# hsp-iit/roft

Hardware: AMD Instinct MI355X
Metric: tracker frames/sec per object (640x480) + ADD-S vs CPU ref (higher is better)
Workload: dtype f64; 1 GPU; BASELINE config #4: 640x480, CV_32FC2 flow grid 1, 64 objects in total, 64 per GPU (sharded by object, no data-path collective; result rows all-gathered over RCCL at N > 1), masks+poses at 5 fps with 6-frame delay, flow-aided masks, re-sync and outlier rejection on, frames submitted in batches of at most 8; objects_per_gpu=64, objects_total=64, width=640, height=480, batch_frames=8, ranks=1, backend=nccl

## Files before the change

include/roft_engine.h:

```cpp
#ifndef ROFT_ENGINE_H
#define ROFT_ENGINE_H

#include <stddef.h>
#include <stdint.h>

#ifdef __cplusplus
extern "C" {
#endif

#define ROFT_ABI_VERSION 2

#define ROFT_OK 0
#define ROFT_ERR_INVALID (-1)
#define ROFT_ERR_DEVICE (-2)
#define ROFT_ERR_CAPACITY (-3)
#define ROFT_ERR_STATE (-4)

#define ROFT_FLOW_S16C2 11
#define ROFT_FLOW_F32C2 13

#define ROFT_MEAS_NONE 0
#define ROFT_MEAS_VELOCITY 1
#define ROFT_MEAS_POSE 2
#define ROFT_MEAS_POSE_VELOCITY 3
// ... 53 lines not shown
                            int reweight, double x_out[6], double P_out[36], int* status_out);

int roft_mask_propagate(uint8_t* mask, int W, int H, const roft_flow* flows, int n_flows,
                        int frames_between);

int roft_pose_process_noise(const double psd_lin_acc[3], const double sigma_ang_vel[3], double T,
                            double Q[81]);
int roft_ukf_predict(const double mean[13], const double P[144], const double Q[81], double T,
                     const roft_ut_params* ut, double mean_out[13], double P_out[144]);
int roft_ukf_correct(const double mean[13], const double P[144], int type, const double* meas,
                     const double* Rdiag, const roft_ut_params* ut, double mean_out[13],
                     double P_out[144], int* status_out);

int roft_mesh_classify(const roft_mesh* mesh, uint8_t* flip_out, int* closed_out);
int roft_render_depth(const roft_mesh* mesh, const double x[3], const double q[4],
                      const roft_camera* cam, int divider, float* tile);
int roft_depth_likelihood(const roft_camera* cam, const float* depth, const uint8_t* mask,
                          const float* tile, int divider, double* L_out, long* samples_out);
int roft_outlier_test(const roft_camera* cam, int divider, const float* depth, const uint8_t* mask, const roft_mesh* mesh,
                      const double x[6], const double q[8], int bands, int vertex_cache, int window_pixels, double L_out[2],
                      long samples_out[2], int* selected_out, float* tiles_out);
int roft_outlier_test_split(const roft_camera* cam, int divider, const float* depth, const uint8_t* mask, const roft_mesh* mesh,
                            const double x[6], const double q[8], int bands, int vertex_cache, int window_pixels, int split,
                            double L_out[2], long samples_out[2], int* selected_out, float* tiles_out);
int roft_render_depth_mode(const roft_mesh* mesh, const double x[3], const double q[4], const roft_camera* cam, int divider, int mode,
                           float* tile);
int roft_outlier_test_mode(const roft_camera* cam, int divider, const float* depth, const uint8_t* mask, const roft_mesh* mesh,
                           const double x[6], const double q[8], int bands, int vertex_cache, int window_pixels, int split, int mode,
                           double L_out[2], long samples_out[2], int* selected_out, float* tiles_out);

#define ROFT_POSE_ERROR_ADD  0
#define ROFT_POSE_ERROR_ADDS 1
int roft_pose_errors(int kind, const double* points, int n_points, const double* est, const double* ref, int n_poses,
                     double* out);


typedef struct roft_engine roft_engine;

typedef struct {
    roft_camera cam;
    int flow_type;
    int flow_grid;
    float flow_scale;
    double sample_time;
    roft_ut_params ut;
    double depth_maximum;
    double subsampling_radius;
    int flow_weighting;
    int use_pose, use_pose_resync, use_velocity;
    int outlier_rejection;
    int flow_aided_segmentation;
    int mask_frames_between;
    int pose_frames_between;
    int stamped_masks;
    int max_objects;
    double ukf_cholesky_guard;
    double ukf_cholesky_guard_bilinear;
    int device;
    int max_batch_frames;
    int mask_workgroups_per_object;
    int outlier_bands_per_alternative;
    int render_mode;
} roft_config;

typedef struct {
    double p_mean0[13];
    double p_cov0_diag[12];
    double v_mean0[6];
    double v_cov0_diag[6];
    double p_sigma_ang_vel[3];
    double p_psd_lin_acc[3];
    double v_q_diag[6];
    double p_meas_cov_v[3], p_meas_cov_w[3], p_meas_cov_x[3], p_meas_cov_q[3];
    double v_meas_cov_flow[2];
    roft_mesh mesh;
} roft_object_desc;

#define ROFT_RETAIN_FRAMES 16
typedef struct {
    double dt;
    const float* depth;
    const void* flow;
    const uint8_t* mask;
    int pose_valid;
    double pose_x[3];
    double pose_q[4];
    int mem_kind;
    double stamp;
    double mask_stamp;
} roft_frame_input;

typedef struct {
    double pose[13];
    double twist[6];
    int n_flow_points;
    int outlier_selected;
    double outlier_L[2];
} roft_object_output;

int roft_default_config(roft_config* cfg, int width, int height, int flow_type);
int roft_default_object(roft_object_desc* obj);

int roft_engine_create(const roft_config* cfg, roft_engine** out);
int roft_engine_destroy(roft_engine* e);
int roft_object_add(roft_engine* e, const roft_object_desc* desc, int* obj_id);

#define ROFT_RESTART_KEEP_MESH 1
int roft_objects_restart(roft_engine* e, const int* obj_ids, const roft_object_desc* descs, int n, int flags);
typedef struct { long long calls, objects, meshes_replaced; } roft_engine_restart_stats;
int roft_engine_get_restart_stats(roft_engine* e, roft_engine_restart_stats* out);

int roft_frame_submit(roft_engine* e, const roft_frame_input* inputs, int n_inputs);
int roft_frames_submit(roft_engine* e, const roft_frame_input* inputs, int n_objects, int n_frames);

#define ROFT_LABEL_U8  1
#define ROFT_LABEL_U16 2
typedef struct {
    const void* labels;
    int label_type;
    int label;
} roft_label_mask;
int roft_frames_submit_labels(roft_engine* e, const roft_frame_input* inputs, const roft_label_mask* labels, int n_objects, int n_frames);
int roft_labels_to_masks(const void* labels, int label_type, int W, int H, const int* values, int n, uint8_t* masks_out, int* counts_out);

int roft_step(roft_engine* e);
int roft_engine_retain_frames(const roft_engine* e);
int roft_sync(roft_engine* e);
int roft_get_state(roft_engine* e, int obj_id, double pose13[13], double P12[144], double twist6[6],
                   double Pv[36]);
int roft_get_outputs(roft_engine* e, roft_object_output* outs, int n_outs);
int roft_get_mask(roft_engine* e, int obj_id, uint8_t* mask_out);

int roft_engine_enable_log(roft_engine* e, int n_frames);
int roft_engine_get_log(roft_engine* e, int first_frame, int n_frames, roft_object_output* outs);
int roft_engine_get_log_rows(roft_engine* e, int first_frame, int n_frames, double* rows);
int roft_engine_score_log(roft_engine* e, int kind, int obj_id, int first_frame, int n_frames, const double* points,
                          int n_points, const double* ref, double* out);

typedef struct {
    long long frames;
    long long batches;
    long long launches;
    long long event_ops;
    long long h2d_bytes;
    long long h2d_copies;
} roft_engine_stats;
int roft_engine_get_stats(roft_engine* e, roft_engine_stats* out);

typedef struct {
    int batch;
    int frames;
    int steady, throttled, handoff, early_lanes, outlier_parts_halved;
    int launches, event_ops;
    double t_submit_us;
    double submit_us;
    double wait_us;
    double step_us;
    double t_done_us;
} roft_batch_trace;
int roft_engine_get_batch_trace(roft_engine* e, roft_batch_trace* out, int capacity, int* n_out);

void* roft_engine_stream(roft_engine* e);

int roft_engine_enable_timing(roft_engine* e, int enable);
int roft_engine_get_timing(roft_engine* e, int* n_out, const char*** names_out, const float** ms_out,
                           const int** launches_out);

void* roft_host_alloc(size_t bytes);
void roft_host_free(void* p);
int roft_host_is_pinned(const void* p);

typedef struct {
    int levels;
    int radius;
    int iterations;
    float det_min;
} roft_of_params;

int roft_default_of_params(roft_of_params* p);

int roft_optical_flow(const uint8_t* prev_gray, const uint8_t* cur_gray, int W, int H, const roft_of_params* p,
                      int out_type, void* flow_out);

typedef struct roft_flow_producer roft_flow_producer;
int roft_flow_producer_create(int W, int H, int max_pairs, const roft_of_params* p, int out_type, int device,
                              roft_flow_producer** out);
int roft_flow_producer_destroy(roft_flow_producer* fp);
int roft_flow_producer_run(roft_flow_producer* fp, const uint8_t* const* prev, const uint8_t* const* cur,
                           void* const* out, int n_pairs);
int roft_flow_producer_sync(roft_flow_producer* fp);
void* roft_flow_producer_stream(roft_flow_producer* fp);

#define ROFT_IMAGE_GRAY8 1
#define ROFT_IMAGE_BGR8  2
#define ROFT_IMAGE_RGB8  3
typedef struct {
    const void* image;
    int image_type;
} roft_frame_image;
int roft_engine_enable_flow(roft_engine* e, const roft_of_params* p);
int roft_frames_submit_images(roft_engine* e, const roft_frame_input* inputs, const roft_label_mask* labels,
                              const roft_frame_image* images, int n_objects, int n_frames);
int roft_engine_get_flow(roft_engine* e, int obj_id, void* flow_out);
typedef struct {
    long long images;
    long long image_bytes;
    long long pyramids;
    long long pairs;
} roft_engine_flow_stats;
int roft_engine_get_flow_stats(roft_engine* e, roft_engine_flow_stats* out);
int roft_image_to_gray(const void* image, int image_type, int W, int H, uint8_t* gray_out);

typedef struct {
    float tolerance_abs, tolerance_rel;
} roft_of_consistency;
int roft_default_of_consistency(roft_of_consistency* c);
int roft_optical_flow_checked(const uint8_t* prev_gray, const uint8_t* cur_gray, int W, int H, const roft_of_params* p,
                              const roft_of_consistency* c, float* flow_out);
int roft_flow_producer_set_consistency(roft_flow_producer* fp, const roft_of_consistency* c);
int roft_engine_enable_flow_consistency(roft_engine* e, const roft_of_consistency* c);

#define ROFT_DEPTH_Z16 1
#define ROFT_DEPTH_ALIGN_MAX_SPAN 16
typedef struct {
    int   type;
    float scale;
    int   align;
    roft_camera cam;
    float R[9];
    float t[3];
} roft_depth_source;
int roft_engine_enable_raw_depth(roft_engine* e, const roft_depth_source* src);
int roft_engine_get_depth(roft_engine* e, int obj_id, float* depth_out);
typedef struct {
    long long images;
    long long image_bytes;
    long long products;
} roft_engine_depth_stats;
int roft_engine_get_depth_stats(roft_engine* e, roft_engine_depth_stats* out);
int roft_depth_convert(const uint16_t* raw, int W, int H, float scale, float* out);
int roft_depth_align(const uint16_t* raw, const roft_depth_source* src, const roft_camera* colour, float* out);

typedef struct {
    int32_t frame;
    int32_t n_mask;
    int32_t n_render;
    int32_t n_both;
    int32_t n_depth;
    int32_t n_front;
    int32_t n_behind;
    int32_t reserved;
    double  depth_err;
} roft_quality_record;
typedef struct {
    int   every;
    float depth_tolerance;
} roft_quality_params;
int roft_default_quality_params(roft_quality_params* p);
int roft_engine_enable_quality(roft_engine* e, const roft_quality_params* p);
int roft_engine_get_quality(roft_engine* e, int first_frame, int n_frames, roft_quality_record* out);
int roft_track_quality(const roft_camera* cam, int divider, const float* depth, const uint8_t* mask, const roft_mesh* mesh,
                       const double x[3], const double q[4], float depth_tolerance, double depth_maximum, int window_pixels,
                       roft_quality_record* out);

typedef struct {
    long long silhouettes;
    long long frames;
} roft_engine_pose_mask_stats;
int roft_engine_enable_pose_masks(roft_engine* e, const int* obj_ids, int n_ids);
int roft_engine_get_pose_mask_stats(roft_engine* e, roft_engine_pose_mask_stats* out);
int roft_pose_silhouette(const roft_camera* cam, const roft_mesh* mesh, const double x[3], const double q[4], int bands, int vertex_cache,
                         uint8_t* mask_out, int* count_out);

typedef struct {
    long long resolved;
    long long hidden;
    long long pixels_removed;
} roft_engine_pose_mask_occlusion_stats;
int roft_engine_enable_pose_mask_occlusion(roft_engine* e, const int* obj_ids, const int* scene_ids, int n_ids);
int roft_engine_get_pose_mask_occlusion_stats(roft_engine* e, roft_engine_pose_mask_occlusion_stats* out);
int roft_pose_silhouettes_occluded(const roft_camera* cam, const roft_mesh* meshes, int n, const double* x ,
                                   const double* q , int bands, int vertex_cache,
                                   uint8_t* masks_out , int* counts_out );

typedef struct {
    float front_tolerance;
    float behind_tolerance;
} roft_pose_mask_gate;
int roft_default_pose_mask_gate(roft_pose_mask_gate* g);
int roft_engine_enable_pose_mask_depth_gate(roft_engine* e, const roft_pose_mask_gate* g);
typedef struct {
    long long gated;
    long long emptied;
    long long pixels_front;
    long long pixels_behind;
} roft_engine_pose_mask_gate_stats;
int roft_engine_get_pose_mask_gate_stats(roft_engine* e, roft_engine_pose_mask_gate_stats* out);
int roft_pose_silhouettes_gated(const roft_camera* cam, const roft_mesh* meshes, int n, const double* x ,
                                const double* q , const float* depth , const roft_pose_mask_gate* g,
                                int bands, int vertex_cache, uint8_t* masks_out ,
                                int* counts_out , int* removed_out );

typedef struct {
    float tint[3];
    float opacity;
    float ambient;
} roft_scene_style;

#define ROFT_SCENE_MAX_INSTANCES 256

typedef struct {
    int n_frames;
    int n_instances;
    const int* mesh_index;
    const double* poses;
    const uint8_t* valid;
    const uint8_t* background;
    int background_frames;
    int gray_background;
    const roft_scene_style* styles;
    int window_pixels;
} roft_scene_desc;

typedef struct roft_scene_renderer roft_scene_renderer;
int roft_scene_renderer_create(const roft_camera* cam, const roft_mesh* meshes, int n_meshes, int max_frames_per_call, int device,
                               roft_scene_renderer** out);
int roft_scene_renderer_destroy(roft_scene_renderer* r);
int roft_scene_render(roft_scene_renderer* r, const roft_scene_desc* desc, uint8_t* rgb_out, float* depth_out, int32_t* instance_out,
                      int32_t* triangle_out);
int roft_render_scene(const roft_camera* cam, const roft_mesh* meshes, int n_meshes, const roft_scene_desc* desc, uint8_t* rgb_out,
                      float* depth_out, int32_t* instance_out, int32_t* triangle_out);

int roft_debug_plan(const roft_config* cfg, const int* pose_valid, int n_frames, int* n_steps, int* n_corrections,
                    int* outlier, int* slots);
int roft_debug_restart_check(const roft_config* cfg, int n_objects, const int* has_mesh, const int* enrolled, int enrol_all,
                             const int* obj_ids, const roft_object_desc* descs, int n, int flags);
int roft_debug_probe_streams(roft_engine* e, double out[25]);
int roft_debug_sector_rate(int device, double* sectors_per_second);
int roft_debug_get_residency(roft_engine* e, unsigned long long out[32]);
int roft_debug_outlier_split(int mode);
int roft_debug_pose_errors_kernel_ms(double* ms_out);
int roft_debug_scene_kernel_ms(roft_scene_renderer* r, double ms_out[2]);
int roft_debug_depth_kernel_ms(roft_engine* e, double* ms_out);
int roft_debug_quality_kernel_ms(roft_engine* e, double* ms_out);
int roft_debug_pose_mask_kernel_ms(roft_engine* e, double* ms_out);
int roft_debug_get_dbg(roft_engine* e, int obj_id, long long out[32]);

#ifdef __cplusplus
}
#endif
#endif
```

roft_amd/_lib.py:

```python
import collections
import ctypes as C
import os
import subprocess

_HERE = os.path.dirname(os.path.abspath(__file__))
CSRC = os.path.join(_HERE, "csrc")
SO = os.environ.get("ROFT_LIB_SO") or os.path.join(CSRC, "libroft_hip.so")

OK = 0
ERR_INVALID, ERR_DEVICE, ERR_CAPACITY, ERR_STATE = -1, -2, -3, -4
FLOW_S16C2 = 11
FLOW_F32C2 = 13
MEAS_NONE, MEAS_VELOCITY, MEAS_POSE, MEAS_POSE_VELOCITY = 0, 1, 2, 3
MEM_HOST, MEM_DEVICE = 0, 1
RETAIN_FRAMES = 16
MAX_BATCH_FRAMES = 8
MAX_FLOW_CHASE = 30
RENDER_CONTRACT, RENDER_GL = 0, 1
ABI_VERSION = 2
POSE_ERROR_ADD, POSE_ERROR_ADDS = 0, 1
RESTART_KEEP_MESH = 1
LABEL_U8, LABEL_U16 = 1, 2
IMAGE_GRAY8, IMAGE_BGR8, IMAGE_RGB8 = 1, 2, 3
DEPTH_Z16 = 1
DEPTH_ALIGN_MAX_SPAN = 16
SCENE_MAX_INSTANCES = 256


class RoftError(RuntimeError):
    pass


class Camera(C.Structure):
    _c_name_ = "roft_camera"
    _fields_ = [("width", C.c_int), ("height", C.c_int), ("fx", C.c_double), ("fy", C.c_double),
                ("cx", C.c_double), ("cy", C.c_double)]


class Flow(C.Structure):
    _c_name_ = "roft_flow"
    _fields_ = [("data", C.c_void_p), ("type", C.c_int), ("cols", C.c_int), ("rows", C.c_int),
                ("grid", C.c_int), ("scale", C.c_float), ("valid", C.c_int)]


class UT(C.Structure):
    _c_name_ = "roft_ut_params"
    _fields_ = [("alpha", C.c_double), ("beta", C.c_double), ("kappa", C.c_double)]


class OFParams(C.Structure):
    _c_name_ = "roft_of_params"
    _fields_ = [("levels", C.c_int), ("radius", C.c_int), ("iterations", C.c_int), ("det_min", C.c_float)]


class OFConsistency(C.Structure):
    _c_name_ = "roft_of_consistency"
    _fields_ = [("tolerance_abs", C.c_float), ("tolerance_rel", C.c_float)]


class Mesh(C.Structure):
    _c_name_ = "roft_mesh"
    _fields_ = [("verts", C.c_void_p), ("n_verts", C.c_int), ("tris", C.c_void_p), ("n_tris", C.c_int)]


class Config(C.Structure):
    _c_name_ = "roft_config"
    _fields_ = [("cam", Camera), ("flow_type", C.c_int), ("flow_grid", C.c_int), ("flow_scale", C.c_float),
                ("sample_time", C.c_double), ("ut", UT), ("depth_maximum", C.c_double),
                ("subsampling_radius", C.c_double), ("flow_weighting", C.c_int), ("use_pose", C.c_int),
                ("use_pose_resync", C.c_int), ("use_velocity", C.c_int), ("outlier_rejection", C.c_int),
                ("flow_aided_segmentation", C.c_int), ("mask_frames_between", C.c_int),
                ("pose_frames_between", C.c_int), ("stamped_masks", C.c_int), ("max_objects", C.c_int), ("ukf_cholesky_guard", C.c_double),
                ("ukf_cholesky_guard_bilinear", C.c_double),
                ("device", C.c_int), ("max_batch_frames", C.c_int), ("mask_workgroups_per_object", C.c_int),
                ("outlier_bands_per_alternative", C.c_int), ("render_mode", C.c_int)]


class ObjectDesc(C.Structure):
    _c_name_ = "roft_object_desc"
    _fields_ = [("p_mean0", C.c_double * 13), ("p_cov0_diag", C.c_double * 12), ("v_mean0", C.c_double * 6),
                ("v_cov0_diag", C.c_double * 6), ("p_sigma_ang_vel", C.c_double * 3),
                ("p_psd_lin_acc", C.c_double * 3), ("v_q_diag", C.c_double * 6),
                ("p_meas_cov_v", C.c_double * 3), ("p_meas_cov_w", C.c_double * 3),
                ("p_meas_cov_x", C.c_double * 3), ("p_meas_cov_q", C.c_double * 3),
                ("v_meas_cov_flow", C.c_double * 2), ("mesh", Mesh)]


class FrameInput(C.Structure):
    _c_name_ = "roft_frame_input"
    _fields_ = [("dt", C.c_double), ("depth", C.c_void_p), ("flow", C.c_void_p), ("mask", C.c_void_p),
                ("pose_valid", C.c_int), ("pose_x", C.c_double * 3), ("pose_q", C.c_double * 4),
                ("mem_kind", C.c_int), ("stamp", C.c_double), ("mask_stamp", C.c_double)]


class LabelMask(C.Structure):
    _c_name_ = "roft_label_mask"
    _fields_ = [("labels", C.c_void_p), ("label_type", C.c_int), ("label", C.c_int)]


class FrameImage(C.Structure):
    _c_name_ = "roft_frame_image"
    _fields_ = [("image", C.c_void_p), ("image_type", C.c_int)]


class EngineFlowStats(C.Structure):
    _c_name_ = "roft_engine_flow_stats"
    _fields_ = [("images", C.c_longlong), ("image_bytes", C.c_longlong), ("pyramids", C.c_longlong), ("pairs", C.c_longlong)]


class DepthSource(C.Structure):
    _c_name_ = "roft_depth_source"
    _fields_ = [("type", C.c_int), ("scale", C.c_float), ("align", C.c_int), ("cam", Camera), ("R", C.c_float * 9), ("t", C.c_float * 3)]


class EngineDepthStats(C.Structure):
    _c_name_ = "roft_engine_depth_stats"
    _fields_ = [("images", C.c_longlong), ("image_bytes", C.c_longlong), ("products", C.c_longlong)]


class QualityRecord(C.Structure):
    _c_name_ = "roft_quality_record"
    _fields_ = [("frame", C.c_int32), ("n_mask", C.c_int32), ("n_render", C.c_int32), ("n_both", C.c_int32), ("n_depth", C.c_int32),
                ("n_front", C.c_int32), ("n_behind", C.c_int32), ("reserved", C.c_int32), ("depth_err", C.c_double)]


class QualityParams(C.Structure):
    _c_name_ = "roft_quality_params"
    _fields_ = [("every", C.c_int), ("depth_tolerance", C.c_float)]


class EnginePoseMaskStats(C.Structure):
    _c_name_ = "roft_engine_pose_mask_stats"
    _fields_ = [("silhouettes", C.c_longlong), ("frames", C.c_longlong)]


class EnginePoseMaskOcclusionStats(C.Structure):
    _c_name_ = "roft_engine_pose_mask_occlusion_stats"
    _fields_ = [("resolved", C.c_longlong), ("hidden", C.c_longlong), ("pixels_removed", C.c_longlong)]


class PoseMaskGate(C.Structure):
    _c_name_ = "roft_pose_mask_gate"
    _fields_ = [("front_tolerance", C.c_float), ("behind_tolerance", C.c_float)]


class EnginePoseMaskGateStats(C.Structure):
    _c_name_ = "roft_engine_pose_mask_gate_stats"
    _fields_ = [("gated", C.c_longlong), ("emptied", C.c_longlong), ("pixels_front", C.c_longlong), ("pixels_behind", C.c_longlong)]


class EngineRestartStats(C.Structure):
    _c_name_ = "roft_engine_restart_stats"
    _fields_ = [("calls", C.c_longlong), ("objects", C.c_longlong), ("meshes_replaced", C.c_longlong)]


class EngineStats(C.Structure):
    _c_name_ = "roft_engine_stats"
    _fields_ = [("frames", C.c_longlong), ("batches", C.c_longlong), ("launches", C.c_longlong),
                ("event_ops", C.c_longlong), ("h2d_bytes", C.c_longlong), ("h2d_copies", C.c_longlong)]


class BatchTrace(C.Structure):
    _c_name_ = "roft_batch_trace"
    _fields_ = [("batch", C.c_int), ("frames", C.c_int), ("steady", C.c_int), ("throttled", C.c_int), ("handoff", C.c_int),
                ("early_lanes", C.c_int), ("outlier_parts_halved", C.c_int), ("launches", C.c_int), ("event_ops", C.c_int),
                ("t_submit_us", C.c_double), ("submit_us", C.c_double), ("wait_us", C.c_double), ("step_us", C.c_double),
                ("t_done_us", C.c_double)]


class ObjectOutput(C.Structure):
    _c_name_ = "roft_object_output"
    _fields_ = [("pose", C.c_double * 13), ("twist", C.c_double * 6), ("n_flow_points", C.c_int),
                ("outlier_selected", C.c_int), ("outlier_L", C.c_double * 2)]


class SceneStyle(C.Structure):
    _c_name_ = "roft_scene_style"
    _fields_ = [("tint", C.c_float * 3), ("opacity", C.c_float), ("ambient", C.c_float)]


class SceneDesc(C.Structure):
    _c_name_ = "roft_scene_desc"
    _fields_ = [("n_frames", C.c_int), ("n_instances", C.c_int), ("mesh_index", C.c_void_p), ("poses", C.c_void_p),
                ("valid", C.c_void_p), ("background", C.c_void_p), ("background_frames", C.c_int), ("gray_background", C.c_int),
                ("styles", C.c_void_p), ("window_pixels", C.c_int)]


Fn = collections.namedtuple("Fn", "name restype argtypes optional")
_int, _vp, _ip, _dp = C.c_int, C.c_void_p, C.POINTER(C.c_int), C.POINTER(C.c_double)
_P = C.POINTER
_REQUIRED, _OPTIONAL = False, True
ABI = (
    Fn("roft_last_error_string", C.c_char_p, [], _REQUIRED),
    Fn("roft_device_count", _int, [], _REQUIRED),
    Fn("roft_abi_version", _int, [], _REQUIRED),
    Fn("roft_flow_measurement", _int, [_P(Camera), _vp, _vp, _P(Flow), C.c_double, C.c_float, C.c_double, _int, _vp, _vp, _vp, _ip], _REQUIRED),
    Fn("roft_kf_predict", _int, [_vp] * 5, _REQUIRED),
    Fn("roft_skf_correct", _int, [_vp, _vp, _int, _vp, _vp, _vp, _int, _vp, _vp, _ip], _REQUIRED),
    Fn("roft_skf_correct_points", _int, [_P(Camera), C.c_double, _vp, _vp, _int, _vp, _vp, _vp, _vp, _int, _vp, _vp, _ip], _REQUIRED),
    Fn("roft_mask_propagate", _int, [_vp, _int, _int, _P(Flow), _int, _int], _REQUIRED),
    Fn("roft_pose_process_noise", _int, [_vp, _vp, C.c_double, _vp], _REQUIRED),
    Fn("roft_ukf_predict", _int, [_vp, _vp, _vp, C.c_double, _P(UT), _vp, _vp], _REQUIRED),
    Fn("roft_ukf_correct", _int, [_vp, _vp, _int, _vp, _vp, _P(UT), _vp, _vp, _ip], _REQUIRED),
    Fn("roft_mesh_classify", _int, [_P(Mesh), _vp, _ip], _REQUIRED),
    Fn("roft_render_depth", _int, [_P(Mesh), _vp, _vp, _P(Camera), _int, _vp], _REQUIRED),
    Fn("roft_depth_likelihood", _int, [_P(Camera), _vp, _vp, _vp, _int, _dp, _P(C.c_long)], _REQUIRED),
    Fn("roft_outlier_test", _int, [_P(Camera), _int, _vp, _vp, _P(Mesh), _vp, _vp, _int, _int, _int, _vp, _vp, _ip, _vp], _REQUIRED),
    Fn("roft_outlier_test_split", _int, [_P(Camera), _int, _vp, _vp, _P(Mesh), _vp, _vp, _int, _int, _int, _int, _vp, _vp, _ip, _vp], _REQUIRED),
    Fn("roft_render_depth_mode", _int, [_P(Mesh), _vp, _vp, _P(Camera), _int, _int, _vp], _REQUIRED),
    Fn("roft_outlier_test_mode", _int, [_P(Camera), _int, _vp, _vp, _P(Mesh), _vp, _vp, _int, _int, _int, _int, _int, _vp, _vp, _ip, _vp],
       _REQUIRED),
    Fn("roft_pose_errors", _int, [_int, _vp, _int, _vp, _vp, _int, _vp], _OPTIONAL),
    Fn("roft_default_config", _int, [_P(Config), _int, _int, _int], _REQUIRED),
    Fn("roft_default_object", _int, [_P(ObjectDesc)], _REQUIRED),
    Fn("roft_engine_create", _int, [_P(Config), _P(_vp)], _REQUIRED),
    Fn("roft_engine_destroy", _int, [_vp], _REQUIRED),
    Fn("roft_object_add", _int, [_vp, _P(ObjectDesc), _ip], _REQUIRED),
    Fn("roft_objects_restart", _int, [_vp, _ip, _P(ObjectDesc), _int, _int], _OPTIONAL),
    Fn("roft_engine_get_restart_stats", _int, [_vp, _P(EngineRestartStats)], _OPTIONAL),
    Fn("roft_frame_submit", _int, [_vp, _P(FrameInput), _int], _REQUIRED),
    Fn("roft_frames_submit", _int, [_vp, _P(FrameInput), _int, _int], _REQUIRED),
    Fn("roft_frames_submit_labels", _int, [_vp, _P(FrameInput), _P(LabelMask), _int, _int], _OPTIONAL),
    Fn("roft_labels_to_masks", _int, [_vp, _int, _int, _int, _ip, _int, _vp, _ip], _OPTIONAL),
    Fn("roft_step", _int, [_vp], _REQUIRED),
    Fn("roft_engine_retain_frames", _int, [_vp], _REQUIRED),
    Fn("roft_sync", _int, [_vp], _REQUIRED),
    Fn("roft_get_state", _int, [_vp, _int, _vp, _vp, _vp, _vp], _REQUIRED),
    Fn("roft_get_outputs", _int, [_vp, _P(ObjectOutput), _int], _REQUIRED),
    Fn("roft_get_mask", _int, [_vp, _int, _vp], _REQUIRED),
    Fn("roft_engine_enable_log", _int, [_vp, _int], _REQUIRED),
    Fn("roft_engine_get_log", _int, [_vp, _int, _int, _P(ObjectOutput)], _REQUIRED),
    Fn("roft_engine_get_log_rows", _int, [_vp, _int, _int, _vp], _REQUIRED),
    Fn("roft_engine_score_log", _int, [_vp, _int, _int, _int, _int, _vp, _int, _vp, _vp], _OPTIONAL),
    Fn("roft_engine_get_stats", _int, [_vp, _P(EngineStats)], _REQUIRED),
    Fn("roft_engine_get_batch_trace", _int, [_vp, _P(BatchTrace), _int, _ip], _REQUIRED),
    Fn("roft_engine_stream", _vp, [_vp], _REQUIRED),
    Fn("roft_engine_enable_timing", _int, [_vp, _int], _REQUIRED),
    Fn("roft_engine_get_timing", _int, [_vp, _ip, _P(_P(C.c_char_p)), _P(_P(C.c_float)), _P(_ip)], _REQUIRED),
    Fn("roft_host_alloc", _vp, [C.c_size_t], _REQUIRED),
    Fn("roft_host_free", None, [_vp], _REQUIRED),
    Fn("roft_host_is_pinned", _int, [_vp], _REQUIRED),
    Fn("roft_default_of_params", _int, [_P(OFParams)], _REQUIRED),
    Fn("roft_optical_flow", _int, [_vp, _vp, _int, _int, _P(OFParams), _int, _vp], _REQUIRED),
    Fn("roft_flow_producer_create", _int, [_int, _int, _int, _P(OFParams), _int, _int, _P(_vp)], _REQUIRED),
    Fn("roft_flow_producer_destroy", _int, [_vp], _REQUIRED),
    Fn("roft_flow_producer_run", _int, [_vp, _P(_vp), _P(_vp), _P(_vp), _int], _REQUIRED),
    Fn("roft_flow_producer_sync", _int, [_vp], _REQUIRED),
    Fn("roft_flow_producer_stream", _vp, [_vp], _REQUIRED),
    Fn("roft_engine_enable_flow", _int, [_vp, _P(OFParams)], _OPTIONAL),
    Fn("roft_frames_submit_images", _int, [_vp, _P(FrameInput), _P(LabelMask), _P(FrameImage), _int, _int], _OPTIONAL),
    Fn("roft_engine_get_flow", _int, [_vp, _int, _vp], _OPTIONAL),
    Fn("roft_engine_get_flow_stats", _int, [_vp, _P(EngineFlowStats)], _OPTIONAL),
    Fn("roft_image_to_gray", _int, [_vp, _int, _int, _int, _vp], _OPTIONAL),
    Fn("roft_default_of_consistency", _int, [_P(OFConsistency)], _OPTIONAL),
    Fn("roft_optical_flow_checked", _int, [_vp, _vp, _int, _int, _P(OFParams), _P(OFConsistency), _vp], _OPTIONAL),
    Fn("roft_flow_producer_set_consistency", _int, [_vp, _P(OFConsistency)], _OPTIONAL),
    Fn("roft_engine_enable_flow_consistency", _int, [_vp, _P(OFConsistency)], _OPTIONAL),
    Fn("roft_engine_enable_raw_depth", _int, [_vp, _P(DepthSource)], _OPTIONAL),
    Fn("roft_engine_get_depth", _int, [_vp, _int, _vp], _OPTIONAL),
    Fn("roft_engine_get_depth_stats", _int, [_vp, _P(EngineDepthStats)], _OPTIONAL),
    Fn("roft_depth_convert", _int, [_vp, _int, _int, C.c_float, _vp], _OPTIONAL),
    Fn("roft_depth_align", _int, [_vp, _P(DepthSource), _P(Camera), _vp], _OPTIONAL),
    Fn("roft_default_quality_params", _int, [_P(QualityParams)], _OPTIONAL),
    Fn("roft_engine_enable_quality", _int, [_vp, _P(QualityParams)], _OPTIONAL),
    Fn("roft_engine_get_quality", _int, [_vp, _int, _int, _vp], _OPTIONAL),
    Fn("roft_track_quality", _int, [_P(Camera), _int, _vp, _vp, _P(Mesh), _vp, _vp, C.c_float, C.c_double, _int, _P(QualityRecord)], _OPTIONAL),
    Fn("roft_engine_enable_pose_masks", _int, [_vp, _ip, _int], _OPTIONAL),
    Fn("roft_engine_get_pose_mask_stats", _int, [_vp, _P(EnginePoseMaskStats)], _OPTIONAL),
    Fn("roft_pose_silhouette", _int, [_P(Camera), _P(Mesh), _vp, _vp, _int, _int, _vp, _ip], _OPTIONAL),
    Fn("roft_engine_enable_pose_mask_occlusion", _int, [_vp, _ip, _ip, _int], _OPTIONAL),
    Fn("roft_engine_get_pose_mask_occlusion_stats", _int, [_vp, _P(EnginePoseMaskOcclusionStats)], _OPTIONAL),
    Fn("roft_pose_silhouettes_occluded", _int, [_P(Camera), _P(Mesh), _int, _vp, _vp, _int, _int, _vp, _ip], _OPTIONAL),
    Fn("roft_default_pose_mask_gate", _int, [_P(PoseMaskGate)], _OPTIONAL),
    Fn("roft_engine_enable_pose_mask_depth_gate", _int, [_vp, _P(PoseMaskGate)], _OPTIONAL),
    Fn("roft_engine_get_pose_mask_gate_stats", _int, [_vp, _P(EnginePoseMaskGateStats)], _OPTIONAL),
    Fn("roft_pose_silhouettes_gated", _int, [_P(Camera), _P(Mesh), _int, _vp, _vp, _vp, _P(PoseMaskGate), _int, _int, _vp, _ip, _ip], _OPTIONAL),
    Fn("roft_scene_renderer_create", _int, [_P(Camera), _P(Mesh), _int, _int, _int, _P(_vp)], _OPTIONAL),
    Fn("roft_scene_renderer_destroy", _int, [_vp], _OPTIONAL),
    Fn("roft_scene_render", _int, [_vp, _P(SceneDesc), _vp, _vp, _vp, _vp], _OPTIONAL),
    Fn("roft_render_scene", _int, [_P(Camera), _P(Mesh), _int, _P(SceneDesc), _vp, _vp, _vp, _vp], _OPTIONAL),
    Fn("roft_debug_plan", _int, [_P(Config), _vp, _int, _vp, _vp, _vp, _vp], _OPTIONAL),
    Fn("roft_debug_restart_check", _int, [_P(Config), _int, _ip, _ip, _int, _ip, _P(ObjectDesc), _int, _int], _OPTIONAL),
    Fn("roft_debug_probe_streams", _int, [_vp, _dp], _OPTIONAL),
    Fn("roft_debug_sector_rate", _int, [_int, _dp], _OPTIONAL),
    Fn("roft_debug_get_residency", _int, [_vp, _P(C.c_ulonglong)], _OPTIONAL),
    Fn("roft_debug_outlier_split", _int, [_int], _OPTIONAL),
    Fn("roft_debug_pose_errors_kernel_ms", _int, [_dp], _OPTIONAL),
    Fn("roft_debug_scene_kernel_ms", _int, [_vp, _dp], _OPTIONAL),
    Fn("roft_debug_depth_kernel_ms", _int, [_vp, _dp], _OPTIONAL),
    Fn("roft_debug_quality_kernel_ms", _int, [_vp, _dp], _OPTIONAL),
    Fn("roft_debug_pose_mask_kernel_ms", _int, [_vp, _dp], _OPTIONAL),
    Fn("roft_debug_get_dbg", _int, [_vp, _int, _P(C.c_longlong)], _OPTIONAL),
)
ABI_SYMBOLS = [f.name for f in ABI]
NEWER_SYMBOLS = tuple(f.name for f in ABI if f.optional and not f.name.startswith("roft_debug_"))


def build(force=False):
    srcs = [os.path.join(CSRC, f) for f in os.listdir(CSRC) if f.endswith((".hip", ".h"))]
    srcs.append(os.path.join(_HERE, "..", "include", "roft_engine.h"))
    stale = (not os.path.exists(SO)) or any(os.path.getmtime(s) > os.path.getmtime(SO) for s in srcs)
    if force or stale:
        jobs = str(min(8, os.cpu_count() or 1))
        r = subprocess.run(["make", "-C", CSRC, "-j", jobs, "libroft_hip.so"], capture_output=True, text=True)
        if r.returncode != 0:
            raise RoftError("building libroft_hip.so failed:\n" + r.stdout[-4000:] + r.stderr[-4000:])
    return SO


_lib = None


def lib():
    global _lib
    if _lib is not None:
        return _lib
    if not os.path.exists(SO):
        build()
    L = C.CDLL(SO)
    version = L.roft_abi_version() if hasattr(L, "roft_abi_version") else None
    if version != ABI_VERSION:
        raise RoftError("%s has ABI version %s, this binding mirrors version %d: rebuild the library" % (SO, version, ABI_VERSION))
    for f in ABI:
        if f.optional and not hasattr(L, f.name):
            continue
        fn = getattr(L, f.name)
        fn.restype, fn.argtypes = f.restype, f.argtypes
    _lib = L
    return L


def check(rc):
    if rc != OK:
        raise RoftError("libroft_hip error %d: %s" % (rc, lib().roft_last_error_string().decode()))


def require_device():
    if lib().roft_device_count() <= 0:
        raise RoftError("no HIP device visible: roft_amd has no CPU fallback")
```

roft_amd/csrc/batch_plan.h:

```cpp
#pragma once

#include <cstdlib>

namespace roft {
namespace host {

constexpr int kPlanLanes = 2;

struct SchedKnobs {
    int handoff_mode = 1;
    int prep_mode = 1;
    int part_mode = 1;
    int feat_mask_mode = 1;
    int lanes_wait_skf = 1;
    int early_lanes = 1;
    int ctrl_ingest = 1;
    int gather_copy = 1;
    int outlier_steady_div = 2;
    bool host_prof = false;
    bool host_prof_per_batch = false;
    bool one_stream = false;
};

inline SchedKnobs knobs_from_env()
{
    SchedKnobs k;
    auto num = [](const char* name, int& v) { const char* s = getenv(name); if (s) v = atoi(s); return s != nullptr; };
    num("ROFT_HANDOFF", k.handoff_mode);
    num("ROFT_PREP_AHEAD", k.prep_mode);
    num("ROFT_MASK_PART_GATE", k.part_mode);
    num("ROFT_FEAT_ON_MASK", k.feat_mask_mode);
    if (!num("ROFT_LANES_WAIT_SKF", k.lanes_wait_skf) && getenv("ROCPROF_COUNTER_COLLECTION")) k.handoff_mode = 0;
    num("ROFT_EARLY_LANES", k.early_lanes);
    num("ROFT_CTRL_INGEST", k.ctrl_ingest);
    num("ROFT_GATHER_COPY", k.gather_copy);
    num("ROFT_OUTLIER_STEADY_DIV", k.outlier_steady_div);
    const char* hp = getenv("ROFT_HOST_PROF");
    k.host_prof = hp && hp[0] == '1';
    k.host_prof_per_batch = k.host_prof && hp[1] == '+';
    const char* one = getenv("ROFT_ONE_STREAM");
    k.one_stream = one && one[0] == '1';
    return k;
}

struct SubmitFacts {
    int T = 1;
    bool had_uploads = false;
    bool produced_flows = false;
    unsigned plain_mask_frames = 0;
    int label_sets = 0;
    int pose_masks = 0;
    int pose_resolve = 0;
    bool any_feat = false, any_feat_now = false;
    bool feat_dep_in_batch = false;
    int n_segments[kPlanLanes] = {1, 1};
    bool lin_any[kPlanLanes] = {false, false};
    int lane_objs[kPlanLanes] = {0, 0}, lane_old_first[kPlanLanes] = {0, 0};
    int relabel_wait[kPlanLanes] = {-1, -1};
};

struct PlanInputs : SubmitFacts {
    SchedKnobs knobs;
    bool multi = true;
    bool timing = false;
    int timing_level = 2;
    bool wait_value_ok = true;
    bool have_skf_started = true;
    int n_obj = 0, cus = 256;
    int batch_counter = 0, idle_mark = 0, lead = 6, completed_batches = 0;
    int outlier_bands_per_alternative = 0;
    bool conflict_free = false;
    bool up_stream_distinct = true;
    bool feat_used_two_back = false;
    bool vel_used_prev = false;
    bool done_used_relabel[kPlanLanes] = {false, false};
    int quality_frames = 0;
};

enum class Signal {
    none,
    stop,
    record,
};
enum class FeatRun { none, mask_stream, behind_skf };
enum class VelWait { none, ev_ctrl, ev_part, ev_mask };
enum class Release {
    none,
    ev_vel,
    ev_skf,
    gate,
    ctrl_only,
};

struct LanePlan {
    bool early = false;
    bool wait_relabel = false;
    Release release = Release::none;
    bool wait_feat = false;
    bool wait_prev_vel = false;
    bool gate_second = false;
    Signal ev_done = Signal::none;
};

struct BatchPlan {
    bool steady = false, handoff = false;
    bool early_lanes = false;
    bool prep = false;
    bool prep_waits_mask = false, prep_waits_feat = false;
    bool wait_up = false;
    bool try_fused = false;
    bool label_ingest = false;
    bool pose_silhouettes = false;
    bool pose_resolve = false;
    Signal ev_ctrl = Signal::none, ev_prep = Signal::none;
    bool part_gate = false;
    Signal ev_mask = Signal::none;
    FeatRun feat = FeatRun::none;
    Signal ev_feat = Signal::none;
    VelWait vel_waits = VelWait::none;
    bool feat_waits_mask = false;
    Signal ev_skf = Signal::none, ev_vel = Signal::none;
    LanePlan lane[kPlanLanes];
    int outlier_div = 1;
    bool quality = false;
    bool quality_waits_mask = false;
    bool quality_waits_lane = false;
    Signal ev_quality = Signal::none;
};

template <class AloneFn>
BatchPlan plan_batch(const PlanInputs& in, AloneFn&& alone)
{
    const SchedKnobs& k = in.knobs;
    BatchPlan p;
    const bool multi = in.multi;
    const bool batch = multi && in.T > 1;
    const bool full = in.timing && in.timing_level > 1;
    auto ends = [full](bool signalled) { return !signalled ? Signal::none : full ? Signal::record : Signal::stop; };
    auto by_mode = [](int mode, bool by_index, bool by_count) { return mode == 2 || (mode == 3 && by_index) || (mode == 1 && by_index && by_count); };
    const bool cus_to_spare = 8 * in.n_obj <= in.cus;
    const bool own_sets = in.feat_dep_in_batch || in.any_feat_now;

    p.steady = in.batch_counter - in.idle_mark >= in.lead;

    p.handoff = batch && k.handoff_mode > 0 && in.wait_value_ok && !(k.handoff_mode == 1 && p.steady && !cus_to_spare) && !own_sets &&
                in.have_skf_started;
    const bool early_ok = p.handoff && !p.steady && k.early_lanes != 0 && in.conflict_free && alone();
    p.early_lanes = early_ok && cus_to_spare;
    bool any_early = false;
    for (int l = 0; l < kPlanLanes; ++l) {
        p.lane[l].early = p.early_lanes || (early_ok && in.n_segments[l] > 1 && in.lane_old_first[l] > 0 &&
                                            8 * (in.lane_objs[l] - in.lane_old_first[l]) <= in.cus && 2 * in.lane_objs[l] <= in.cus);
        any_early = any_early || p.lane[l].early;
    }

    p.prep = batch && in.up_stream_distinct && by_mode(k.prep_mode, p.steady, !cus_to_spare);
    p.prep_waits_mask = p.prep && in.batch_counter >= 2;
    p.prep_waits_feat = p.prep_waits_mask && in.feat_used_two_back;
    p.wait_up = multi && (in.had_uploads || in.produced_flows) && !p.prep;
    p.try_fused = k.ctrl_ingest != 0 && !p.prep && in.plain_mask_frames != 0 && !in.timing;
    p.ev_ctrl = (multi && (in.T == 1 || any_early)) ? Signal::stop : Signal::none;
    p.label_ingest = in.label_sets > 0;
    p.pose_silhouettes = in.pose_masks > 0;
    p.pose_resolve = p.pose_silhouettes && in.pose_resolve > 0;
    p.ev_prep = !p.prep ? Signal::none
                : (full || (in.plain_mask_frames == 0 && !p.label_ingest && !p.pose_silhouettes)) ? Signal::record : Signal::stop;

    p.part_gate = batch && by_mode(k.part_mode, !p.steady, cus_to_spare);
    p.ev_mask = ends(multi);

    const bool feat_behind_skf = batch && !(k.feat_mask_mode == 2 || (k.feat_mask_mode == 1 && 16 * in.n_obj <= in.cus));
    p.feat = !in.any_feat ? FeatRun::none : feat_behind_skf ? FeatRun::behind_skf : FeatRun::mask_stream;
    p.ev_feat = ends(multi && p.feat == FeatRun::mask_stream);

    p.vel_waits = !multi ? VelWait::none : in.T == 1 ? VelWait::ev_ctrl : p.part_gate ? VelWait::ev_part : VelWait::ev_mask;
    p.feat_waits_mask = p.feat == FeatRun::behind_skf && p.part_gate;
    const bool lanes_wait_skf = p.feat == FeatRun::behind_skf && k.lanes_wait_skf != 0 && !own_sets;
    p.ev_skf = ends(lanes_wait_skf);
    p.ev_vel = ends(multi);

    const bool lanes_wait_feat = p.ev_feat != Signal::none && (in.T > 1 || in.any_feat_now);
    for (int l = 0; l < kPlanLanes; ++l) {
        LanePlan& lp = p.lane[l];
        const int wb = in.relabel_wait[l];
        lp.wait_relabel = multi && wb >= in.completed_batches && wb < in.batch_counter && in.done_used_relabel[l];
        if (!in.lin_any[l]) continue;
        lp.ev_done = ends(true);
        if (!multi) continue;
        const bool tests = in.n_segments[l] > 1;
        if (lp.early) {
            lp.release = Release::ctrl_only;
            lp.wait_prev_vel = tests && in.batch_counter - 1 >= in.completed_batches && in.batch_counter >= 1 && in.vel_used_prev;
            lp.gate_second = !p.early_lanes;
        } else if (p.handoff) {
            lp.release = Release::gate;
        } else {
            lp.release = lanes_wait_skf ? Release::ev_skf : Release::ev_vel;
            lp.wait_feat = lanes_wait_feat && tests;
        }
    }

    p.quality = in.quality_frames > 0;
    p.quality_waits_mask = p.quality && multi;
    p.quality_waits_lane = p.quality && multi && in.lin_any[0];
    p.ev_quality = ends(p.quality);

    p.outlier_div = (in.outlier_bands_per_alternative == 0 && p.steady && k.outlier_steady_div > 1) ? k.outlier_steady_div : 1;
    return p;
}

enum class PrepLaunch { none, mask_ingest, label_ingest, pose_silhouettes, pose_resolve };
inline PrepLaunch prep_last_launch(const BatchPlan& p, unsigned plain_mask_frames)
{
    return p.pose_resolve ? PrepLaunch::pose_resolve
           : p.pose_silhouettes ? PrepLaunch::pose_silhouettes
           : p.label_ingest ? PrepLaunch::label_ingest
           : plain_mask_frames ? PrepLaunch::mask_ingest : PrepLaunch::none;
}
inline int pose_silhouette_launches(const BatchPlan& p) { return p.pose_resolve ? 2 : p.pose_silhouettes ? 1 : 0; }

}
}
```

roft_amd/csrc/engine_debug.hip:

```cpp
#include "engine_internal.h"


extern "C" int roft_debug_get_dbg(roft_engine* e, int id, long long out[32])
{
    if (!e || id < 0 || id >= (int)e->objs.size()) return ROFT_ERR_INVALID;
    if (roft_sync(e) != ROFT_OK) return ROFT_ERR_DEVICE;
    ObjState* st = new ObjState();
    hipError_t err = hipMemcpy(st, e->arr.state.p + id, sizeof(ObjState), hipMemcpyDeviceToHost);
    if (err == hipSuccess) std::memcpy(out, st->dbg, sizeof(long long) * 32);
    delete st;
    if (err == hipSuccess) err = hipMemset(reinterpret_cast<char*>(e->arr.state.p + id) + offsetof(ObjState, dbg), 0, sizeof(long long) * 32);
    return err == hipSuccess ? ROFT_OK : ROFT_ERR_DEVICE;
}

extern "C" int roft_debug_outlier_split(int mode)
{
    roft::set_outlier_split(mode);
    return ROFT_OK;
}

extern "C" int roft_debug_get_residency(roft_engine* e, unsigned long long out[32])
{
    if (!e || !out) return ROFT_ERR_INVALID;
    if (roft_sync(e) != ROFT_OK) return ROFT_ERR_DEVICE;
    if (hipMemcpy(out, e->arr.residency.p, sizeof(unsigned long long) * 32, hipMemcpyDeviceToHost) != hipSuccess) return ROFT_ERR_DEVICE;
    return hipMemset(e->arr.residency.p, 0, sizeof(unsigned long long) * 32) == hipSuccess ? ROFT_OK : ROFT_ERR_DEVICE;
}

extern "C" int roft_debug_sector_rate(int device, double* sectors_per_second)
{
    if (!sectors_per_second) return fail(ROFT_ERR_INVALID, "null output");
    HIP_TRY(hipSetDevice(device));
    const size_t bytes = (size_t)2 << 30;
    unsigned* buf = nullptr;
    unsigned* sink = nullptr;
    HIP_TRY(hipMalloc(reinterpret_cast<void**>(&buf), bytes));
    const int grid = 2048;
    hipError_t err = hipMalloc(reinterpret_cast<void**>(&sink), (size_t)grid * 1024 * sizeof(unsigned));
    hipEvent_t e0 = nullptr, e1 = nullptr;
    if (err == hipSuccess) err = hipMemset(buf, 0, bytes);
    if (err == hipSuccess) err = hipEventCreate(&e0);
    if (err == hipSuccess) err = hipEventCreate(&e1);
    float best_ms = 0.f;
    for (int rep = 0; rep < 5 && err == hipSuccess; ++rep) {
        (void)hipEventRecord(e0, nullptr);
        hipLaunchKernelGGL(probe_sectors_kernel, dim3(grid), dim3(1024), 0, nullptr, buf, (unsigned)(bytes / 64 - 1), 0x9e3779b9u * (unsigned)(rep + 1), sink);
        (void)hipEventRecord(e1, nullptr);
        err = hipEventSynchronize(e1);
        float ms = 0.f;
        if (err == hipSuccess) err = hipEventElapsedTime(&ms, e0, e1);
        if (rep > 0 && (best_ms == 0.f || ms < best_ms)) best_ms = ms;
    }
    if (e0) (void)hipEventDestroy(e0);
    if (e1) (void)hipEventDestroy(e1);
    (void)hipFree(sink);
    (void)hipFree(buf);
    if (err != hipSuccess || !(best_ms > 0.f)) return fail(ROFT_ERR_DEVICE, std::string("sector-rate probe: ") + hipGetErrorString(err));
    *sectors_per_second = (double)grid * 1024.0 * 8.0 / ((double)best_ms * 1e-3);
    return ROFT_OK;
}

extern "C" int roft_debug_probe_streams(roft_engine* e, double out[25])
{
    if (!e || !out) return ROFT_ERR_INVALID;
    if (roft_sync(e) != ROFT_OK) return ROFT_ERR_DEVICE;
    hipStream_t st[5] = {e->pose_stream[0], e->pose_stream[1], e->vel_stream, e->stream, e->up_stream};
    (void)set_max_dynamic_lds(reinterpret_cast<const void*>(probe_blocker_kernel), 150 * 1024);
    DevBuf<int> flag;
    if (flag.ensure(1) != hipSuccess) return ROFT_ERR_DEVICE;
    const int cus = device_cu_count();
    for (int a = 0; a < 5; ++a)
        for (int b = 0; b < 5; ++b) {
            out[a * 5 + b] = 0.0;
            if (a == b || st[a] == st[b]) continue;
            double best = 1e30;
            for (int rep = 0; rep < 3; ++rep) {
                (void)hipDeviceSynchronize();
                const double t0 = host_now_us();
                hipLaunchKernelGGL(probe_blocker_kernel, dim3(3 * cus), dim3(64), 150 * 1024, st[a], 10000ll);
                hipLaunchKernelGGL(probe_tiny_kernel, dim3(1), dim3(64), 0, st[b], flag.p);
                (void)hipStreamSynchronize(st[b]);
                best = std::min(best, host_now_us() - t0);
            }
            out[a * 5 + b] = best;
        }
    (void)hipDeviceSynchronize();
    return hipGetLastError() == hipSuccess ? ROFT_OK : ROFT_ERR_DEVICE;
}

extern "C" int roft_debug_plan(const roft_config* cfg, const int* pose_valid, int n_frames, int* n_steps, int* n_corrections,
                               int* outlier, int* slots )
{
    if (!cfg || !pose_valid || n_frames < 0) return ROFT_ERR_INVALID;
    Sched o;
    roft_frame_input in{};
    for (int k = 0; k < n_frames; ++k) {
        FrameCtrl c;
        clear_ctrl(c);
        in.pose_valid = pose_valid[k];
        if (!build_pose_program(*cfg, o, in, c)) return ROFT_ERR_CAPACITY;
        o.frame_idx++;
        o.track_frames++;
        if (n_steps) n_steps[k] = c.n_steps;
        int nc = 0;
        for (int s = 0; s < c.n_steps; ++s) {
            nc += c.steps[s].n_corr;
            if (slots) slots[k * kMaxSteps + s] = c.steps[s].twist_slot;
        }
        if (slots) for (int s = c.n_steps; s < kMaxSteps; ++s) slots[k * kMaxSteps + s] = -1;
        if (n_corrections) n_corrections[k] = nc;
        if (outlier) outlier[k] = c.outlier_step;
    }
    return ROFT_OK;
}
```

roft_amd/csrc/engine_internal.h:

```cpp
#pragma once

#include <hip/hip_runtime.h>

#include <algorithm>
#include <cfloat>
#include <chrono>
#include <cmath>
#include <cstdio>
#include <cstdlib>
#include <cstring>
#include <map>
#include <mutex>
#include <string>
#include <vector>

#include "roft_device.h"
#include "mesh_class.h"
#include "mesh_clusters.h"
#include "scene.h"
#include "batch_plan.h"
#include "pose_mask_gate.h"
#include "opticalflow.h"
#include "depth.h"
#include "quality.h"
// ... 11 lines not shown
    do {                                                                                                   \
        hipError_t _e = (expr);                                                                            \
        if (_e != hipSuccess)                                                                              \
            return fail(ROFT_ERR_DEVICE, std::string(#expr) + ": " + hipGetErrorString(_e));               \
    } while (0)
#define TRY(call) do { if (int _rc = (call)) return _rc; } while (0)

template <class T>
struct DevBuf {
    T* p = nullptr;
    size_t n = 0;
    DevBuf() = default;
    DevBuf(DevBuf&& o) noexcept { swap(o); }
    DevBuf& operator=(DevBuf&& o) noexcept { swap(o); return *this; }
    void swap(DevBuf& o) { std::swap(p, o.p); std::swap(n, o.n); }
    ~DevBuf() { release(); }
    void release()
    {
        if (p) (void)hipFree(p);
        p = nullptr;
        n = 0;
    }
    hipError_t ensure(size_t count, bool zero = false)
    {
        if (count <= n && p) return hipSuccess;
        release();
        hipError_t e = hipMalloc(reinterpret_cast<void**>(&p), std::max<size_t>(count, 1) * sizeof(T));
        if (e != hipSuccess) { p = nullptr; return e; }
        n = count;
        if (zero) e = hipMemset(p, 0, std::max<size_t>(count, 1) * sizeof(T));
        return e;
    }
};

inline int check_mesh(const roft_mesh& m, const std::string& what, bool may_be_absent, int tri_index_bits = 0)
{
    if (!has_mesh(m)) return may_be_absent ? ROFT_OK : fail(ROFT_ERR_INVALID, what + ": no vertices or no triangles");
    if (tri_index_bits > 0 && m.n_tris >= (1 << tri_index_bits))
        return fail(ROFT_ERR_INVALID, what + ": 2^" + std::to_string(tri_index_bits) + " triangles or more (a triangle's index is kept in that many bits)");
    const MeshFault f = check_mesh_arrays(m.verts, m.n_verts, m.tris, m.n_tris);
    if (f.kind == MeshFault::kNullArray) return fail(ROFT_ERR_INVALID, what + ": null vertex or triangle array");
    if (f.kind == MeshFault::kBadIndex)
        return fail(ROFT_ERR_INVALID, what + ": triangle " + std::to_string(f.triangle) + " refers to vertex " + std::to_string(f.vertex) + " of " +
                                          std::to_string(m.n_verts));
    return ROFT_OK;
}

struct DeviceMesh {
    DevBuf<float> verts;
    DevBuf<int32_t> tris;
    DevBuf<uint8_t> flip;
    DevBuf<uint32_t> cl_headers, cl_words;
    DevBuf<float> cl_slots, box_corners;
    int n_verts = 0, n_tris = 0, n_clusters = 0;
    bool closed = false;

    int upload(const roft_mesh& m, MeshLayout layout, hipStream_t s)
    {
        const bool clusters = layout == MeshLayout::kWalkClusters;
        n_verts = n_tris = n_clusters = 0;
        closed = false;
        if (!has_mesh(m)) return ROFT_OK;
        PreparedMesh pm;
        prepare_mesh(m.verts, m.n_verts, m.tris, m.n_tris, layout, pm);
        HIP_TRY(verts.ensure((size_t)3 * m.n_verts));
        HIP_TRY(tris.ensure((size_t)3 * m.n_tris));
        HIP_TRY(hipMemcpyAsync(verts.p, m.verts, sizeof(float) * 3 * m.n_verts, hipMemcpyHostToDevice, s));
        HIP_TRY(hipMemcpyAsync(tris.p, pm.tris(m.tris), sizeof(int32_t) * 3 * m.n_tris, hipMemcpyHostToDevice, s));
        if (pm.closed) {
            HIP_TRY(flip.ensure((size_t)m.n_tris));
            HIP_TRY(hipMemcpyAsync(flip.p, pm.flip.data(), (size_t)m.n_tris, hipMemcpyHostToDevice, s));
        }
        MeshClusters mc;
        if (clusters) {
            build_clusters(m.verts, m.n_verts, pm.tris(m.tris), m.n_tris, pm.closed ? pm.flip.data() : nullptr,
                           pm.bucket.empty() ? nullptr : pm.bucket.data(), mc);
            HIP_TRY(cl_headers.ensure(mc.headers.size()));
            HIP_TRY(cl_slots.ensure(mc.slots.size()));
            HIP_TRY(cl_words.ensure(mc.words.size()));
            HIP_TRY(box_corners.ensure(24));
            HIP_TRY(hipMemcpyAsync(cl_headers.p, mc.headers.data(), sizeof(uint32_t) * mc.headers.size(), hipMemcpyHostToDevice, s));
            HIP_TRY(hipMemcpyAsync(cl_slots.p, mc.slots.data(), sizeof(float) * mc.slots.size(), hipMemcpyHostToDevice, s));
            HIP_TRY(hipMemcpyAsync(cl_words.p, mc.words.data(), sizeof(uint32_t) * mc.words.size(), hipMemcpyHostToDevice, s));
            HIP_TRY(hipMemcpyAsync(box_corners.p, &mc.box[0][0], sizeof(float) * 24, hipMemcpyHostToDevice, s));
        }
        HIP_TRY(hipStreamSynchronize(s));
        n_verts = m.n_verts;
        n_tris = m.n_tris;
        n_clusters = mc.n_clusters;
        closed = pm.closed;
        return ROFT_OK;
    }

    SceneMesh scene_mesh() const
    {
        const bool has = has_mesh(*this);
        return SceneMesh{has ? verts.p : nullptr, has ? tris.p : nullptr, closed ? flip.p : nullptr, n_verts, n_tris};
    }
    void describe(ObjParams& p) const
    {
        const SceneMesh m = scene_mesh();
        p.verts = m.verts; p.tris = m.tris; p.tri_flip = m.flip;
        p.n_verts = m.n_verts; p.n_tris = m.n_tris;
        const bool cl = has_mesh(*this) && n_clusters > 0;
        p.cl_headers = cl ? cl_headers.p : nullptr; p.cl_slots = cl ? cl_slots.p : nullptr; p.cl_words = cl ? cl_words.p : nullptr;
        p.box_corners = cl ? box_corners.p : nullptr; p.n_clusters = cl ? n_clusters : 0;
    }
};

inline size_t flow_bytes(const DevFlowFmt& f)
{
    return (size_t)f.cols * f.rows * 2 * (f.type == ROFT_FLOW_S16C2 ? sizeof(int16_t) : sizeof(float));
}

inline DevCamera make_cam(const roft_camera& c)
{
    DevCamera d;
    d.W = c.width;
    d.H = c.height;
    d.wpr = c.width / 32;
    d.divider = (c.width == 640) ? 2 : 4;
    d.fx = c.fx; d.fy = c.fy; d.cx = c.cx; d.cy = c.cy;
    return d;
}

inline int check_geometry(int W, int H)
{
    if (W <= 0 || H <= 0 || (W % 32) != 0 || (((size_t)W * H) % 64) != 0)
        return fail(ROFT_ERR_INVALID, "image width must be a multiple of 32 and width*height a multiple of 64");
    if ((size_t)W * H >= (1u << 24))
        return fail(ROFT_ERR_INVALID, "width*height must be < 2^24 (float-accumulated sampling index, hpp:237)");
    return ROFT_OK;
}

struct Arrays {
    EngineArrays a{};
    DevBuf<ObjParams> params;
    DevBuf<ObjState> state;
    DevBuf<FrameCtrl> ctrl;
    DevBuf<uint32_t> planes;
    DevBuf<int32_t> map;
    DevBuf<FlowRec> cand, recs;
    DevBuf<double> norms;
    DevBuf<int> npts;
    DevBuf<MaskRec> mrec;
    DevBuf<unsigned> mask_general;
    DevBuf<uint32_t> feat_pix;
    DevBuf<float> feat_depth;
    DevBuf<uint32_t> zbuf;
    DevBuf<uint32_t> zmerge;
    DevBuf<int> zcount;
    int ensure_zmerge(int n, size_t tpix)
    {
        const size_t slabs = std::max<size_t>((size_t)n, std::min<size_t>((size_t)n * kMaxOutlierParts, (size_t)std::max(device_cu_count() / 2, 1)));
        const size_t need = (size_t)kNumLin * slabs * 2 * tpix;
        if (need > zmerge.n || !zmerge.p || tpix != a.zmerge_stride || slabs != a.zmerge_slabs) {
            HIP_TRY(zmerge.ensure(need));
            a.zmerge_stride = tpix;
            a.zmerge_slabs = slabs;
        }
        HIP_TRY(zcount.ensure((size_t)kNumLin * n * 2 * kMaxOutlierParts, true));
        a.zmerge = zmerge.p;
        a.zcount = zcount.p;
        return ROFT_OK;
    }
    DevBuf<roft_object_output> log;
    DevBuf<unsigned long long> skf_started, residency;

    int alloc(int n_obj, int T, const DevCamera& cam, const DevFlowFmt& ffmt, int radius)
    {
        a.n_obj = n_obj;
        a.T = 1;
        a.cam = cam;
        a.ffmt = ffmt;
        a.plane_words = (size_t)cam.wpr * cam.H;
        const size_t npix = (size_t)cam.W * cam.H;
        a.cand_cap = ((int)((npix + radius - 1) / std::max(radius, 1)) + 9) & ~1;
        a.feat_cap = (int)(npix / 2 + 8);
        a.tile_w = cam.W / cam.divider;
        a.tile_h = cam.H / cam.divider;
        HIP_TRY(params.ensure(n_obj, true));
        HIP_TRY(state.ensure(n_obj, true));
        HIP_TRY(ctrl.ensure((size_t)n_obj * T, true));
        HIP_TRY(planes.ensure((size_t)n_obj * kPlaneSlotsTotal * 2 * a.plane_words, true));
        HIP_TRY(mrec.ensure((size_t)2 * n_obj * (kMaxBatch + 1), true));
        HIP_TRY(mask_general.ensure(n_obj, true));
        HIP_TRY(map.ensure((size_t)n_obj * npix, true));
        HIP_TRY(cand.ensure((size_t)n_obj * T * a.cand_cap));
        HIP_TRY(recs.ensure((size_t)n_obj * T * a.cand_cap));
        HIP_TRY(npts.ensure((size_t)n_obj * T, true));
        HIP_TRY(norms.ensure((size_t)n_obj * 3 * a.cand_cap));
        HIP_TRY(feat_pix.ensure((size_t)n_obj * kFeatRing * a.feat_cap));
        HIP_TRY(feat_depth.ensure((size_t)n_obj * kFeatRing * a.feat_cap));
        HIP_TRY(zbuf.ensure((size_t)2 * a.tile_w * a.tile_h));
        if (int rc = ensure_zmerge(n_obj, (size_t)a.tile_w * a.tile_h)) return rc;
        a.params = params.p; a.state = state.p; a.ctrl = ctrl.p; a.planes = planes.p; a.map = map.p;
        a.cand = cand.p; a.recs = recs.p; a.norms = norms.p; a.npts = npts.p; a.mrec = mrec.p;
        a.mask_general = mask_general.p;
        a.mrec_carry = mrec.p; a.slot_new = kSlotNew; a.slot_prev0 = -1; a.feat_pix = feat_pix.p; a.feat_depth = feat_depth.p;
        a.zbuf = zbuf.p;
        a.out_log = nullptr;
        a.log_cap = 0;
        a.max_tris = 0;
        a.max_verts = 0;
        a.meshes_without_clusters = 0;
        a.ukf_chol_guard = 0.0;
        a.ukf_chol_guard_bil = 0.0;
        a.mask_wgs = 0;
        a.outlier_parts = 0;
        a.dev_error = nullptr;
        a.k1_span = nullptr;
        HIP_TRY(skf_started.ensure(1, true));
        HIP_TRY(residency.ensure(32, true));
        a.residency = residency.p;
        a.skf_started = nullptr;
        a.handoff = 0;
        return ROFT_OK;
    }
};

struct PoseErrorScratch {
    DevBuf<double> pts, est, ref, cloud, partial, out;
    hipEvent_t ev0 = nullptr, ev1 = nullptr;
    bool timed = false;
    ~PoseErrorScratch()
    {
        if (ev0) (void)hipEventDestroy(ev0);
        if (ev1) (void)hipEventDestroy(ev1);
    }
};
int pose_errors_run(PoseErrorScratch& sc, int kind, const double* d_pts, int P, const double* est_host, PoseView est_dev,
                    const double* ref_host, int n, double* out_host, hipStream_t s);

inline void init_state(ObjState& st)
{
    std::memset(&st, 0, sizeof(st));
    for (PoseLane& pl : st.lane) { pl.pending_frame = -1; pl.outlier_selected = -1; }
    st.n_flow_points = -1;
}

inline void clear_ctrl(FrameCtrl& c)
{
    std::memset(&c, 0, sizeof(c));
    c.outlier_step = -1;
    c.feat_write = c.feat_read = -1;
}



struct FlowEntry {
    const void* ptr;
    int frame;
    int owned;
    const float* depth_before;
};

struct Sched {
    int frame_idx = 0;
    int track_frames = 0;
    bool seg_available = false;
    bool of_first_frame = true;
    bool flow_first_frame = true;
    bool features_initialized = false;
    int feat_slot = 0;
    int feat_next = 0;
    int feat_use[kFeatRing];
    int feat_batch[kFeatRing];
    int n_hist = 0;
    FlowEntry hist[kMaxFlowHist];
    int n_stamps = 0;
    double stamps[30];
    int n_vel = 0;
    int vel_buf[kTwistRing];
    int last_meas_slot = 0;
    int cur_slot = 0;
    int own[kNumLin] = {0, 1};
    int last_touch[kNumLin] = {-1, -1};
    int flows_since_mask = 0;
    int flows_buffered = 0;
    const float* depth_prev = nullptr;
    int pyr_prev = -1;
    const void* flow_made = nullptr;
    Sched() { for (int i = 0; i < kFeatRing; ++i) feat_use[i] = feat_batch[i] = -1; }
};

struct OwnedFlow {
    DevBuf<unsigned char> buf;
    DevBuf<float> depth;
    int last_ref_frame = -1;
};

struct HostObject {
    Sched s;
    int stepped_slot = 0, stepped_lane = 0;
    const void* stepped_flow = nullptr;
    const float* stepped_depth = nullptr;
    std::vector<OwnedFlow*> owned;
    DeviceMesh mesh;
    bool pose_masks = false;
    int pose_scene = -1, pose_zscene = -1;
    double pose0[7] = {0, 0, 0, 1, 0, 0, 0};
    roft_object_output last_out{};
    bool last_out_valid = false;
    ~HostObject() { for (auto* o : owned) delete o; }
};

struct FlowImageJob { const void* dev; int type; };
// ... 248 lines not shown
```

roft_amd/csrc/engine_step.hip:

```cpp
#include "engine_internal.h"

__global__ void ctrl_upload_kernel(const uint4* __restrict__ src, EngineArrays a, size_t n16, int reset)
{
    uint4* dst = reinterpret_cast<uint4*>(a.ctrl);
    const size_t i0 = (size_t)blockIdx.x * blockDim.x + threadIdx.x, stride = (size_t)gridDim.x * blockDim.x;
    for (size_t i = i0; i < n16; i += stride) dst[i] = src[i];
    if (reset)
        for (size_t i = i0; i < (size_t)a.T * a.n_obj; i += stride) roft::mask_reset_tables(a, i);
}


static hipEvent_t push_mark(roft_engine* e, const char* name, int which)
{
    const size_t idx = e->tmark.size();
    while (e->tev.size() <= idx) {
        hipEvent_t ev;
        (void)hipEventCreate(&ev);
        e->tev.push_back(ev);
    }
    int id = -1;
    if (name) {
        for (size_t i = 0; i < e->tnames_s.size(); ++i)
            if (e->tnames_s[i] == name) id = (int)i;
        if (id < 0) { e->tnames_s.push_back(name); id = (int)e->tnames_s.size() - 1; }
// ... 15 lines not shown
    if (!e->timing) return;
    *start = push_mark(e, nullptr, which);
    *stop = push_mark(e, name, which);
}

#define CHECK_LAUNCH(what)                                                                              \
    do {                                                                                                \
        hipError_t _e = hipGetLastError();                                                              \
        if (_e != hipSuccess) return fail(ROFT_ERR_DEVICE, std::string(what) + ": " + hipGetErrorString(_e)); \
    } while (0)

struct Enqueue {
    roft_engine* e;
    const BatchPlan& p;
    BatchSlot& cur;
    EngineArrays a;
    long long& launches;
    long long& evops;
    int wait(hipStream_t s, hipEvent_t ev)
    {
        HIP_TRY(hipStreamWaitEvent(s, ev, 0));
        ++evops;
        return ROFT_OK;
    }
    int wait_gate(hipStream_t s)
    {
        HIP_TRY(hipStreamWaitValue64(s, e->arr.skf_started.p, e->skf_total, hipStreamWaitValueGte, ~0ull));
        ++evops;
        return ROFT_OK;
    }
    static hipEvent_t stop(Signal how, hipEvent_t ev) { return how == Signal::stop ? ev : nullptr; }
    int signalled(Signal how, hipEvent_t ev, hipStream_t s)
    {
        if (how != Signal::record) return ROFT_OK;
        HIP_TRY(hipEventRecord(ev, s));
        ++evops;
        return ROFT_OK;
    }
};

static int enqueue_preparation(Enqueue& q)
{
    roft_engine* e = q.e;
    const PendingBatch& pb = e->pending;
    const BatchPlan& p = q.p;
    const EngineArrays& a = q.a;
    hipStream_t s = e->stream, sp = p.prep ? e->up_stream : s;
    if (p.wait_up) TRY(q.wait(s, q.cur.ev_up));
    if (p.prep_waits_mask) {
        BatchSlot& two_back = e->slot_of(e->batch_counter - 2);
        TRY(q.wait(sp, two_back.ev_mask));
        if (p.prep_waits_feat) TRY(q.wait(sp, two_back.ev_feat));
    }
    tmark(e, nullptr, p.prep ? 4 : 0);
    static_assert(sizeof(FrameCtrl) % 16 == 0, "FrameCtrl is copied in 16-byte units");
    const size_t n16 = (sizeof(FrameCtrl) * (size_t)a.n_obj * a.T + (p.label_ingest ? pb.label_table_bytes : 0)) / 16;
    const hipEvent_t ctrl_stop = Enqueue::stop(p.ev_ctrl, q.cur.ev_ctrl);
    const PrepLaunch last_launch = prep_last_launch(p, pb.facts.plain_mask_frames);
    auto label_ingest = [&]() -> int {
        LabelIngestArgs la;
        la.sets = reinterpret_cast<const LabelSet*>(a.ctrl + (size_t)a.n_obj * a.T);
        la.members = reinterpret_cast<const LabelMember*>(la.sets + pb.label_sets.size());
        la.planes = a.planes;
        la.plane_words = a.plane_words;
        la.obj_stride = (size_t)kPlaneSlotsTotal * 2 * a.plane_words;
        la.slot0 = a.slot_new;
        la.mrec = a.mrec;
        la.n_obj = a.n_obj;
        la.n_grp = a.cam.W * a.cam.H / 64;
        launch_label_ingest(la, (int)pb.label_sets.size(), sp, last_launch == PrepLaunch::label_ingest ? Enqueue::stop(p.ev_prep, q.cur.ev_prep) : nullptr);
        ++q.launches;
        CHECK_LAUNCH("label image ingest");
        return ROFT_OK;
    };
    auto pose_silhouettes = [&]() -> int {
        EnginePoseMasks& pm = e->pose_masks;
        SilhouetteArgs sa{};
        sa.ctrl = a.ctrl;
        sa.params = a.params;
        sa.planes = a.planes;
        sa.plane_words = a.plane_words;
        sa.obj_stride = (size_t)kPlaneSlotsTotal * 2 * a.plane_words;
        sa.slot0 = a.slot_new;
        sa.mrec = a.mrec;
        sa.n_obj = a.n_obj;
        sa.W = a.cam.W; sa.H = a.cam.H; sa.wpr = a.cam.wpr;
        sa.fx = (float)a.cam.fx; sa.fy = (float)a.cam.fy; sa.cx = (float)a.cam.cx; sa.cy = (float)a.cam.cy;
        int n_frames = 0;
        for (int t = 0; t < a.T && t < 8; ++t)
            if (pb.pose_mask_frames & (1u << t)) sa.frames_packed |= (unsigned)t << (4 * n_frames++);
        if (p.pose_resolve) {
            const int par = e->batch_counter & 1;
            sa.n_zscenes = pm.n_zscenes;
            sa.zbuf = pm.zbuf.p + (size_t)par * kMaxBatch * pm.n_zscenes * a.cam.W * a.cam.H;
            sa.zpairs = pm.zpairs.p + (size_t)par * kMaxBatch * e->cfg.max_objects;
            sa.zstats = pm.zstats.p;
        }
        if (pm.gate) {
            sa.gate = 1;
            sa.gate_tf = pm.gate_prm.front_tolerance;
            sa.gate_tb = pm.gate_prm.behind_tolerance;
            sa.gstats = pm.gstats.p;
            sa.zpairs = pm.zpairs.p + (size_t)(e->batch_counter & 1) * kMaxBatch * e->cfg.max_objects;
        }
        const int slot = e->batch_counter % roft_engine::kBatchRing;
        const hipEvent_t plan_stop = Enqueue::stop(p.ev_prep, q.cur.ev_prep);
        if (!p.prep) tmark(e, nullptr, 0);
        const int launched = launch_pose_silhouette(sa, n_frames, a.max_verts, 0, 1, sp, pm.ev_start[slot], plan_stop ? plan_stop : pm.ev_stop[slot]);
        if (launched != pose_silhouette_launches(p))
            return fail(ROFT_ERR_INVALID, "pose masks: the image does not fit the kernel's bit window");
        pm.last_slot = slot;
        pm.last_timed = plan_stop == nullptr;
        q.launches += launched;
        CHECK_LAUNCH(p.pose_resolve ? "pose silhouettes: clear, draw and resolve" : "pose silhouettes");
        if (!p.prep) tmark(e, "pose_silhouettes", 0);
        return ROFT_OK;
    };
    if (p.try_fused && launch_ctrl_ingest(q.cur.stage, a, n16, pb.facts.plain_mask_frames, sp, ctrl_stop)) {
        ++q.launches;
        CHECK_LAUNCH("FrameCtrl upload + mask ingest");
        if (p.label_ingest) TRY(label_ingest());
        return p.pose_silhouettes ? pose_silhouettes() : ROFT_OK;
    }
    hipExtLaunchKernelGGL(ctrl_upload_kernel, dim3((unsigned)std::min<size_t>((n16 + 255) / 256, 64)), dim3(256), 0, sp, nullptr, ctrl_stop, 0,
                          reinterpret_cast<const uint4*>(q.cur.stage), a, n16, 1);
    ++q.launches;
    CHECK_LAUNCH("FrameCtrl upload");
    int last = -1;
    for (int t = 0; t < a.T; ++t)
        if (pb.facts.plain_mask_frames & (1u << t)) last = t;
    for (int t = 0; t <= last; ++t)
        if (pb.facts.plain_mask_frames & (1u << t)) {
            launch_mask_ingest(a, t, sp, (t == last && last_launch == PrepLaunch::mask_ingest) ? Enqueue::stop(p.ev_prep, q.cur.ev_prep) : nullptr);
            ++q.launches;
        }
    CHECK_LAUNCH("mask ingest");
    if (p.label_ingest) TRY(label_ingest());
    if (p.pose_silhouettes) TRY(pose_silhouettes());
    if (p.prep) {
        TRY(q.signalled(p.ev_prep, q.cur.ev_prep, sp));
        tmark(e, "mask_prepare", 4);
        TRY(q.wait(s, q.cur.ev_prep));
    }
    return ROFT_OK;
}

static int enqueue_mask_frames(Enqueue& q)
{
    roft_engine* e = q.e;
    const BatchPlan& p = q.p;
    hipStream_t s = e->stream;
    tmark(e, nullptr, 0);
    q.launches += launch_mask_chain(q.a, e->cfg.mask_frames_between, e->cfg.flow_aided_segmentation, e->pending.new_mask_frames, s,
                                    Enqueue::stop(p.ev_mask, q.cur.ev_mask), p.part_gate ? q.cur.ev_part : nullptr);
    CHECK_LAUNCH("mask chain");
    tmark(e, "mask_chain", 0);
    TRY(q.signalled(p.ev_mask, q.cur.ev_mask, s));
    q.cur.feat_used = p.ev_feat != Signal::none;
    if (p.feat == FeatRun::mask_stream) {
        launch_features(q.a, s, Enqueue::stop(p.ev_feat, q.cur.ev_feat), e->pending.feat_frames);
        ++q.launches;
        CHECK_LAUNCH("features");
        tmark(e, "features", 0);
        TRY(q.signalled(p.ev_feat, q.cur.ev_feat, s));
    }
    return ROFT_OK;
}

static int enqueue_velocity(Enqueue& q)
{
    roft_engine* e = q.e;
    const BatchPlan& p = q.p;
    const EngineArrays& a = q.a;
    hipStream_t sv = e->vel_stream;
    if (p.vel_waits != VelWait::none)
        TRY(q.wait(sv, p.vel_waits == VelWait::ev_ctrl ? q.cur.ev_ctrl : p.vel_waits == VelWait::ev_part ? q.cur.ev_part : q.cur.ev_mask));
    {
        hipEvent_t k1_start = nullptr, k1_stop = nullptr;
        tmark_kernel(e, "flow_measure", 2, &k1_start, &k1_stop);
        EngineArrays ak = a;
        if (e->timing && (int)e->span_wgs.size() < roft_engine::kSpanLaunches && e->k1_span.p) {
            ak.k1_span = e->k1_span.p + (size_t)2 * kMaxBatch * e->cfg.max_objects * e->span_wgs.size();
            e->span_wgs.push_back(a.T * a.n_obj);
        }
        launch_flow_measure(ak, e->cfg.depth_maximum, (int)(size_t)e->cfg.subsampling_radius, sv, k1_start, k1_stop);
        ++q.launches;
        CHECK_LAUNCH("flow measurement");
    }
    const bool feat_behind = p.feat == FeatRun::behind_skf;
    const Signal skf_how = feat_behind ? p.ev_skf : p.ev_vel;
    const hipEvent_t skf_ev = feat_behind ? q.cur.ev_skf : q.cur.ev_vel;
    q.cur.vel_used = p.ev_vel != Signal::none;
    launch_skf_chain(a, e->cfg.flow_weighting, sv, Enqueue::stop(skf_how, skf_ev));
    ++q.launches;
    if (hipError_t le = hipGetLastError()) {
        e->knobs.handoff_mode = 0;
        return fail(ROFT_ERR_DEVICE, std::string("velocity filter chain: ") + hipGetErrorString(le));
    }
    e->skf_total += (unsigned long long)a.n_obj;
    tmark(e, "skf_chain", 2);
    TRY(q.signalled(skf_how, skf_ev, sv));
    if (feat_behind) {
        if (p.feat_waits_mask) TRY(q.wait(sv, q.cur.ev_mask));
        launch_features(a, sv, Enqueue::stop(p.ev_vel, q.cur.ev_vel), e->pending.feat_frames);
        ++q.launches;
        CHECK_LAUNCH("features");
        tmark(e, "features", 2);
        TRY(q.signalled(p.ev_vel, q.cur.ev_vel, sv));
    }
    return ROFT_OK;
}

static int enqueue_lane(Enqueue& q, int lin)
{
    roft_engine* e = q.e;
    const LanePlan& lp = q.p.lane[lin];
    hipStream_t sp = e->pose_stream[lin];
    q.cur.done_used[lin] = lp.ev_done != Signal::none;
    const SubmitFacts& facts = e->pending.facts;
    if (lp.wait_relabel) TRY(q.wait(sp, e->slot_of(facts.relabel_wait[lin]).ev_done[1 - lin]));
    if (!facts.lin_any[lin]) return ROFT_OK;
    const int which = lin == 0 ? 1 : 3;
    switch (lp.release) {
    case Release::none: break;
    case Release::ctrl_only: TRY(q.wait(sp, q.cur.ev_ctrl)); break;
    case Release::gate: TRY(q.wait_gate(sp)); break;
    case Release::ev_skf: TRY(q.wait(sp, q.cur.ev_skf)); break;
    case Release::ev_vel: TRY(q.wait(sp, q.cur.ev_vel)); break;
    }
    if (lp.wait_feat) TRY(q.wait(sp, q.cur.ev_feat));
    tmark(e, nullptr, which);
    OutlierLaunchOpts oo;
    oo.render_mode = e->cfg.render_mode;
    if (q.p.outlier_div > 1) oo.parts = -q.p.outlier_div;
    const int n_seg = facts.n_segments[lin];
    for (int seg = 0; seg < n_seg; ++seg) {
        const bool last = seg == n_seg - 1;
        if (seg == 1 && lp.gate_second) TRY(q.wait_gate(sp));
        launch_ukf_chain(q.a, e->cfg.ut, seg == 0, lin, sp, last ? Enqueue::stop(lp.ev_done, q.cur.ev_done[lin]) : nullptr);
        ++q.launches;
        CHECK_LAUNCH("pose chain segment");
        tmark(e, "ukf_chain", which);
        if (last) break;
        if (seg == 0 && lp.wait_prev_vel) TRY(q.wait(sp, e->slot_of(e->batch_counter - 1).ev_vel));
        TRY(launch_outlier(q.a, lin, sp, nullptr, &oo));
        ++q.launches;
        CHECK_LAUNCH("outlier rejection");
        tmark(e, "outlier_render_likelihood", which);
    }
    return q.signalled(lp.ev_done, q.cur.ev_done[lin], sp);
}

static int enqueue_quality(Enqueue& q)
{
    roft_engine* e = q.e;
    const BatchPlan& p = q.p;
    q.cur.quality_used = p.ev_quality != Signal::none;
    if (!p.quality) return ROFT_OK;
    const int slot = e->batch_counter % roft_engine::kBatchRing;
    hipStream_t sp = e->pose_stream[kNumLin - 1];
    if (p.quality_waits_mask) TRY(q.wait(sp, q.cur.ev_mask));
    if (p.quality_waits_lane) TRY(q.wait(sp, q.cur.ev_done[0]));
    int n_frames = 0;
    const unsigned packed = quality_frames_of_batch(e, &n_frames);
    EngineQuality& eq = e->quality;
    launch_quality(q.a, eq.ring.p, eq.cap, packed, n_frames, eq.prm.depth_tolerance, e->cfg.depth_maximum, 0, sp, eq.ev_start[slot],
                   Enqueue::stop(p.ev_quality, eq.ev_done[slot]));
    ++q.launches;
    CHECK_LAUNCH("track quality");
    tmark(e, "track_quality", 3);
    eq.last_slot = slot;
    return q.signalled(p.ev_quality, eq.ev_done[slot], sp);
}

static PlanInputs plan_inputs(roft_engine* e)
{
    PlanInputs in;
    static_cast<SubmitFacts&>(in) = e->pending.facts;
    in.knobs = e->knobs;
    in.multi = e->multi();
    in.timing = e->timing;
    in.timing_level = e->timing_level;
    in.wait_value_ok = e->wait_value_ok;
    in.have_skf_started = e->arr.skf_started.p != nullptr;
    in.n_obj = e->arr.a.n_obj;
    in.cus = device_cu_count();
    in.batch_counter = e->batch_counter; in.idle_mark = e->idle_mark; in.lead = e->lead; in.completed_batches = e->completed_batches;
    in.outlier_bands_per_alternative = e->cfg.outlier_bands_per_alternative;
    in.conflict_free = e->streams && e->streams->conflicts == 0;
    in.up_stream_distinct = e->up_stream != e->stream;
    if (e->quality.enabled) (void)quality_frames_of_batch(e, &in.quality_frames);
    in.feat_used_two_back = e->batch_counter >= 2 && e->slot_of(e->batch_counter - 2).feat_used;
    in.vel_used_prev = e->batch_counter >= 1 && e->slot_of(e->batch_counter - 1).vel_used;
    for (int l = 0; l < kNumLin; ++l) in.done_used_relabel[l] = in.relabel_wait[l] >= 0 && e->slot_of(in.relabel_wait[l]).done_used[1 - l];
    return in;
}

int step_batch(roft_engine* e)
{
    const PendingBatch& pb = e->pending;
    const int T = pb.facts.T;
    double hp_t = e->knobs.host_prof ? host_now_us() : 0.0;
    (void)hipGetLastError();
    const BatchPlan p = plan_batch(plan_inputs(e), [e] { return e->alone_on_device = alone_on_device(e->streams); });
    BatchSlot& cur = e->slot_of(e->batch_counter);
    Enqueue q{e, p, cur, e->arr.a, e->stats.launches, e->stats.event_ops};
    EngineArrays& a = q.a;
    a.T = T;
    a.ctrl = cur.dctrl.p;
    {
        const size_t table = (size_t)(kMaxBatch + 1) * a.n_obj;
        const int par = e->batch_counter & 1;
        MaskRec* base = e->arr.mrec.p;
        a.mrec = base + par * table;
        a.mrec_carry = e->prev_T > 0 ? base + (1 - par) * table + (size_t)e->prev_T * a.n_obj : a.mrec;
        a.slot_new = kSlotNew + par * kMaxBatch;
        a.slot_prev0 = (e->frame_counter + kPlaneSlots - 1) % kPlaneSlots;
    }
    a.handoff = p.handoff ? 1 : 0;
    a.skf_started = e->arr.skf_started.p;
    const long long launches0 = e->stats.launches, evops0 = e->stats.event_ops;

    TRY(enqueue_preparation(q));
    HP_MARK(e, 3, hp_t);
    TRY(enqueue_mask_frames(q));
    HP_MARK(e, 4, hp_t);
    TRY(enqueue_velocity(q));
    HP_MARK(e, 5, hp_t);
    for (int lin = 0; lin < kNumLin; ++lin) TRY(enqueue_lane(q, lin));
    TRY(enqueue_quality(q));
    HP_MARK(e, 6, hp_t);
    if (e->knobs.host_prof) {
        e->hp_batches++;
        if (e->knobs.host_prof_per_batch)
            std::fprintf(stderr, "[roft host batch %d T=%d] ctrl %.1f mask %.1f vel %.1f lanes %.1f us (cumulative)\n", e->batch_counter, T,
                         e->hp_acc[3], e->hp_acc[4], e->hp_acc[5], e->hp_acc[6]);
    }
    {
        roft_batch_trace& tr = e->trace[e->batch_counter % roft_engine::kTraceRing];
        tr = roft_batch_trace{};
        tr.batch = e->batch_counter;
        tr.frames = T;
        tr.steady = p.steady; tr.throttled = pb.throttled; tr.handoff = p.handoff;
        tr.early_lanes = (p.early_lanes ? 4 : 0) | (p.lane[0].early ? 1 : 0) | (p.lane[1].early ? 2 : 0);
        tr.outlier_parts_halved = p.outlier_div > 1 ? 1 : 0;
        tr.launches = (int)(e->stats.launches - launches0);
        tr.event_ops = (int)(e->stats.event_ops - evops0);
        tr.t_submit_us = pb.submit_t0; tr.submit_us = pb.submit_us; tr.wait_us = pb.wait_us;
    }
    HIP_TRY(hipGetLastError());
    return ROFT_OK;
}

int roft_step(roft_engine* e)
{
    if (!e) return fail(ROFT_ERR_INVALID, "null engine");
    if (!e->submitted) return fail(ROFT_ERR_STATE, "roft_frame_submit must precede roft_step");
    HIP_TRY(hipSetDevice(e->cfg.device));
    const double t_step0 = host_now_us();
    const int rc = step_batch(e);
    if (rc != ROFT_OK && e->arr.mask_general.p) {
        (void)hipMemsetAsync(e->arr.mask_general.p, 0, sizeof(unsigned) * (size_t)std::max(e->arr.a.n_obj, 1), e->stream);
        if (e->arr.mrec.p) {
            EngineArrays a2 = e->arr.a;
            a2.T = kMaxBatch;
            for (int par = 0; par < 2; ++par) {
                a2.mrec = e->arr.mrec.p + (size_t)par * (kMaxBatch + 1) * a2.n_obj;
                launch_mask_reset(a2, e->stream);
            }
        }
        (void)hipGetLastError();
    }
    {
        roft_batch_trace& tr = e->trace[e->batch_counter % roft_engine::kTraceRing];
        if (tr.batch == e->batch_counter) tr.step_us = host_now_us() - t_step0;
    }
    for (HostObject* ho : e->objs) { ho->stepped_slot = ho->s.cur_slot; ho->stepped_lane = ho->s.own[ho->s.cur_slot]; ho->stepped_flow = ho->s.flow_made; ho->stepped_depth = ho->s.depth_prev; ho->last_out_valid = false; }
    const int T = e->pending.facts.T;
    e->frame_counter += T;
    e->prev_T = T;
    e->slot_of(e->batch_counter).end_frame = e->frame_counter;
    e->batch_counter++;
    e->stats.frames += T;
    e->stats.batches++;
    e->submitted = false;
    return rc;
}

int roft_sync(roft_engine* e)
{
    if (!e) return fail(ROFT_ERR_INVALID, "null engine");
    HIP_TRY(hipSetDevice(e->cfg.device));
    const int first_open = e->completed_batches, n_open = e->batch_counter - e->completed_batches;
    if (e->multi() && n_open > 1)
        for (int b = first_open; b < e->batch_counter; ++b)
            if (int rc = wait_batch(e, b)) return rc;
    HIP_TRY(hipStreamSynchronize(e->stream));
    if (e->multi()) {
        HIP_TRY(hipStreamSynchronize(e->vel_stream));
        for (int l = 0; l < kNumLin; ++l) HIP_TRY(hipStreamSynchronize(e->pose_stream[l]));
        HIP_TRY(hipStreamSynchronize(e->up_stream));
    }
    for (int b = std::max(first_open, e->batch_counter - roft_engine::kTraceRing); b < e->batch_counter; ++b) {
        roft_batch_trace& tr = e->trace[b % roft_engine::kTraceRing];
        if (tr.batch == b && tr.t_done_us == 0.0) tr.t_done_us = host_now_us();
    }
    e->completed_batches = e->batch_counter;
    e->completed_frames = e->frame_counter;
    e->idle_mark = e->batch_counter;
    return check_dev_error(e);
}
```

roft_amd/csrc/k_mask.hip:

```cpp
#include <algorithm>
#include <initializer_list>

#include "roft_device.h"

namespace roft {

__device__ __forceinline__ void bytes_to_bits(uint32_t w, int shift, unsigned long long& nz, unsigned long long& ob)
{
#pragma unroll
    for (int k = 0; k < 4; ++k) {
        const uint32_t v = (w >> (8 * k)) & 0xFFu;
        nz |= (unsigned long long)(v != 0u) << (shift + k);
        ob |= (unsigned long long)(v > 1u) << (shift + k);
    }
}

__device__ __forceinline__ void ingest_group(const uint4* src, int g, uint2* nz, uint2* ob, int& count, int& ones)
{
    unsigned long long bnz = 0, bob = 0;
    uint4 v[4];
#pragma unroll
    for (int q = 0; q < 4; ++q) v[q] = src[(size_t)g * 4 + q];
#pragma unroll
    for (int q = 0; q < 4; ++q) {
        bytes_to_bits(v[q].x, 16 * q, bnz, bob);
        bytes_to_bits(v[q].y, 16 * q + 4, bnz, bob);
        bytes_to_bits(v[q].z, 16 * q + 8, bnz, bob);
        bytes_to_bits(v[q].w, 16 * q + 12, bnz, bob);
    }
    nz[g] = make_uint2((uint32_t)bnz, (uint32_t)(bnz >> 32));
    ob[g] = make_uint2((uint32_t)bob, (uint32_t)(bob >> 32));
    count += __popcll(bnz);
    ones += __popcll(bnz & ~bob);
}

__device__ __forceinline__ void ingest_delivered(const EngineArrays& a, const FrameCtrl& c, int t, int obj, int chunk)
{
    const int n_grp = (a.cam.W * a.cam.H) >> 6;
    const int g = chunk * blockDim.x + threadIdx.x;
    int count = 0, ones = 0;
    if (g < n_grp)
        ingest_group(reinterpret_cast<const uint4*>(c.new_mask), g,
                     reinterpret_cast<uint2*>(a.planes + plane_offset(a, obj, a.slot_new + t, 0)),
                     reinterpret_cast<uint2*>(a.planes + plane_offset(a, obj, a.slot_new + t, 1)), count, ones);
    for (int off = 32; off > 0; off >>= 1) { count += __shfl_xor(count, off, 64); ones += __shfl_xor(ones, off, 64); }
    if ((threadIdx.x & 63) == 0 && count) {
        MaskRec& r = a.mrec[(size_t)(t + 1) * a.n_obj + obj];
        atomicAdd(&r.new_count, count);
        if (ones) atomicAdd(&r.new_ones, ones);
    }
}

__global__ __launch_bounds__(256) void mask_ingest_kernel(EngineArrays a, int t)
{
    ROFT_RESIDENT(a, RK_MASK_INGEST);
    const int obj = blockIdx.y;
    const FrameCtrl& c = frame_ctrl(a, t, obj);
    if (!c.has_new_mask || c.label_type) return;
    ingest_delivered(a, c, t, obj, blockIdx.x);
}

__global__ __launch_bounds__(256) void ctrl_ingest_kernel(const uint4* __restrict__ src, EngineArrays a, size_t n16, int copy_blocks,
                                                          int chunks, unsigned frames_packed)
{
    if ((int)blockIdx.x < copy_blocks) {
        uint4* dst = reinterpret_cast<uint4*>(a.ctrl);
        const size_t stride = (size_t)copy_blocks * blockDim.x;
        for (size_t i = (size_t)blockIdx.x * blockDim.x + threadIdx.x; i < n16; i += stride) dst[i] = src[i];
        return;
    }
    ROFT_RESIDENT(a, RK_MASK_INGEST);
    const int w = (int)blockIdx.x - copy_blocks;
    const int chunk = w % chunks, rest = w / chunks, obj = rest % a.n_obj, fi = rest / a.n_obj;
    const int t = (int)((frames_packed >> (4 * fi)) & 15u);
    const FrameCtrl& c = reinterpret_cast<const FrameCtrl*>(src)[(size_t)t * a.n_obj + obj];
    if (!c.has_new_mask || c.label_type) return;
    ingest_delivered(a, c, t, obj, chunk);
}

bool launch_ctrl_ingest(const void* staging, const EngineArrays& a, size_t n16, unsigned new_mask_frames, hipStream_t s, hipEvent_t stop)
{
    unsigned packed = 0;
    int n_frames = 0;
    for (int t = 0; t < a.T && t < 16; ++t)
        if (new_mask_frames & (1u << t)) {
            if (n_frames >= 8) return false;
            packed |= (unsigned)t << (4 * n_frames++);
        }
    const int n_grp = a.cam.W * a.cam.H / 64, chunks = (n_grp + 255) / 256;
    const int copy_blocks = (int)std::min<size_t>((n16 + 255) / 256, 64);
    const unsigned grid = (unsigned)copy_blocks + (unsigned)n_frames * (unsigned)a.n_obj * (unsigned)chunks;
    hipExtLaunchKernelGGL(ctrl_ingest_kernel, dim3(grid), dim3(256), 0, s, nullptr, stop, 0, reinterpret_cast<const uint4*>(staging), a, n16,
                          copy_blocks, chunks, packed);
    return true;
}

void launch_mask_ingest(const EngineArrays& a, int t, hipStream_t s, hipEvent_t stop)
{
    const int n_grp = a.cam.W * a.cam.H / 64;
    hipExtLaunchKernelGGL(mask_ingest_kernel, dim3((n_grp + 255) / 256, a.n_obj), dim3(256), 0, s, nullptr, stop, 0, a, t);
}

__device__ __forceinline__ uint32_t eq_bits_u8(uint32_t w, uint32_t rep)
{
    const uint32_t x = w ^ rep;
    const uint32_t z = ~(((x & 0x7F7F7F7Fu) + 0x7F7F7F7Fu) | x | 0x7F7F7F7Fu);
    return ((z >> 7) * 0x01020408u) >> 24;
}
__device__ __forceinline__ uint32_t eq_bits_u16(uint32_t w, uint32_t rep)
{
    const uint32_t x = w ^ rep;
    const uint32_t z = ~(((x & 0x7FFF7FFFu) + 0x7FFF7FFFu) | x | 0x7FFF7FFFu);
    return ((z >> 15) | (z >> 30)) & 3u;
}

template <int NQ>
__device__ __forceinline__ void label_ingest_group(const LabelIngestArgs& la, const LabelSet& set, LabelMember* s_mem, int g)
{
    const bool in = g < la.n_grp;
    uint4 v[NQ];
#pragma unroll
    for (int q = 0; q < NQ; ++q) v[q] = in ? reinterpret_cast<const uint4*>(set.img)[(size_t)g * NQ + q] : make_uint4(0u, 0u, 0u, 0u);
    const size_t slot_off = (size_t)(la.slot0 + set.t) * 2 * la.plane_words;
    for (int m0 = 0; m0 < set.n; m0 += 256) {
        __syncthreads();
        if (m0 + (int)threadIdx.x < set.n) s_mem[threadIdx.x] = la.members[set.first + m0 + threadIdx.x];
        __syncthreads();
        const int n_here = min(256, set.n - m0);
        for (int m = 0; m < n_here; ++m) {
            const LabelMember mem = s_mem[m];
            if ((unsigned)mem.obj >= (unsigned)la.n_obj) continue;
            unsigned long long bits = 0ull;
            if (NQ == 4) {
                const uint32_t rep = (uint32_t)mem.label * 0x01010101u;
#pragma unroll
                for (int q = 0; q < 4; ++q) {
                    const uint32_t b = eq_bits_u8(v[q].x, rep) | (eq_bits_u8(v[q].y, rep) << 4) | (eq_bits_u8(v[q].z, rep) << 8) |
                                       (eq_bits_u8(v[q].w, rep) << 12);
                    bits |= (unsigned long long)b << (16 * q);
                }
            } else {
                const uint32_t rep = (uint32_t)mem.label * 0x00010001u;
#pragma unroll
                for (int q = 0; q < 8; ++q) {
                    const uint32_t b = eq_bits_u16(v[q].x, rep) | (eq_bits_u16(v[q].y, rep) << 2) | (eq_bits_u16(v[q].z, rep) << 4) |
                                       (eq_bits_u16(v[q].w, rep) << 6);
                    bits |= (unsigned long long)b << (8 * q);
                }
            }
            if (in) {
                uint32_t* base = la.planes + (size_t)mem.obj * la.obj_stride + slot_off;
                const uint2 w = make_uint2((uint32_t)bits, (uint32_t)(bits >> 32));
                reinterpret_cast<uint2*>(base)[g] = w;
// ... 176 lines not shown
            float t_x[NCH], t_y[NCH];
            int src[NCH];
#pragma unroll
            for (int u = 0; u < NCH; ++u) {
                t_x[u] = nan;
                t_y[u] = 0.0f;
                src[u] = 0;
                if (pending) {
                    const int it = __builtin_ctzll(pending);
                    pending &= pending - 1;
                    const uint32_t yx = (uint32_t)__builtin_amdgcn_readlane((int)my_yx, it);
                    unsigned long long bits = ((unsigned long long)(uint32_t)__builtin_amdgcn_readlane((int)mine.y, it) << 32) |
                                              (uint32_t)__builtin_amdgcn_readlane((int)mine.x, it);
                    if (clear00 && yx == 0u) bits &= ~1ull;
                    const int y0 = (int)(yx >> 16), x0 = (int)(yx & 0xFFFFu);
                    int px, py;
                    group_pixel(W, yx, lane, px, py);
                    src[u] = y0 * W + x0 + lane;
                    t_x[u] = ((bits >> lane) & 1ull) ? (float)px : nan;
                    t_y[u] = (float)py;
                }
            }
            for (int j = n_flows - 1; j >= 0; --j) {
                const ROFT_GLOBAL unsigned char* fl = uniform_global(flows[j]);
                uint2 raw[NCH];
#pragma unroll
                for (int u = 0; u < NCH; ++u) {
                    const int ix = trunc_clamped(t_x[u]), iy = trunc_clamped(t_y[u]);
                    const bool in = (unsigned)ix < (unsigned)W && (unsigned)iy < (unsigned)H;
                    t_x[u] = in ? t_x[u] : nan;
                    int fr, fc;
                    if (MODE == 2) { fr = iy; fc = ix; }
                    else if (MODE == 1) { fr = trunc_clamped(t_y[u] * g.inv_grid); fc = trunc_clamped(t_x[u] * g.inv_grid); }
                    else { fr = trunc_clamped(t_y[u] / g.grid_f); fc = trunc_clamped(t_x[u] / g.grid_f); }
                    raw[u] = flow_load<FT>(fl + (in ? (uint32_t)(fr * g.cols + fc) * kFlowElem<FT> : 0u));
                }
#pragma unroll
                for (int u = 0; u < NCH; ++u) {
                    float dx, dy;
                    flow_value<FT>(raw[u], dx, dy);
                    scale_flow<MODE>(g, dx, dy);
                    t_x[u] += dx;
                    t_y[u] += dy;
                }
            }
#pragma unroll
            for (int u = 0; u < NCH; ++u) {
                const int ix = trunc_clamped(t_x[u]), iy = trunc_clamped(t_y[u]);
                if ((unsigned)ix < (unsigned)W && (unsigned)iy < (unsigned)H) hit(iy * W + ix, ix, iy, src[u]);
            }
        }
    }
}

constexpr int kSingleWalks = 12;
template <int FT, int MODE, int NW>
__device__ __forceinline__ void walk_single(const ChaseGeo g, const uint32_t* list_, const uint2* words_, int n_list, bool clear00,
                                            const void* flow, const OrTarget tgt)
{
    constexpr int NCH = kSingleWalks;
    const ROFT_LDS uint32_t* const list = uniform_lds(list_);
    const ROFT_LDS uint32_t* const words = uniform_lds(words_);
    const int W = g.W, H = g.H;
    const int lane = threadIdx.x & 63, wave = threadIdx.x >> 6;
    const ROFT_GLOBAL unsigned char* fl = uniform_global(flow);
    for (int e0 = wave; e0 < n_list; e0 += NCH * NW) {
        uint2 raw[NCH];
#pragma unroll
        for (int u = 0; u < NCH; ++u) {
            const int e = e0 + u * NW;
            raw[u] = make_uint2(0u, 0u);
            if (e < n_list) {
                const uint32_t yx = (uint32_t)__builtin_amdgcn_readfirstlane((int)list[e]);
                int px, py, fr, fc;
                group_pixel(W, yx, lane, px, py);
                if (MODE == 2) { fr = py; fc = px; }
                else { fr = trunc_clamped((float)py * g.inv_grid); fc = trunc_clamped((float)px * g.inv_grid); }
                raw[u] = flow_load<FT>(fl + (uint32_t)(fr * g.cols + fc) * kFlowElem<FT>);
            }
        }
#pragma unroll
        for (int u = 0; u < NCH; ++u) {
            const int e = e0 + u * NW;
            if (e < n_list) {
                const uint32_t yx = (uint32_t)__builtin_amdgcn_readfirstlane((int)list[e]);
                unsigned long long bits = ((unsigned long long)(uint32_t)__builtin_amdgcn_readfirstlane((int)words[2 * e + 1]) << 32) |
                                          (uint32_t)__builtin_amdgcn_readfirstlane((int)words[2 * e]);
                if (clear00 && yx == 0u) bits &= ~1ull;
                int px, py;
                group_pixel(W, yx, lane, px, py);
                float dx, dy;
                flow_value<FT>(raw[u], dx, dy);
                scale_flow<MODE>(g, dx, dy);
                const float t_x = (float)px + dx, t_y = (float)py + dy;
                const int ix = trunc_clamped(t_x), iy = trunc_clamped(t_y);
                if (((bits >> lane) & 1ull) && (unsigned)ix < (unsigned)W && (unsigned)iy < (unsigned)H) tgt.hit(iy * W + ix);
            }
        }
    }
}

template <int FT, int MODE, int NW>
__device__ __forceinline__ void walk_single_aligned(const ChaseGeo g, const uint32_t* list_, const uint2* words_, int n_list, bool clear00,
                                                    const void* flow, const OrTarget tgt)
{
    static_assert(MODE == 1 || MODE == 2, "power-of-two grid and scale");
    constexpr int NCH = kSingleWalks;
    const ROFT_LDS uint32_t* const list = uniform_lds(list_);
    const ROFT_LDS uint32_t* const words = uniform_lds(words_);
    const int W = g.W, H = g.H;
    const int lane = threadIdx.x & 63, wave = __builtin_amdgcn_readfirstlane((int)(threadIdx.x >> 6));
    constexpr uint32_t elem = kFlowElem<FT>;
    const int sh = (MODE == 2) ? 0 : __builtin_ctz((unsigned)g.grid);
    const ROFT_GLOBAL unsigned char* const fl = uniform_global(flow);
    const uint32_t lane_off = (uint32_t)(lane >> sh) * elem;
    const uint32_t m_lo = lane < 32 ? 1u << lane : 0u, m_hi = lane < 32 ? 0u : 1u << (lane - 32);
    const float lane_f = (float)lane;
    const int my_e = wave + lane * NW;
    uint32_t my_yx = 0u, my_lo = 0u, my_hi = 0u;
    if (my_e < n_list) { my_yx = list[my_e]; my_lo = words[2 * my_e]; my_hi = words[2 * my_e + 1]; }
    const int n_mine = n_list > wave ? min(64, (n_list - wave + NW - 1) / NW) : 0;
    for (int u0 = 0; u0 < n_mine; u0 += NCH) {
        uint2 raw[NCH];
#pragma unroll
        for (int u = 0; u < NCH; ++u) {
            raw[u] = make_uint2(0u, 0u);
            if (u0 + u < n_mine) {
                const uint32_t yx = (uint32_t)__builtin_amdgcn_readlane((int)my_yx, u0 + u);
                const uint32_t y0 = yx >> 16, x0 = yx & 0xFFFFu;
                const uint32_t off = ((y0 >> sh) * (uint32_t)g.cols + (x0 >> sh)) * elem;
                raw[u] = flow_load<FT>(fl + off + lane_off);
            }
        }
#pragma unroll
        for (int u = 0; u < NCH; ++u) {
            if (u0 + u < n_mine) {
                const uint32_t yx = (uint32_t)__builtin_amdgcn_readlane((int)my_yx, u0 + u);
                uint32_t lo = (uint32_t)__builtin_amdgcn_readlane((int)my_lo, u0 + u);
                const uint32_t hi = (uint32_t)__builtin_amdgcn_readlane((int)my_hi, u0 + u);
                if (clear00 && yx == 0u) lo &= ~1u;
                const float x0f = (float)(int)(yx & 0xFFFFu), y0f = (float)(int)(yx >> 16);
                float dx, dy;
                flow_value<FT>(raw[u], dx, dy);
                scale_flow<MODE>(g, dx, dy);
                const float t_x = (x0f + lane_f) + dx, t_y = y0f + dy;
                const int ix = trunc_clamped(t_x), iy = trunc_clamped(t_y);
                if ((((lo & m_lo) | (hi & m_hi)) != 0u) && (unsigned)ix < (unsigned)W && (unsigned)iy < (unsigned)H) tgt.hit(iy * W + ix);
            }
        }
    }
}

constexpr int kBinaryWalks = 8;
template <int FT, int NW>
__device__ __forceinline__ void propagate_binary(ChaseGeo g, const uint2* plane2, const uint32_t* list, int n_list, int n_flows,
                                                 bool clear00, const void* const* flows, const OrTarget tgt, const uint2* words)
{
    if (n_flows == 1 && words && g.mode != 0) {
        if ((g.W & 63) == 0 && n_list <= 64 * NW) {
            if (g.mode == 2) walk_single_aligned<FT, 2, NW>(g, list, words, n_list, clear00, flows[0], tgt);
            else walk_single_aligned<FT, 1, NW>(g, list, words, n_list, clear00, flows[0], tgt);
        } else if (g.mode == 2) walk_single<FT, 2, NW>(g, list, words, n_list, clear00, flows[0], tgt);
        else walk_single<FT, 1, NW>(g, list, words, n_list, clear00, flows[0], tgt);
        return;
    }
    auto hit = [tgt](int tp, int, int, int) { tgt.hit(tp); };
    if (g.mode == 2) chase_groups<FT, kBinaryWalks, 2, NW>(g, plane2, list, n_list, n_flows, clear00, flows, hit, words);
    else if (g.mode == 1) chase_groups<FT, kBinaryWalks, 1, NW>(g, plane2, list, n_list, n_flows, clear00, flows, hit, words);
    else chase_groups<FT, 4, 0, NW>(g, plane2, list, n_list, n_flows, clear00, flows, hit, words);
}

template <int FT, int NW>
__device__ __noinline__ void propagate_general(ChaseGeo g, const uint2* plane2, const uint32_t* list, int n_list, int n_flows,
                                               bool clear00, const void* const* flows, int32_t* map, int* s_bbox)
{
    int bx0 = INT32_MAX, by0 = INT32_MAX, bx1 = -1, by1 = -1;
    auto hit = [map, &bx0, &by0, &bx1, &by1](int tp, int ix, int iy, int p) {
        atomicMax(&map[tp], p);
        bx0 = min(bx0, ix); bx1 = max(bx1, ix);
        by0 = min(by0, iy); by1 = max(by1, iy);
    };
    if (g.mode == 2) chase_groups<FT, 4, 2, NW>(g, plane2, list, n_list, n_flows, clear00, flows, hit);
    else if (g.mode == 1) chase_groups<FT, 4, 1, NW>(g, plane2, list, n_list, n_flows, clear00, flows, hit);
    else chase_groups<FT, 4, 0, NW>(g, plane2, list, n_list, n_flows, clear00, flows, hit);
    for (int off = 32; off > 0; off >>= 1) {
        bx0 = min(bx0, __shfl_xor(bx0, off, 64)); by0 = min(by0, __shfl_xor(by0, off, 64));
        bx1 = max(bx1, __shfl_xor(bx1, off, 64)); by1 = max(by1, __shfl_xor(by1, off, 64));
    }
    if ((threadIdx.x & 63) == 0 && bx1 >= 0) {
        atomicMin(&s_bbox[0], bx0); atomicMin(&s_bbox[1], by0);
        atomicMax(&s_bbox[2], bx1); atomicMax(&s_bbox[3], by1);
    }
}

__device__ __forceinline__ void plane_copy(uint32_t* d, const uint32_t* s, size_t n_words)
{
    if (((n_words & 3) | ((reinterpret_cast<uintptr_t>(d) | reinterpret_cast<uintptr_t>(s)) & 15)) == 0)
        for (size_t i = threadIdx.x; i < n_words / 4; i += blockDim.x) reinterpret_cast<uint4*>(d)[i] = reinterpret_cast<const uint4*>(s)[i];
    else
        for (size_t i = threadIdx.x; i < n_words / 2; i += blockDim.x) reinterpret_cast<uint2*>(d)[i] = reinterpret_cast<const uint2*>(s)[i];
}

__device__ __forceinline__ void plane_fill(uint32_t* d, uint32_t v, size_t n_words)
{
    if (((n_words & 3) | (reinterpret_cast<uintptr_t>(d) & 15)) == 0)
        for (size_t i = threadIdx.x; i < n_words / 4; i += blockDim.x) reinterpret_cast<uint4*>(d)[i] = make_uint4(v, v, v, v);
    else
        for (size_t i = threadIdx.x; i < n_words / 2; i += blockDim.x) reinterpret_cast<uint2*>(d)[i] = make_uint2(v, v);
}

__device__ __forceinline__ MaskRec decide_frame(const MaskRec& prev, const MaskRec& cur, int new_slot, const FrameCtrl& c,
                                                int frames_between, int flow_aided)
{
    MaskRec r = cur;
    const int new_count = c.has_new_mask ? r.new_count : 0;
    const int new_binary = r.new_ones == 0;
    if (flow_aided) {
        r.mode = decide_mode(c, new_slot, prev.fbuf_n, new_count, frames_between, r.src_slot, r.n_flows);
        r.fbuf_n = next_fbuf(c, prev.fbuf_n, new_count, r.mode, frames_between);
    } else {
        r.mode = 0;
        r.src_slot = c.has_new_mask ? new_slot : c.slot_prev;
        r.n_flows = 0;
        r.fbuf_n = 0;
    }
    r.src_binary = (r.src_slot >= kSlotNew) ? new_binary : prev.binary;
    r.binary = r.src_binary;
    return r;
}

#ifdef ROFT_MASK_PROFILE
#define MTICK(i) do { __syncthreads(); if (threadIdx.x == 0) atomicMax((unsigned long long*)&a.state[blockIdx.y].dbg[(i)], (unsigned long long)wall_clock64()); } while (0)
#else
#define MTICK(i) do {} while (0)
#endif

template <int FT, int THREADS>
__global__ __launch_bounds__(THREADS) __attribute__((amdgpu_waves_per_eu(4, 8)))
void mask_frame_kernel(EngineArrays a, int t, int frames_between, int flow_aided, int grp_per_wg, int margin, int win_cap)
{
#ifdef ROFT_MASK_PROFILE
    if (threadIdx.x == 0) atomicMax((unsigned long long*)&a.state[blockIdx.y].dbg[8], (unsigned long long)((1ll << 62) - wall_clock64()));
#endif
    ROFT_RESIDENT(a, THREADS == kFreshThreads ? RK_MASK_FRESH_EMPTY : RK_MASK_FRAME_EMPTY);
    extern __shared__ __attribute__((aligned(16))) unsigned char smem[];
    __shared__ MaskShared S;
    __shared__ FrameCtrl s_c;
    __shared__ MaskRec s_rec[2];
    static_assert(sizeof(MaskRec) == 32, "two 16-byte loads per record");
    uint32_t* s_win = reinterpret_cast<uint32_t*>(smem);
    uint32_t* s_list = s_win + win_cap;
    uint2* s_words = reinterpret_cast<uint2*>(s_list + THREADS);
    const int obj = blockIdx.y, q = blockIdx.x;
    const int W = a.cam.W, H = a.cam.H, wpr = a.cam.wpr, n_grp = (W * H) >> 6;
    const int tid = threadIdx.x;
    const int g0 = q * grp_per_wg, g1 = min(n_grp, g0 + grp_per_wg);
    const int r_lo = max(0, (g0 * 64) / W - margin), r_hi = min(H - 1, (g1 * 64 - 1) / W + margin);
    const int win_off = r_lo * wpr, win_words = min(win_cap, (r_hi - r_lo + 1) * wpr);
    stage_ctrl(&s_c, frame_ctrl(a, t, obj));
    if (tid >= THREADS / 2 && tid < THREADS / 2 + 4) {
        const int k = tid - THREADS / 2;
        const MaskRec* prev = (t == 0) ? a.mrec_carry + obj : a.mrec + (size_t)t * a.n_obj + obj;
        reinterpret_cast<uint4*>(s_rec)[k] = (k >= 2) ? reinterpret_cast<const uint4*>(a.mrec + (size_t)(t + 1) * a.n_obj + obj)[k & 1]
                                                      : reinterpret_cast<const uint4*>(prev)[k & 1];
    }
    const int guess_prev = a.slot_prev0 >= 0 ? (a.slot_prev0 + t) % kPlaneSlots : -1, guess_new = a.slot_new + t;
    const ROFT_GLOBAL unsigned long long* pl_prev = guess_prev >= 0 ? (const ROFT_GLOBAL unsigned long long*)(a.planes + plane_offset(a, obj, guess_prev, 1)) : nullptr;
    const ROFT_GLOBAL unsigned long long* pl_new = (const ROFT_GLOBAL unsigned long long*)(a.planes + plane_offset(a, obj, guess_new, 1));
    unsigned long long w_prev = 0ull, w_new = 0ull;
    if (g0 + tid < g1) {
        if (pl_prev) w_prev = pl_prev[g0 + tid];
        w_new = pl_new[g0 + tid];
    }
    if (tid == THREADS * 3 / 4) { S.w00[0] = pl_prev ? pl_prev[0] : 0ull; S.w00[1] = pl_new[0]; }
    for (int i = tid; i < win_words; i += THREADS) s_win[i] = 0u;
    if (tid == 0) S.n_list = 0;
    __syncthreads();
    MTICK(4);
    const FrameCtrl& c = s_c;
    const MaskRec r = decide_frame(s_rec[0], s_rec[1], a.slot_new + t, c, frames_between, flow_aided);
    if (q == 0 && tid == 0) a.mrec[(size_t)(t + 1) * a.n_obj + obj] = r;
    if (tid < kMaxFlowHist) S.flows[tid] = (tid < r.n_flows) ? c.flow[tid] : nullptr;
    MTICK(0);
    const size_t sh0 = (size_t)2 * g0, sh_n = (size_t)2 * (g1 - g0);
    plane_fill(a.planes + plane_offset(a, obj, (c.slot_cur + 1) % kPlaneSlots, 1) + sh0, 0u, sh_n);
    MTICK(5);
    const uint32_t* src = a.planes + plane_offset(a, obj, r.src_slot, 1);
    uint32_t* dst = a.planes + plane_offset(a, obj, c.slot_cur, 1);
    if (!r.src_binary) {
        if (q == 0 && tid == 0) atomicOr(&a.mask_general[obj], 1u << t);
        return;
    }
    if (r.mode == 0) {
        plane_copy(dst + sh0, src + sh0, sh_n);
        return;
    }
    const bool from_guess = r.src_slot == guess_prev || r.src_slot == guess_new;
    const unsigned long long w00 = from_guess ? S.w00[r.src_slot == guess_new ? 1 : 0] : *reinterpret_cast<const unsigned long long*>(src);
    if (r.mode == 2 && (w00 & 1ull)) {
        plane_fill(dst + sh0, ~0u, sh_n);
        return;
    }
    MTICK(6);
    const ChaseGeo geo = make_chase_geo(a.cam, a.ffmt);
    OrTarget tgt;
    tgt.win = uniform_lds(s_win);
    tgt.off = win_off;
    tgt.words = win_words;
    tgt.dst = dst;
    const uint2* plane2 = reinterpret_cast<const uint2*>(src);
    for (int c0 = g0; c0 < g1; c0 += THREADS) {
        const int g = c0 + tid;
        unsigned long long ww = 0ull;
        if (g < g1) {
            if (c0 == g0 && from_guess) ww = (r.src_slot == guess_new) ? w_new : w_prev;
            else ww = *reinterpret_cast<const unsigned long long*>(plane2 + g);
        }
        if (c0 > g0) {
            __syncthreads();
            if (tid == 0) S.n_list = 0;
            __syncthreads();
        }
        MTICK(7);
        const ListSlot slot = list_reserve(S.n_list, ww != 0ull);
        if (ww != 0ull) {
            const int e = slot.entry();
            s_list[e] = group_entry(g, W);
            s_words[e] = make_uint2((uint32_t)ww, (uint32_t)(ww >> 32));
        }
        __syncthreads();
        MTICK(1);
        if (S.n_list > 0) ROFT_RESIDENT_AS(a, THREADS == kFreshThreads ? RK_MASK_FRESH : RK_MASK_FRAME);
        propagate_binary<FT, THREADS / 64>(geo, plane2, s_list, S.n_list, r.n_flows, r.mode == 1, S.flows, tgt, s_words);
    }
    __syncthreads();
    MTICK(2);
    for (int i = tid; i < win_words; i += THREADS) {
        const uint32_t v = s_win[i];
        if (v) atomicOr(&dst[win_off + i], v);
    }
    MTICK(3);
}

constexpr int kMaskThreads = 256;
constexpr int kMaskWaves = kMaskThreads / 64;
constexpr int kGeneralList = 16384;
template <int FT>
__global__ __launch_bounds__(kMaskThreads) void mask_general_kernel(EngineArrays a, int final_launch)
{
    extern __shared__ __attribute__((aligned(16))) unsigned char smem[];
    __shared__ MaskShared S;
    uint32_t* s_list = reinterpret_cast<uint32_t*>(smem);
    const int obj = blockIdx.x;
    const int W = a.cam.W, H = a.cam.H, npix = W * H, n_grp = npix >> 6;
    const int tid = threadIdx.x, lane = tid & 63;
    ROFT_RESIDENT(a, RK_MASK_GENERAL);
    if (final_launch && tid < a.T) {
        MaskRec& r0 = a.mrec[(size_t)(tid + 1) * a.n_obj + obj];
        r0.new_count = 0;
        r0.new_ones = 0;
    }
    const unsigned todo = a.mask_general[obj];
    if (!todo) return;
    __syncthreads();
    if (tid == 0) a.mask_general[obj] = 0u;
    for (int t = 0; t < a.T; ++t) {
        if (!((todo >> t) & 1u)) continue;
        const MaskRec r = a.mrec[(size_t)(t + 1) * a.n_obj + obj];
        const FrameCtrl& c = frame_ctrl(a, t, obj);
        const uint32_t* snz = a.planes + plane_offset(a, obj, r.src_slot, 0);
        const uint32_t* sob = a.planes + plane_offset(a, obj, r.src_slot, 1);
        uint32_t* dnz = a.planes + plane_offset(a, obj, c.slot_cur, 0);
        uint32_t* dob = a.planes + plane_offset(a, obj, c.slot_cur, 1);
        if (r.mode == 0) {
            plane_copy(dnz, snz, a.plane_words);
            plane_copy(dob, sob, a.plane_words);
        } else {
            const bool bg_nz = (r.mode == 2) && (snz[0] & 1u), bg_ob = (r.mode == 2) && (sob[0] & 1u);
            if (tid < kMaxFlowHist) S.flows[tid] = (tid < r.n_flows) ? c.flow[tid] : nullptr;
            if (tid == 0) { S.n_list = 0; S.bbox[0] = INT32_MAX; S.bbox[1] = INT32_MAX; S.bbox[2] = -1; S.bbox[3] = -1; }
            __syncthreads();
            const uint2* plane2 = reinterpret_cast<const uint2*>(snz);
            int32_t* map = a.map + (size_t)obj * npix;
            for (int c0 = 0; c0 < n_grp; c0 += kGeneralList) {
                const int c1 = min(n_grp, c0 + kGeneralList);
                for (int g0 = c0; g0 < c1; g0 += kMaskThreads) {
                    const int g = g0 + tid;
                    bool ne = false;
                    if (g < c1) { const uint2 w = plane2[g]; ne = (w.x | w.y) != 0u; }
                    const ListSlot slot = list_reserve(S.n_list, ne);
                    if (ne) { const uint32_t yx = group_entry(g, W); s_list[slot.entry()] = yx; }
                }
                __syncthreads();
                propagate_general<FT, kMaskWaves>(make_chase_geo(a.cam, a.ffmt), plane2, s_list, S.n_list, r.n_flows, r.mode == 1, S.flows, map, S.bbox);
                __syncthreads();
                if (tid == 0) S.n_list = 0;
                __syncthreads();
            }
            const int bx0 = S.bbox[0], by0 = S.bbox[1], bx1 = S.bbox[2], by1 = S.bbox[3];
            const int wave = tid >> 6;
            for (int g = wave; g < n_grp; g += kMaskWaves) {
                const int p = g * 64 + lane;
                const int y = p / W, x = p - y * W;
                bool nzb = bg_nz, obb = bg_ob;
                if (y >= by0 && y <= by1 && x >= bx0 && x <= bx1) {
                    const int m = atomicExch(&map[p], 0);
                    if (m != 0) {
                        nzb = (snz[m >> 5] >> (m & 31)) & 1u;
                        obb = (sob[m >> 5] >> (m & 31)) & 1u;
                    }
                }
                const unsigned long long b1 = __ballot(nzb), b2 = __ballot(obb);
                if (lane == 0) {
                    reinterpret_cast<uint2*>(dnz)[g] = make_uint2((uint32_t)b1, (uint32_t)(b1 >> 32));
                    reinterpret_cast<uint2*>(dob)[g] = make_uint2((uint32_t)b2, (uint32_t)(b2 >> 32));
                }
            }
        }
        __syncthreads();
    }
}

int launch_mask_chain(const EngineArrays& a, int frames_between, int flow_aided, unsigned new_mask_frames, hipStream_t s, hipEvent_t stop,
                      hipEvent_t stop_early)
{
    const int n_grp = a.cam.W * a.cam.H / 64;
    constexpr int kBandRows = 20, kBandRowsFresh = 6;
    auto per_for = [&](bool fresh) {
        if (a.mask_wgs > 0) return (n_grp + a.mask_wgs - 1) / a.mask_wgs;
        const int per = std::max(1, (fresh ? kBandRowsFresh : kBandRows) * a.cam.W / 64);
        return std::min(per, n_grp);
    };
    const size_t lds_cap = 160 * 1024 - 4096;
    auto frame_kernel = [](bool s16, int threads) {
        if (threads == kFrameThreads) return s16 ? mask_frame_kernel<ROFT_FLOW_S16C2, kFrameThreads> : mask_frame_kernel<ROFT_FLOW_F32C2, kFrameThreads>;
        return s16 ? mask_frame_kernel<ROFT_FLOW_S16C2, kFreshThreads> : mask_frame_kernel<ROFT_FLOW_F32C2, kFreshThreads>;
    };
    auto general_kernel = [](bool s16) { return s16 ? mask_general_kernel<ROFT_FLOW_S16C2> : mask_general_kernel<ROFT_FLOW_F32C2>; };
    for (int threads : {kFrameThreads, kFreshThreads})
        for (bool f16 : {true, false}) (void)set_max_dynamic_lds(reinterpret_cast<const void*>(frame_kernel(f16, threads)), (int)lds_cap);
    int launches = 0;
    const bool s16 = a.ffmt.type == ROFT_FLOW_S16C2;
    auto launch_general = [&](hipEvent_t ev, int final_launch) {
        const size_t lds_gen = ((size_t)std::min(n_grp, kGeneralList) * 4 + 15) & ~(size_t)15;
        for (bool f16 : {true, false}) (void)set_max_dynamic_lds(reinterpret_cast<const void*>(general_kernel(f16)), kGeneralList * 4 + 16);
        hipExtLaunchKernelGGL(general_kernel(s16), dim3(a.n_obj), dim3(kMaskThreads), (uint32_t)lds_gen, s, nullptr, ev, 0, a, final_launch);
    };
    for (int t = 0; t < a.T; ++t) {
        const bool fresh = (new_mask_frames >> t) & 1u;
        const int per = per_for(fresh);
        constexpr int kMargin = 16, kMarginFresh = 48;
        const int margin = fresh ? kMarginFresh : kMargin;
        const int threads = fresh ? kFreshThreads : kFrameThreads;
        const size_t fixed = (size_t)threads * 12;
        size_t win_cap = ((size_t)std::min(a.cam.H, (per * 64 + a.cam.W - 1) / a.cam.W + 1 + 2 * margin) * a.cam.wpr + 1) & ~(size_t)1;
        win_cap = std::min(win_cap, ((lds_cap - fixed) / 4) & ~(size_t)1);
        const size_t lds = win_cap * 4 + fixed;
        const dim3 grid((n_grp + per - 1) / per, a.n_obj);
        hipLaunchKernelGGL(frame_kernel(s16, threads), grid, dim3(threads), (uint32_t)lds, s, a, t, frames_between, flow_aided, per, margin, (int)win_cap);
        ++launches;
        if (stop_early && t == a.T - 2) { launch_general(stop_early, 0); ++launches; }
    }
    launch_general(stop, 1);
    return launches + 1;
}

__global__ __launch_bounds__(256) void plane_to_mask_kernel(const uint32_t* nz, const uint32_t* ob, int npix,
                                                            uint8_t* mask)
{
    const int p = blockIdx.x * blockDim.x + threadIdx.x;
    if (p >= npix) return;
    const bool o = (ob[p >> 5] >> (p & 31)) & 1u;
    const bool n = nz ? ((nz[p >> 5] >> (p & 31)) & 1u) : false;
    mask[p] = o ? 255 : (n ? 1 : 0);
}

void launch_planes_to_mask(const uint32_t* nz, const uint32_t* ob, int npix, uint8_t* mask, hipStream_t s)
{
    hipLaunchKernelGGL(plane_to_mask_kernel, dim3((npix + 255) / 256), dim3(256), 0, s, nz, ob, npix, mask);
}

}
```

roft_amd/csrc/k_render.hip:

```cpp
#include <algorithm>
#include <atomic>
#include <string>

#include "mesh_clusters.h"
#include "plane_rank.h"
#include "raster.h"

namespace roft {

namespace host { int fail(int code, const std::string& msg); }

constexpr int kFeatThreads = 1024;

#ifdef ROFT_FEAT_PROFILE
#define FTICK(i) do { __syncthreads(); if (threadIdx.x == 0) { long long _t = wall_clock64(); a.state[obj].dbg[i] = _t - f_t0; f_t0 = _t; } } while (0)
#else
#define FTICK(i) do {} while (0)
#endif

template <bool LDS>
__global__ __launch_bounds__(kFeatThreads) void features_kernel(EngineArrays a, unsigned frames_packed)
{
    ROFT_RESIDENT(a, RK_FEATURES);
    extern __shared__ __attribute__((aligned(16))) unsigned char smem[];
    __shared__ int s_wave[16];
    __shared__ int s_chunk[kFeatThreads];
    const int obj = blockIdx.x;
    const FrameCtrl& c = frame_ctrl(a, (int)((frames_packed >> (4 * blockIdx.y)) & 15u), obj);
#ifdef ROFT_FEAT_PROFILE
    long long f_t0 = wall_clock64();
#endif
    int feat_write = c.feat_write, slot_cur = c.slot_cur;
    const float* depth = c.depth_cur;
    asm volatile("" : "+v"(feat_write), "+v"(slot_cur), "+v"(depth));
    if (feat_write < 0) return;
    const int W = a.cam.W, wpr = a.cam.wpr;
    const uint32_t* gplane = a.planes + plane_offset(a, obj, slot_cur, 1);
    uint32_t* s_stage = reinterpret_cast<uint32_t*>(smem);
    if (LDS) {
        const size_t n4 = a.plane_words / 4;
        for (size_t i = threadIdx.x; i < n4; i += blockDim.x)
            reinterpret_cast<uint4*>(s_stage)[i] = reinterpret_cast<const uint4*>(gplane)[i];
        for (size_t i = n4 * 4 + threadIdx.x; i < a.plane_words; i += blockDim.x) s_stage[i] = gplane[i];
        __syncthreads();
    }
    const uint32_t* s_plane = LDS ? s_stage : gplane;
    FTICK(0);
    uint32_t* fpix = a.feat_pix + ((size_t)obj * kFeatRing + feat_write) * a.feat_cap;
    float* fdep = a.feat_depth + ((size_t)obj * kFeatRing + feat_write) * a.feat_cap;
    const int n_words = (int)a.plane_words;
    const int per = (n_words + blockDim.x - 1) / blockDim.x;
    const int w0 = min(n_words, (int)threadIdx.x * per), w1 = min(n_words, w0 + per);
    int cnt = 0;
    for (int w = w0; w < w1; ++w) cnt += __popc(s_plane[w]);
    int total;
    s_chunk[threadIdx.x] = block_exclusive_scan(cnt, s_wave, &total);
    __syncthreads();
    FTICK(1);
    for (int w = threadIdx.x; w < n_words; w += blockDim.x) {
        uint32_t bits = s_plane[w];
        if (!bits) continue;
        const int chunk = w / per;
        int r0 = s_chunk[chunk];
        for (int v = chunk * per; v < w; ++v) r0 += __popc(s_plane[v]);
        if (r0 & 1) bits &= bits - 1;
        int slot = (r0 + 1) >> 1;
        const int row = w / wpr;
        const uint32_t pix0 = ((uint32_t)row << 16) | (uint32_t)((w - row * wpr) * 32);
        while (bits) {
            if (slot < a.feat_cap) fpix[slot] = pix0 + (uint32_t)__builtin_ctz(bits);
            ++slot;
            bits &= bits - 1;
            bits &= bits - 1;
        }
    }
    __syncthreads();
    FTICK(2);
    constexpr int kBatch = 16;
    const int n = min((total + 1) / 2, a.feat_cap);
    for (int sb = threadIdx.x; sb < n; sb += kBatch * blockDim.x) {
        uint32_t px[kBatch];
        float d[kBatch];
#pragma unroll
        for (int u = 0; u < kBatch; ++u) {
            const int sl = sb + u * (int)blockDim.x;
            px[u] = (sl < n) ? fpix[sl] : 0u;
        }
#pragma unroll
        for (int u = 0; u < kBatch; ++u) d[u] = depth[(size_t)(px[u] >> 16) * W + (px[u] & 0xFFFFu)];
#pragma unroll
        for (int u = 0; u < kBatch; ++u) {
            const int sl = sb + u * (int)blockDim.x;
            if (sl < n) fdep[sl] = d[u];
        }
    }
    FTICK(3);
    if (threadIdx.x == 0) a.state[obj].n_feat[feat_write] = n;
}

void launch_features(const EngineArrays& a, hipStream_t s, hipEvent_t stop, unsigned feat_frames)
{
    unsigned packed = 0;
    int n_frames = 0;
    for (int t = 0; t < a.T && t < 8; ++t)
        if (feat_frames == 0 || (feat_frames & (1u << t))) packed |= (unsigned)t << (4 * n_frames++);
    if (n_frames == 0) n_frames = 1;
    const size_t lds = (a.plane_words * 4 + 15) & ~(size_t)15;
    const size_t lds_cap = 160 * 1024 - 256 - kFeatThreads * sizeof(int) - 128;
    if (lds <= lds_cap) {
        (void)set_max_dynamic_lds(reinterpret_cast<const void*>(features_kernel<true>), (int)lds_cap);
        hipExtLaunchKernelGGL(features_kernel<true>, dim3(a.n_obj, n_frames), dim3(kFeatThreads), (uint32_t)lds, s, nullptr, stop, 0, a, packed);
    } else {
        hipExtLaunchKernelGGL(features_kernel<false>, dim3(a.n_obj, n_frames), dim3(kFeatThreads), 0, s, nullptr, stop, 0, a, packed);
    }
}


constexpr float kGlNear = 0.001f, kGlFar = 1000.0f;
constexpr uint32_t kGlDepthClear = 0xFFFFFFu;
constexpr uint64_t kGlKeyClear = ((uint64_t)kGlDepthClear << 32) | 0xFFFFFFFFu;

__device__ __forceinline__ void project_vertex_gl(const float* v, const RenderPose& P, float fx, float fy, float cx,
                                                  float cy, float& sx, float& sy, float& z)
{
    const float X = ((P.R[0] * v[0] + P.R[1] * v[1]) + P.R[2] * v[2]) + P.t[0];
    const float Y = ((P.R[3] * v[0] + P.R[4] * v[1]) + P.R[5] * v[2]) + P.t[1];
    z = ((P.R[6] * v[0] + P.R[7] * v[1]) + P.R[8] * v[2]) + P.t[2];
    if (z > 0.001f) {
        sx = (fx * X) / z + cx;
        sy = (fy * Y) / z + cy;
    } else {
        sx = sy = 0.0f;
    }
}

__device__ __forceinline__ float gl_vertex_window_z(float Z)
{
    const float gl_a = (kGlFar + kGlNear) / (kGlFar - kGlNear), gl_b = (2.0f * (kGlFar * kGlNear)) / (kGlFar - kGlNear);
    const float z_ndc = (gl_a * Z - gl_b) / Z;
    return 0.5f * z_ndc + 0.5f;
}

__device__ __forceinline__ float gl_pixel_window_z(float x0, float y0, float x1, float y1, float x2, float y2, float zw0, float zw1,
                                                   float zw2, float px, float py)
{
    const double dw0 = ((double)x2 - x1) * ((double)py - y1) - ((double)y2 - y1) * ((double)px - x1);
    const double dw1 = ((double)x0 - x2) * ((double)py - y2) - ((double)y0 - y2) * ((double)px - x2);
    const double dw2 = ((double)x1 - x0) * ((double)py - y0) - ((double)y1 - y0) * ((double)px - x0);
    return (float)((dw0 * zw0 + dw1 * zw1 + dw2 * zw2) / (dw0 + dw1 + dw2));
}

__device__ __forceinline__ float gl_linear_depth(float z_w)
{
    const float zn = z_w * 2.0f - 1.0f;
    return (2.0f * kGlNear * kGlFar) / (kGlFar + kGlNear - zn * (kGlFar - kGlNear));
}

template <class Store>
__device__ __forceinline__ void raster_projected_gl(float x0, float y0, float z0, float x1, float y1, float z1, float x2, float y2,
                                                    float z2, int w, int h, int j_lo, int j_hi, Store store)
{
    if (!(z0 > 0.001f && z1 > 0.001f && z2 > 0.001f)) return;
    const float area = (x1 - x0) * (y2 - y0) - (x2 - x0) * (y1 - y0);
    if (area == 0.0f || !(area == area)) return;
    const float minx = fminf(x0, fminf(x1, x2)), maxx = fmaxf(x0, fmaxf(x1, x2));
    const float miny = fminf(y0, fminf(y1, y2)), maxy = fmaxf(y0, fmaxf(y1, y2));
    float fi0 = ceilf(minx - 0.5f), fi1 = floorf(maxx - 0.5f);
    float fj0 = ceilf(miny - 0.5f), fj1 = floorf(maxy - 0.5f);
    if (fi0 < 0.0f) fi0 = 0.0f;
    if (fj0 < 0.0f) fj0 = 0.0f;
    if (fi1 > (float)(w - 1)) fi1 = (float)(w - 1);
    if (fj1 > (float)(h - 1)) fj1 = (float)(h - 1);
    if (!(fi0 <= fi1) || !(fj0 <= fj1)) return;
    const int ia = (int)fi0, ib = (int)fi1, ja = max((int)fj0, j_lo), jb = min((int)fj1, j_hi);
    if (jb < ja) return;
    const float sgn = (area > 0.0f) ? 1.0f : -1.0f;
    const float ea0 = -sgn * (y2 - y1), ea1 = -sgn * (y0 - y2), ea2 = -sgn * (y1 - y0);
    const float eb0 = sgn * (x2 - x1), eb1 = sgn * (x0 - x2), eb2 = sgn * (x1 - x0);
    const bool own0 = (ea0 > 0.0f) || (ea0 == 0.0f && eb0 > 0.0f);
    const bool own1 = (ea1 > 0.0f) || (ea1 == 0.0f && eb1 > 0.0f);
    const bool own2 = (ea2 > 0.0f) || (ea2 == 0.0f && eb2 > 0.0f);
    const float zw0 = gl_vertex_window_z(z0), zw1 = gl_vertex_window_z(z1), zw2 = gl_vertex_window_z(z2);
    for (int j = ja; j <= jb; ++j) {
        const float py = (float)j + 0.5f;
        for (int i = ia; i <= ib; ++i) {
            const float px = (float)i + 0.5f;
            const float w0 = (x2 - x1) * (py - y1) - (y2 - y1) * (px - x1);
            const float w1 = (x0 - x2) * (py - y2) - (y0 - y2) * (px - x2);
            const float w2 = (x1 - x0) * (py - y0) - (y1 - y0) * (px - x0);
            const bool inside = (area > 0.0f) ? (w0 >= 0.0f && w1 >= 0.0f && w2 >= 0.0f)
                                              : (w0 <= 0.0f && w1 <= 0.0f && w2 <= 0.0f);
            if (!inside) continue;
            if ((w0 == 0.0f && !own0) || (w1 == 0.0f && !own1) || (w2 == 0.0f && !own2)) continue;
            const float z_w = gl_pixel_window_z(x0, y0, x1, y1, x2, y2, zw0, zw1, zw2, px, py);
            if (!(z_w >= 0.0f && z_w <= 1.0f)) continue;
            const uint32_t qz = (uint32_t)floor((double)z_w * 16777215.0 + 0.5);
            if (qz >= kGlDepthClear) continue;
            store(i, j, qz);
        }
    }
}

constexpr int kOutlierThreads = 1024;

__global__ __launch_bounds__(kOutlierThreads) void outlier_kernel(EngineArrays a, int lin)
{
    __shared__ double s_err[2][kOutlierThreads / 64];
    __shared__ double s_cnt[2][kOutlierThreads / 64];
    __shared__ int s_sel;
    const int obj = blockIdx.x;
    ObjState& st = a.state[obj];
    PoseLane& pl = st.lane[lin];
    if (pl.pending_frame < 0) return;
    const FrameCtrl& c = frame_ctrl(a, pl.pending_frame, obj);
    const int d = a.cam.divider, tw = a.tile_w;
    const int fslot = (c.feat_read >= 0) ? c.feat_read : 0;
    const uint32_t* fpix = a.feat_pix + ((size_t)obj * kFeatRing + fslot) * a.feat_cap;
    const float* fdep = a.feat_depth + ((size_t)obj * kFeatRing + fslot) * a.feat_cap;
    const uint32_t* z0 = a.zbuf + (((size_t)lin * a.n_obj + obj) * 2) * a.tile_w * a.tile_h;
    const uint32_t* z1 = z0 + (size_t)a.tile_w * a.tile_h;
    double err[2] = {0.0, 0.0}, cnt[2] = {0.0, 0.0};
    const int n = st.n_feat[fslot];
    constexpr int kBatch = 16;
    for (int i0 = threadIdx.x; i0 < n; i0 += kBatch * blockDim.x) {
        float dep[kBatch];
        uint32_t pix[kBatch];
#pragma unroll
        for (int k = 0; k < kBatch; ++k) {
            const int i = i0 + k * blockDim.x;
            dep[k] = (i < n) ? fdep[i] : 0.0f;
            pix[k] = (i < n) ? fpix[i] : 0u;
        }
        uint32_t b0[kBatch], b1[kBatch];
#pragma unroll
        for (int k = 0; k < kBatch; ++k) {
            const int v = (int)(pix[k] >> 16), u = (int)(pix[k] & 0xFFFFu);
            const size_t ti = (size_t)(v / d) * tw + (u / d);
            b0[k] = z0[ti];
            b1[k] = z1[ti];
        }
#pragma unroll
        for (int k = 0; k < kBatch; ++k) {
            if (!((dep[k] > 0) && ((double)dep[k] < 2.0))) continue;
            if (b0[k] != kDepthEmpty) { err[0] += (double)fabsf(dep[k] - __uint_as_float(b0[k])); cnt[0] += 1.0; }
            if (b1[k] != kDepthEmpty) { err[1] += (double)fabsf(dep[k] - __uint_as_float(b1[k])); cnt[1] += 1.0; }
        }
    }
    for (int k = 0; k < 2; ++k) {
        double e = err[k], n2 = cnt[k];
        for (int off = 32; off > 0; off >>= 1) { e += __shfl_down(e, off, 64); n2 += __shfl_down(n2, off, 64); }
        if ((threadIdx.x & 63) == 0) { s_err[k][threadIdx.x >> 6] = e; s_cnt[k][threadIdx.x >> 6] = n2; }
    }
    __syncthreads();
    if (threadIdx.x == 0) {
        double L[2];
        for (int k = 0; k < 2; ++k) {
            double e = 0.0, n2 = 0.0;
            for (int w = 0; w < kOutlierThreads / 64; ++w) { e += s_err[k][w]; n2 += s_cnt[k][w]; }
            L[k] = (n2 == 0.0) ? 1.7976931348623157e308 : (e / n2) / 1.0;
        }
        const int sel = (L[0] > 2.0 * L[1]) ? 1 : 0;
        pl.outlier_selected = sel;
        pl.outlier_L[0] = L[0];
        pl.outlier_L[1] = L[1];
        for (int k = 0; k < 2; ++k) {
            double n2 = 0.0;
            for (int w = 0; w < kOutlierThreads / 64; ++w) n2 += s_cnt[k][w];
            pl.outlier_cnt[k] = n2;
        }
        s_sel = sel;
    }
    __syncthreads();
    const PoseBelief& src = st.belief[b_alt(lin, s_sel ? 1 : 0)];
    PoseBelief& dst = st.belief[c.cur_slot];
    for (int i = threadIdx.x; i < 144; i += blockDim.x) dst.cov[i] = src.cov[i];
    if (threadIdx.x < 13) dst.mean[threadIdx.x] = src.mean[threadIdx.x];
    if (roft_object_output* row = log_row(a, c, obj)) {
        if (threadIdx.x < 13) row->pose[threadIdx.x] = src.mean[threadIdx.x];
        if (threadIdx.x == 0) {
            row->outlier_selected = s_sel;
            row->outlier_L[0] = pl.outlier_L[0];
            row->outlier_L[1] = pl.outlier_L[1];
        }
    }
}

constexpr int kFusedThreads = 1024;
#ifdef ROFT_FUSED_PROFILE
#define UTICK(i) do { __syncthreads(); if (threadIdx.x == 0 && bx < 4) { long long _t = wall_clock64(); st.dbg[bx * 8 + (i)] += _t - u_t0; u_t0 = _t; } } while (0)
#else
#define UTICK(i) do {} while (0)
#endif

template <bool GL>
__global__ __launch_bounds__(kFusedThreads) void outlier_fused_kernel(EngineArrays a, int lin, int vcache_cap, int win_cap, int parts,
                                                                     int split_tris, float* tile_dump)
{
    ROFT_RESIDENT(a, RK_OUTLIER);
    extern __shared__ __attribute__((aligned(16))) unsigned char smem[];
    __shared__ long long s_hi[kFusedThreads / 64], s_lo[kFusedThreads / 64];
    __shared__ int s_cnt[kFusedThreads / 64];
    __shared__ int s_box[4];
    __shared__ int s_behind;
    __shared__ int s_last;
    __shared__ int s_settled;
    const int per = 2 * parts, lin_id = (int)blockIdx.x;
    const int obj = (lin_id / (8 * per)) * 8 + (lin_id & 7), bx = (lin_id >> 3) % per;
    if (obj >= a.n_obj) return;
    const int alt = bx / parts, part = bx % parts, tid = threadIdx.x;
    ObjState& st = a.state[obj];
    PoseLane& pl = st.lane[lin];
    if (pl.pending_frame < 0) return;
    const FrameCtrl& c = frame_ctrl(a, pl.pending_frame, obj);
    const ObjParams& prm = a.params[obj];
    const PoseBelief& bl = st.belief[b_alt(lin, alt)];
    const RenderPose P = make_pose(bl.mean + 6, bl.mean + 9);
    const int d = a.cam.divider, tw = a.tile_w, th = a.tile_h;
    const float fx = (float)(a.cam.fx / d), fy = (float)(a.cam.fy / d), cx = (float)(a.cam.cx / d), cy = (float)(a.cam.cy / d);
    const int nv = prm.n_verts, nt = prm.n_tris;
    const bool cached = GL && nv <= vcache_cap;
    float* s_v = reinterpret_cast<float*>(smem);
    uint32_t* s_z = reinterpret_cast<uint32_t*>(smem + (GL ? vertex_cache_bytes(vcache_cap) : 0));
    uint64_t* s_k = reinterpret_cast<uint64_t*>(s_z);
    if (tid < 4) s_box[tid] = (tid < 2) ? INT32_MAX : -1;
    if (tid == 0) s_behind = 0;
#ifdef ROFT_FUSED_PROFILE
    long long u_t0 = wall_clock64();
    if (tid < 8 && bx < 4) st.dbg[bx * 8 + tid] = 0;
#endif
    __syncthreads();
    auto project = [&](const float* v, float& sx, float& sy, float& z) {
        if constexpr (GL) project_vertex_gl(v, P, fx, fy, cx, cy, sx, sy, z);
        else project_vertex(v, P, fx, fy, cx, cy, sx, sy, z);
    };
    if constexpr (GL) {
        project_mesh<kFusedThreads, 4>(prm.verts, nv, cached, s_v, tw, th, s_box, &s_behind, project);
        __syncthreads();
    } else {
        if (tid < 64 && prm.n_clusters > 0) {
            const int k = tid & 7;
            const float vc[3] = {prm.box_corners[3 * k], prm.box_corners[3 * k + 1], prm.box_corners[3 * k + 2]};
            int box[4];
            const bool settled = corner_box_settles(vc, P, fx, fy, cx, cy, tw, th, box);
            if (tid == 0) {
                s_settled = settled ? 1 : 0;
                if (settled) { s_box[0] = box[0]; s_box[1] = box[1]; s_box[2] = box[2]; s_box[3] = box[3]; }
            }
        } else if (tid == 0) {
            s_settled = 1;
        }
        __syncthreads();
        if (!s_settled) {
            project_mesh<kFusedThreads, 4>(prm.verts, nv, false, s_v, tw, th, s_box, &s_behind, project);
            __syncthreads();
        }
    }
    UTICK(0);
    const int i0 = min(s_box[0], tw - 1), i1 = s_box[2];
    int j0 = min(s_box[1], th - 1), j1 = s_box[3];
    int R = parts;
    if (!GL && split_tris && parts > 1 && i1 >= i0 && j1 >= j0 && i0 >= 0 && j0 >= 0) {
        const long long w_all = i1 - i0 + 1, rows_all = j1 - j0 + 1;
        for (R = 1; R < parts; ++R)
            if (parts % R == 0 && ((rows_all + R - 1) / R) * w_all <= (long long)win_cap) break;
    }
    const int G = parts / R, band = part / G, grp = part % G;
    const bool split = G > 1;
    if (j1 >= j0 && R > 1) {
        const int rows_all = j1 - j0 + 1, b0 = j0 + (int)((long long)rows_all * band / R), b1 = j0 + (int)((long long)rows_all * (band + 1) / R) - 1;
        j0 = b0;
        j1 = b1;
    }
    const int win_w = i1 - i0 + 1;
    const int fslot = (c.feat_read >= 0) ? c.feat_read : 0;
    const uint32_t* fpix = a.feat_pix + ((size_t)obj * kFeatRing + fslot) * a.feat_cap;
    const float* fdep = a.feat_depth + ((size_t)obj * kFeatRing + fslot) * a.feat_cap;
    const int n = st.n_feat[fslot];
    LikelihoodSum err;
    int cnt = 0;
    auto gl_resolve = [&](uint64_t key, int i, int j) -> float {
        const int32_t* tri = prm.tris + (size_t)3 * (uint32_t)key;
        const int v0 = tri[0], v1 = tri[1], v2 = tri[2];
        float x0, y0, z0, x1, y1, z1, x2, y2, z2;
        fetch_triangle(s_v, cached, prm.verts, v0, v1, v2, project, x0, y0, z0, x1, y1, z1, x2, y2, z2);
        return gl_linear_depth(gl_pixel_window_z(x0, y0, x1, y1, x2, y2, gl_vertex_window_z(z0), gl_vertex_window_z(z1),
                                                 gl_vertex_window_z(z2), (float)i + 0.5f, (float)j + 0.5f));
    };
    if (win_w > 0 && j1 >= j0 && i0 >= 0 && j0 >= 0) {
        const int rows = max(1, win_cap / win_w);
        for (int js = j0; js <= j1; js += rows) {
            const int je = min(j1, js + rows - 1), npx = win_w * (je - js + 1);
            if constexpr (GL) {
                for (int i = tid; i < npx; i += kFusedThreads) s_k[i] = kGlKeyClear;
            } else {
                for (int i = tid; i < npx; i += kFusedThreads) s_z[i] = kDepthEmpty;
            }
            __syncthreads();
            UTICK(1);
            ROFT_LDS uint32_t* const zw = pin_lds(s_z);
            auto store = [zw, i0, js, win_w](int i, int j, float z) {
                (void)__hip_atomic_fetch_min(zw + ((j - js) * win_w + (i - i0)), __float_as_uint(z), __ATOMIC_RELAXED, __HIP_MEMORY_SCOPE_WORKGROUP);
            };
            ROFT_LDS uint64_t* const zk = (ROFT_LDS uint64_t*)zw;
            auto store_key = [zk, i0, js, win_w](int i, int j, uint64_t key) {
                (void)__hip_atomic_fetch_min(zk + ((j - js) * win_w + (i - i0)), key, __ATOMIC_RELAXED, __HIP_MEMORY_SCOPE_WORKGROUP);
            };
            if constexpr (GL) {
                constexpr int kTB = 8;
                for (int tb = tid; tb < nt; tb += kTB * kFusedThreads) {
                    int idx[kTB][3];
#pragma unroll
                    for (int k = 0; k < kTB; ++k) {
                        const int32_t* tri = prm.tris + (size_t)3 * min(tb + k * kFusedThreads, nt - 1);
                        idx[k][0] = tri[0]; idx[k][1] = tri[1]; idx[k][2] = tri[2];
                    }
#pragma unroll
                    for (int k = 0; k < kTB; ++k) {
                        if (tb + k * kFusedThreads >= nt) break;
                        float x0, y0, z0, x1, y1, z1, x2, y2, z2;
                        fetch_triangle(s_v, cached, prm.verts, idx[k][0], idx[k][1], idx[k][2], project, x0, y0, z0, x1, y1, z1, x2, y2, z2);
                        const uint64_t t = (uint32_t)(tb + k * kFusedThreads);
                        raster_projected_gl(x0, y0, z0, x1, y1, z1, x2, y2, z2, tw, th, js, je,
                                            [&](int i, int j, uint32_t qz) { store_key(i, j, ((uint64_t)qz << 32) | t); });
                    }
                }
            } else {
                const bool rule_on = cull_table(prm.tri_flip, s_behind) != nullptr;
                const bool cones = rule_on && fx > 0.0f && fy > 0.0f && pose_is_rotation(P.R);
                const float f_lo = fminf(fx, fy), f_hi = fmaxf(fx, fy), c_abs = fabsf(cx) + fabsf(cy);
                const int lane = tid & 63, wave = __builtin_amdgcn_readfirstlane(tid >> 6);
                const int nc = prm.n_clusters, n_waves = kFusedThreads / 64;
                auto cluster_of = [=](int i) { return (i * n_waves + wave) * G + grp; };
                auto fetch = [&](int c, float (&v)[3], uint32_t& w) {
                    const float* sl = prm.cl_slots + (size_t)c * 3 * kClusterSize + lane;
                    v[0] = sl[0]; v[1] = sl[kClusterSize]; v[2] = sl[2 * kClusterSize];
                    w = prm.cl_words[(size_t)c * kClusterSize + lane];
                };
                for (int base = 0; cluster_of(base) < nc; base += 64) {
                    const int mine = cluster_of(base + lane);
                    bool live = mine < nc;
                    if (live && cones) {
                        const uint4* hp = reinterpret_cast<const uint4*>(prm.cl_headers + (size_t)mine * kClusterWords);
                        const uint4 h0 = hp[0], h1 = hp[1], h2 = hp[2], h3 = hp[3];
                        static_assert(kCwCone == 2 && kCwAxis == 4 && kCwCos == 7 && kCwSin == 8 && kCwCenter == 9 && kCwRadius == 12 &&
                                      kCwAreaMin == 13 && kCwEdgeMax == 14, "the header words as they are unpacked here");
                        if (h0.z && cluster_faces_away(__uint_as_float(h1.x), __uint_as_float(h1.y), __uint_as_float(h1.z), __uint_as_float(h1.w),
                                                       __uint_as_float(h2.x), __uint_as_float(h2.y), __uint_as_float(h2.z), __uint_as_float(h2.w),
                                                       __uint_as_float(h3.x), __uint_as_float(h3.y), __uint_as_float(h3.z), P.R, P.t, f_lo, f_hi, c_abs))
                            live = false;
                    }
                    unsigned long long todo = __ballot(live);
                    if (!todo) continue;
                    float v[3];
                    uint32_t w;
                    fetch(cluster_of(base + (int)__builtin_ctzll(todo)), v, w);
                    while (todo) {
                        todo &= todo - 1;
                        float v_n[3] = {v[0], v[1], v[2]};
                        uint32_t w_n = w;
                        if (todo) fetch(cluster_of(base + (int)__builtin_ctzll(todo)), v_n, w_n);
                        float sx, sy, z;
                        project_vertex(v, P, fx, fy, cx, cy, sx, sy, z);
                        const int a0 = (int)(w & 63u), a1 = (int)((w >> 6) & 63u), a2 = (int)((w >> 12) & 63u);
                        const float x0 = __shfl(sx, a0, 64), y0 = __shfl(sy, a0, 64), z0 = __shfl(z, a0, 64);
                        const float x1 = __shfl(sx, a1, 64), y1 = __shfl(sy, a1, 64), z1 = __shfl(z, a1, 64);
                        const float x2 = __shfl(sx, a2, 64), y2 = __shfl(sy, a2, 64), z2 = __shfl(z, a2, 64);
                        raster_projected(x0, y0, z0, x1, y1, z1, x2, y2, z2, tw, th, js, je, rule_on ? 1 + (int)((w >> 18) & 1u) : 0, store);
                        v[0] = v_n[0]; v[1] = v_n[1]; v[2] = v_n[2];
                        w = w_n;
                    }
                }
            }
            __syncthreads();
            UTICK(2);
            if constexpr (!GL) if (split) {
                const size_t slab0 = (((size_t)lin * a.zmerge_slabs + (size_t)obj * parts + (size_t)band * G) * 2 + alt) * a.zmerge_stride;
                uint32_t* mine = a.zmerge + slab0 + (size_t)grp * 2 * a.zmerge_stride;
                int* arrivals = a.zcount + (((size_t)lin * a.n_obj + obj) * 2 + alt) * kMaxOutlierParts + band;
                for (int i = tid; i < npx; i += kFusedThreads)
                    __hip_atomic_store(&mine[i], s_z[i], __ATOMIC_RELAXED, __HIP_MEMORY_SCOPE_AGENT);
                __atomic_signal_fence(__ATOMIC_SEQ_CST);
                __builtin_amdgcn_s_waitcnt(0);
                __atomic_signal_fence(__ATOMIC_SEQ_CST);
                __syncthreads();
                if (tid == 0) {
                    const int before = __hip_atomic_fetch_add(arrivals, 1, __ATOMIC_RELAXED, __HIP_MEMORY_SCOPE_AGENT);
                    s_last = (before == G - 1) ? 1 : 0;
                    if (before == G - 1) __hip_atomic_store(arrivals, 0, __ATOMIC_RELAXED, __HIP_MEMORY_SCOPE_AGENT);
                }
                __syncthreads();
                if (!s_last) return;
                static_assert(kMaxOutlierParts <= 8, "eight slabs per pixel");
                const uint32_t* others = a.zmerge + slab0;
                const size_t slab_step = 2 * a.zmerge_stride;
                const uint32_t* op[7];
                {
                    int k = 0;
#pragma unroll
                    for (int p = 0; p < 8; ++p)
                        if (p < G && p != grp && k < 7) op[k++] = others + (size_t)p * slab_step;
                    for (; k < 7; ++k) op[k] = others;
                }
                for (int i = tid; i < npx; i += kFusedThreads) {
                    uint32_t m = s_z[i];
                    uint32_t v0, v1, v2, v3, v4, v5, v6;
                    switch (G - 1) {
                    case 1:
                        asm volatile("global_load_dword %0, %1, off sc1\n\ts_waitcnt vmcnt(0)" : "=&v"(v0) : "v"(op[0] + i) : "memory");
                        m = min(m, v0);
                        break;
                    case 2:
                        asm volatile("global_load_dword %0, %2, off sc1\n\tglobal_load_dword %1, %3, off sc1\n\ts_waitcnt vmcnt(0)"
                                     : "=&v"(v0), "=&v"(v1) : "v"(op[0] + i), "v"(op[1] + i) : "memory");
                        m = min(m, min(v0, v1));
                        break;
                    case 3:
                        asm volatile("global_load_dword %0, %3, off sc1\n\tglobal_load_dword %1, %4, off sc1\n\tglobal_load_dword %2, %5, off sc1\n\t"
                                     "s_waitcnt vmcnt(0)"
                                     : "=&v"(v0), "=&v"(v1), "=&v"(v2) : "v"(op[0] + i), "v"(op[1] + i), "v"(op[2] + i) : "memory");
                        m = min(min(m, v0), min(v1, v2));
                        break;
                    case 4:
                        asm volatile("global_load_dword %0, %4, off sc1\n\tglobal_load_dword %1, %5, off sc1\n\tglobal_load_dword %2, %6, off sc1\n\t"
                                     "global_load_dword %3, %7, off sc1\n\ts_waitcnt vmcnt(0)"
                                     : "=&v"(v0), "=&v"(v1), "=&v"(v2), "=&v"(v3) : "v"(op[0] + i), "v"(op[1] + i), "v"(op[2] + i), "v"(op[3] + i) : "memory");
                        m = min(m, min(min(v0, v1), min(v2, v3)));
                        break;
                    default:
                        asm volatile("global_load_dword %0, %7, off sc1\n\tglobal_load_dword %1, %8, off sc1\n\tglobal_load_dword %2, %9, off sc1\n\t"
                                     "global_load_dword %3, %10, off sc1\n\tglobal_load_dword %4, %11, off sc1\n\tglobal_load_dword %5, %12, off sc1\n\t"
                                     "global_load_dword %6, %13, off sc1\n\ts_waitcnt vmcnt(0)"
                                     : "=&v"(v0), "=&v"(v1), "=&v"(v2), "=&v"(v3), "=&v"(v4), "=&v"(v5), "=&v"(v6)
                                     : "v"(op[0] + i), "v"(op[1] + i), "v"(op[2] + i), "v"(op[3] + i), "v"(op[4] + i), "v"(op[5] + i), "v"(op[6] + i) : "memory");
                        m = min(min(m, v0), min(min(v1, v2), min(min(v3, v4), min(v5, v6))));
                        break;
                    case 0: break;
                    }
                    s_z[i] = m;
                }
                __syncthreads();
            }
            if (tile_dump) {
                float* tile = tile_dump + (size_t)alt * tw * th;
                if constexpr (GL) {
                    for (int i = tid; i < npx; i += kFusedThreads) {
                        const uint64_t key = s_k[i];
                        const int pi = i0 + i % win_w, pj = js + i / win_w;
                        tile[(size_t)pj * tw + pi] = ((uint32_t)(key >> 32) == kGlDepthClear) ? 0.0f : gl_resolve(key, pi, pj);
                    }
                } else {
                    for (int i = tid; i < npx; i += kFusedThreads) {
                        const uint32_t b = s_z[i];
                        tile[(size_t)(js + i / win_w) * tw + (i0 + i % win_w)] = (b == kDepthEmpty) ? 0.0f : __uint_as_float(b);
                    }
                }
            }
            constexpr int kBatch = 16;
            for (int f0 = tid; f0 < n; f0 += kBatch * kFusedThreads) {
                float dep[kBatch];
                uint32_t pix[kBatch];
#pragma unroll
                for (int k = 0; k < kBatch; ++k) {
                    const int i = f0 + k * kFusedThreads;
                    dep[k] = (i < n) ? fdep[i] : 0.0f;
                    pix[k] = (i < n) ? fpix[i] : 0u;
                }
#pragma unroll
                for (int k = 0; k < kBatch; ++k) {
                    if (!((dep[k] > 0) && ((double)dep[k] < 2.0))) continue;
                    const int v = (int)(pix[k] >> 16), u = (int)(pix[k] & 0xFFFFu);
                    const int tj = v / d, ti = u / d;
                    if (tj < js || tj > je || ti < i0 || ti > i1) continue;
                    if constexpr (GL) {
                        const uint64_t key = s_k[(tj - js) * win_w + (ti - i0)];
                        if ((uint32_t)(key >> 32) != kGlDepthClear) { err.add(fabsf(dep[k] - gl_resolve(key, ti, tj))); cnt += 1; }
                    } else {
                        const uint32_t b = s_z[(tj - js) * win_w + (ti - i0)];
                        if (b != kDepthEmpty) { err.add(fabsf(dep[k] - __uint_as_float(b))); cnt += 1; }
                    }
                }
            }
            __syncthreads();
            UTICK(3);
#ifdef ROFT_FUSED_PROFILE
            if (tid == 0 && bx < 4) st.dbg[bx * 8 + 4] += 1;
            if (tid == 0 && bx < 4) st.dbg[bx * 8 + 5] = (long long)win_w * 100 ;
            if (tid == 0 && bx < 4) st.dbg[bx * 8 + 6] = (long long)(j1 - j0 + 1) * 100;
#endif
        }
    }
    for (int off = 32; off > 0; off >>= 1) {
        err.hi += __shfl_down(err.hi, off, 64);
        err.lo += __shfl_down(err.lo, off, 64);
        cnt += __shfl_down(cnt, off, 64);
    }
    if ((tid & 63) == 0) { s_hi[tid >> 6] = err.hi; s_lo[tid >> 6] = err.lo; s_cnt[tid >> 6] = cnt; }
    __syncthreads();
    if (tid == 0) {
        long long hi = 0, lo = 0;
        int n2 = 0;
        for (int w = 0; w < kFusedThreads / 64; ++w) { hi += s_hi[w]; lo += s_lo[w]; n2 += s_cnt[w]; }
        pl.part_hi[alt][band] = hi;
        pl.part_lo[alt][band] = lo;
        pl.part_cnt[alt][band] = (double)n2;
        if (band == 0) pl.n_parts[alt] = R;
    }
}

static std::atomic<int> g_outlier_split{-1};
void set_outlier_split(int mode) { g_outlier_split.store(mode < 0 ? -1 : (mode ? 1 : 0), std::memory_order_relaxed); }

int launch_outlier(const EngineArrays& a, int lin, hipStream_t s, hipEvent_t stop, const OutlierLaunchOpts* opts)
{
    if (!(opts && opts->render_mode == ROFT_RENDER_GL) && a.meshes_without_clusters > 0)
        return host::fail(ROFT_ERR_STATE, "outlier test: a mesh went up without clusters (MeshLayout::kWalkClusters)");
    const size_t lds_total = kRasterLdsBudget;
    const size_t vbytes = vertex_cache_bytes(a.max_verts);
    const bool gl = opts && opts->render_mode == ROFT_RENDER_GL;
    const size_t zb = gl ? 8 : 4;
    const size_t min_win = zb * std::max(8192, a.tile_w);
    const bool cache = gl && vbytes + min_win <= lds_total && !(opts && opts->no_vertex_cache);
    const int vcache_cap = cache ? a.max_verts : 0;
    int win_cap = (int)((lds_total - (cache ? vbytes : 0)) / zb);
    (void)set_max_dynamic_lds(gl ? reinterpret_cast<const void*>(outlier_fused_kernel<true>) : reinterpret_cast<const void*>(outlier_fused_kernel<false>),
                              (int)lds_total);
    int parts = std::max(1, std::min(kMaxOutlierParts, device_cu_count() / (2 * std::max(a.n_obj, 1))));
    if (a.outlier_parts > 0) parts = std::min(a.outlier_parts, kMaxOutlierParts);
    if (opts && opts->parts > 0) parts = std::min(opts->parts, kMaxOutlierParts);
    if (opts && opts->parts < 0) parts = std::max(1, parts / -opts->parts);
    static const int split_env = getenv("ROFT_OUTLIER_SPLIT") ? atoi(getenv("ROFT_OUTLIER_SPLIT")) : -1;
    const int forced = g_outlier_split.load(std::memory_order_relaxed) >= 0 ? g_outlier_split.load(std::memory_order_relaxed) : split_env;
    int split = (opts && opts->split >= 0) ? opts->split : (forced >= 0 ? forced : 1);
    if (parts <= 1 || !a.zmerge || (size_t)a.n_obj * parts > a.zmerge_slabs) split = 0;
    if (gl) split = 0;
    const int lds_parts = split ? 1 : parts;
    const size_t win_need = zb * std::max((size_t)a.tile_w, ((size_t)a.tile_w * a.tile_h + lds_parts - 1) / lds_parts + (size_t)a.tile_w);
    const size_t lds = std::min(lds_total, (((cache ? vbytes : 0) + win_need + 15) & ~(size_t)15));
    win_cap = std::min(win_cap, (int)((lds - (cache ? vbytes : 0)) / zb));
    if (opts && opts->window_pixels > 0) win_cap = std::max(a.tile_w, std::min(win_cap, opts->window_pixels));
    if (gl)
        hipExtLaunchKernelGGL(outlier_fused_kernel<true>, dim3(2 * parts * ((a.n_obj + 7) / 8) * 8), dim3(kFusedThreads), (uint32_t)lds, s, nullptr, stop, 0, a,
                              lin, vcache_cap, win_cap, parts, split, opts ? opts->tile_dump : nullptr);
    else
        hipExtLaunchKernelGGL(outlier_fused_kernel<false>, dim3(2 * parts * ((a.n_obj + 7) / 8) * 8), dim3(kFusedThreads), (uint32_t)lds, s, nullptr, stop, 0, a,
                              lin, vcache_cap, win_cap, parts, split, opts ? opts->tile_dump : nullptr);
    return ROFT_OK;
}

void launch_outlier_only(const EngineArrays& a, hipStream_t s)
{
    hipLaunchKernelGGL(outlier_kernel, dim3(a.n_obj), dim3(kOutlierThreads), 0, s, a, 0);
}

}
```

roft_amd/csrc/roft_device.h:

```cpp
#pragma once

#include <hip/hip_runtime.h>
#include <hip/hip_ext.h>
#include <stdint.h>

#include "../../include/roft_engine.h"

namespace roft {

constexpr int kWave = 64;
constexpr int kNumLin = 2;
constexpr int kNumBelief = 9;
constexpr int kMaxBatch = ROFT_MAX_BATCH_FRAMES;
constexpr int kTwistRing = 64;
constexpr int kMaxFlowHist = ROFT_MAX_FLOW_CHASE;
constexpr int kMaxOutlierParts = 8;
constexpr int kMaxSteps = 10;
constexpr int kPlaneSlots = 64;
constexpr int kFeatRing = 12;

enum BeliefSlot { B_LIN0 = 0, B_LIN1 = 1, B_PRED = 2 , B_ALT0 = 4 , B_ALT1 = 5 ,
                  B_SPARE = 8, B_CORR = B_LIN0  };
__host__ __device__ inline int b_alt(int lane, int k) { return B_ALT0 + 2 * lane + k; }

// ... 184 lines not shown
struct ResidencyTimer {
    unsigned long long* p;
    long long t0;
    __device__ ResidencyTimer(unsigned long long* base, int kid) : p(base ? base + 2 * kid : nullptr), t0(wall_clock64()) {}
    __device__ ~ResidencyTimer()
    {
        if (p && threadIdx.x == 0) { atomicAdd(p, (unsigned long long)(wall_clock64() - t0)); atomicAdd(p + 1, 1ull); }
    }
    __device__ void rekind(unsigned long long* base, int kid) { if (base) p = base + 2 * kid; }
};
#define ROFT_RESIDENT(a, kid) ResidencyTimer roft_resident_timer_((a).residency, (kid))
#define ROFT_RESIDENT_AS(a, kid) roft_resident_timer_.rekind((a).residency, (kid))
#else
#define ROFT_RESIDENT(a, kid) do {} while (0)
#define ROFT_RESIDENT_AS(a, kid) do {} while (0)
#endif

constexpr int ROFT_DEV_ERROR_TWIST_WAIT = 2;
constexpr int ROFT_DEV_ERROR_MASK_BARRIER = 1;

#define ROFT_LDS __attribute__((address_space(3)))

__device__ __forceinline__ ROFT_LDS uint32_t* pin_lds(uint32_t* p)
{
    uint32_t off = (uint32_t)(uintptr_t)(ROFT_LDS uint32_t*)p;
    asm volatile("" : "+s"(off));
    return (ROFT_LDS uint32_t*)(uintptr_t)off;
}

__device__ inline void stage_ctrl(FrameCtrl* s_c, const FrameCtrl& g)
{
    constexpr int n16 = (int)(sizeof(FrameCtrl) / 16);
    for (int i = threadIdx.x; i < n16; i += blockDim.x)
        reinterpret_cast<uint4*>(s_c)[i] = reinterpret_cast<const uint4*>(&g)[i];
}

__device__ inline const FrameCtrl& frame_ctrl(const EngineArrays& a, int t, int obj)
{
    return a.ctrl[(size_t)t * a.n_obj + obj];
}

__device__ inline roft_object_output* log_row(const EngineArrays& a, const FrameCtrl& c, int obj)
{
    if (!a.out_log) return nullptr;
    return a.out_log + (size_t)(c.frame_idx % a.log_cap) * a.n_obj + obj;
}

constexpr int kSlotNew = kPlaneSlots;
constexpr int kPlaneSlotsTotal = kPlaneSlots + 2 * kMaxBatch;

__device__ inline int decide_mode(const FrameCtrl& c, int new_slot, int fbuf_n, int new_count, int frames_between,
                                  int& src_slot, int& n_flows)
{
    const int n_avail = fbuf_n + (c.flow_valid ? 1 : 0);
    int mode;
    if (c.force_mode == 3) {
        src_slot = new_slot;
        n_flows = n_avail;
        mode = 2;
    } else if (c.has_new_mask && !c.first_mask && new_count > 0) {
        src_slot = new_slot;
        if (c.stamped && c.n_region <= 0) {
            n_flows = 1;
            return c.flow_valid ? 1 : 0;
        }
        n_flows = c.stamped ? c.n_region : n_avail;
        mode = 2;
    } else {
        src_slot = (c.has_new_mask && c.first_mask) ? new_slot : c.slot_prev;
        n_flows = 1;
        return c.flow_valid ? 1 : 0;
    }
    if (frames_between > 0 && n_flows > frames_between) n_flows = frames_between;
    if (n_flows > c.n_hist) n_flows = c.n_hist;
    return mode;
}

__device__ inline int next_fbuf(const FrameCtrl& c, int fbuf_n, int new_count, int mode, int frames_between)
{
    if (c.has_new_mask && !c.first_mask && new_count == 0 && frames_between <= 0) fbuf_n = 0;
    int n = fbuf_n + (c.flow_valid ? 1 : 0);
    if (n > kMaxFlowHist) n = kMaxFlowHist;
    return (mode == 2) ? 0 : n;
}

__host__ __device__ inline size_t plane_offset(const EngineArrays& a, int obj, int slot, int which)
{
    return (((size_t)obj * kPlaneSlotsTotal + slot) * 2 + which) * a.plane_words;
}

void launch_mask_ingest(const EngineArrays& a, int t, hipStream_t s, hipEvent_t stop = nullptr);
bool launch_ctrl_ingest(const void* staging, const EngineArrays& a, size_t n16, unsigned new_mask_frames, hipStream_t s, hipEvent_t stop = nullptr);
struct alignas(16) LabelSet {
    const void* img;
    int type;
    int t;
    int first, n;
};
struct LabelMember { int obj, label; };
struct LabelIngestArgs {
    const LabelSet* sets;
    const LabelMember* members;
    uint32_t* planes;
    size_t obj_stride, plane_words;
    int slot0;
    MaskRec* mrec;
    int n_obj, n_grp;
};
void launch_label_ingest(const LabelIngestArgs& la, int n_sets, hipStream_t s, hipEvent_t stop = nullptr);
constexpr int kMaskFromPose = 3;
constexpr int kSilhouetteCacheVerts = 8192;
constexpr int kSilhouetteWindowWords = 8192;
struct SilhouettePair {
    int box0, box1;
    int raw;
    int kept;
    int done;
    int front, behind;
};
struct SilhouetteArgs {
    const FrameCtrl* ctrl;
    const ObjParams* params;
    uint32_t* planes;
    size_t obj_stride, plane_words;
    int slot0;
    MaskRec* mrec;
    int n_obj;
    int W, H, wpr;
    float fx, fy, cx, cy;
    unsigned frames_packed;
    int vcache_cap;
    int win_rows;
    unsigned long long* zbuf;
    int n_zscenes;
    SilhouettePair* zpairs;
    unsigned long long* zstats;
    int gate;
    float gate_tf, gate_tb;
    unsigned long long* gstats;
    int* gremoved;
};
int launch_pose_silhouette(SilhouetteArgs sa, int n_frames, int max_verts, int bands, int vertex_cache, hipStream_t s,
                            hipEvent_t start = nullptr, hipEvent_t stop = nullptr);
void launch_mask_reset(const EngineArrays& a, hipStream_t s);
__device__ inline void mask_reset_tables(const EngineArrays& a, size_t i)
{
    if (i < (size_t)a.T * a.n_obj) {
        MaskRec& r = a.mrec[(size_t)a.n_obj + i];
        r.new_count = 0;
        r.new_ones = 0;
    }
}
int launch_mask_chain(const EngineArrays& a, int frames_between, int flow_aided, unsigned new_mask_frames, hipStream_t s, hipEvent_t stop = nullptr,
                      hipEvent_t stop_early = nullptr);
void launch_planes_to_mask(const uint32_t* nz, const uint32_t* ob, int npix, uint8_t* mask, hipStream_t s);
void launch_flow_measure(const EngineArrays& a, double depth_max, int radius, hipStream_t s,
                         hipEvent_t start = nullptr, hipEvent_t stop = nullptr);
void launch_skf_chain(const EngineArrays& a, int reweight, hipStream_t s, hipEvent_t stop = nullptr);
void launch_skf_arrays(const double* x_pred, const double* P_pred, int N, const double* y, const double* H,
                       const double* Rdiag, int reweight, double* norms, double* x_out, double* P_out, int* status,
                       hipStream_t s);
void launch_skf_records(const double* x_pred, const double* P_pred, int N, const FlowRec* recs, DevCamera cam, double dt,
                        const double* Rdiag, int reweight, double* norms, double* x_out, double* P_out, int* status,
                        hipStream_t s);
void launch_kf_predict(const double* x, const double* P, const double* qdiag, double* xo, double* Po, hipStream_t s);
void launch_ukf_chain(const EngineArrays& a, roft_ut_params ut, bool first_segment, int lin, hipStream_t s, hipEvent_t stop = nullptr);
void launch_features(const EngineArrays& a, hipStream_t s, hipEvent_t stop = nullptr, unsigned feat_frames = 0);
struct OutlierLaunchOpts {
    int parts = 0;
    int no_vertex_cache = 0;
    int window_pixels = 0;
    float* tile_dump = nullptr;
    int split = -1;
    int render_mode = ROFT_RENDER_CONTRACT;
};
int launch_outlier(const EngineArrays& a, int lin, hipStream_t s, hipEvent_t stop = nullptr, const OutlierLaunchOpts* opts = nullptr);
void set_outlier_split(int mode);
void launch_outlier_only(const EngineArrays& a, hipStream_t s);

int device_cu_count();
hipError_t set_max_dynamic_lds(const void* func, int bytes);

void launch_expand_yh(const FlowRec* recs, const int* n, DevCamera cam, double dt, int32_t* uv, double* y,
                      double* H, int cap, hipStream_t s);

constexpr int kCandBatch = 8;
struct PoseView {
    const double* base;
    long stride;
    int first, ring;
};
int pose_error_padded_points(int P);
int pose_error_waves(int P);
void launch_float_to_double(const float* in, int n, double* out, hipStream_t s);
void launch_pose_errors(int kind, const double* pts, int P, const PoseView& est, const PoseView& ref, int f0, int n, double* cloud,
                        double* partial, double* out, bool fma, hipStream_t s);

}
```

Before: 1.778 million object-frames/s.

## Add half-size outlier kernel and single-walk mask kernel when CUs are not spare

Templates the fused outlier raster kernel on thread count and adds a 512-thread variant with a smaller LDS window. The plan selects it when there are no spare CUs and bands per alternative is zero, so more workgroups can be resident per CU. It also adds a single-walk variant of the mask frame kernel with a higher waves-per-EU hint, selected under the same condition. The zmerge slab buffer is sized to the full CU count, and debug and env overrides for both choices are added. The smaller LDS window may mean more raster passes per tile, and fewer walks per thread may lower per-thread throughput.

```diff
diff --git a/include/roft_engine.h b/include/roft_engine.h
--- a/include/roft_engine.h
+++ b/include/roft_engine.h
@@ -229,6 +229,7 @@
     int frames;
     int steady, throttled, handoff, early_lanes, outlier_parts_halved;
     int launches, event_ops;
+    int outlier_shape;
     double t_submit_us;
     double submit_us;
     double wait_us;
@@ -416,6 +417,8 @@
 int roft_debug_sector_rate(int device, double* sectors_per_second);
 int roft_debug_get_residency(roft_engine* e, unsigned long long out[32]);
 int roft_debug_outlier_split(int mode);
+int roft_debug_outlier_shape(int threads, int parts_scale);
+int roft_debug_mask_kernel(int mode);
 int roft_debug_pose_errors_kernel_ms(double* ms_out);
 int roft_debug_scene_kernel_ms(roft_scene_renderer* r, double ms_out[2]);
 int roft_debug_depth_kernel_ms(roft_engine* e, double* ms_out);
diff --git a/roft_amd/_lib.py b/roft_amd/_lib.py
--- a/roft_amd/_lib.py
+++ b/roft_amd/_lib.py
@@ -164,7 +164,7 @@
     _c_name_ = "roft_batch_trace"
     _fields_ = [("batch", C.c_int), ("frames", C.c_int), ("steady", C.c_int), ("throttled", C.c_int), ("handoff", C.c_int),
                 ("early_lanes", C.c_int), ("outlier_parts_halved", C.c_int), ("launches", C.c_int), ("event_ops", C.c_int),
-                ("t_submit_us", C.c_double), ("submit_us", C.c_double), ("wait_us", C.c_double), ("step_us", C.c_double),
+                ("outlier_shape", C.c_int), ("t_submit_us", C.c_double), ("submit_us", C.c_double), ("wait_us", C.c_double), ("step_us", C.c_double),
                 ("t_done_us", C.c_double)]
 
 
@@ -285,6 +285,8 @@
     Fn("roft_debug_sector_rate", _int, [_int, _dp], _OPTIONAL),
     Fn("roft_debug_get_residency", _int, [_vp, _P(C.c_ulonglong)], _OPTIONAL),
     Fn("roft_debug_outlier_split", _int, [_int], _OPTIONAL),
+    Fn("roft_debug_outlier_shape", _int, [_int, _int], _OPTIONAL),
+    Fn("roft_debug_mask_kernel", _int, [_int], _OPTIONAL),
     Fn("roft_debug_pose_errors_kernel_ms", _int, [_dp], _OPTIONAL),
     Fn("roft_debug_scene_kernel_ms", _int, [_vp, _dp], _OPTIONAL),
     Fn("roft_debug_depth_kernel_ms", _int, [_vp, _dp], _OPTIONAL),
diff --git a/roft_amd/csrc/batch_plan.h b/roft_amd/csrc/batch_plan.h
--- a/roft_amd/csrc/batch_plan.h
+++ b/roft_amd/csrc/batch_plan.h
@@ -115,6 +115,7 @@
     Signal ev_ctrl = Signal::none, ev_prep = Signal::none;
     bool part_gate = false;
     Signal ev_mask = Signal::none;
+    bool mask_single_flow = false;
     FeatRun feat = FeatRun::none;
     Signal ev_feat = Signal::none;
     VelWait vel_waits = VelWait::none;
@@ -122,6 +123,8 @@
     Signal ev_skf = Signal::none, ev_vel = Signal::none;
     LanePlan lane[kPlanLanes];
     int outlier_div = 1;
+    int outlier_threads = 1024;
+    int outlier_parts_scale = 1;
     bool quality = false;
     bool quality_waits_mask = false;
     bool quality_waits_lane = false;
@@ -168,6 +171,7 @@
 
     p.part_gate = batch && by_mode(k.part_mode, !p.steady, cus_to_spare);
     p.ev_mask = ends(multi);
+    p.mask_single_flow = !cus_to_spare;
 
     const bool feat_behind_skf = batch && !(k.feat_mask_mode == 2 || (k.feat_mask_mode == 1 && 16 * in.n_obj <= in.cus));
     p.feat = !in.any_feat ? FeatRun::none : feat_behind_skf ? FeatRun::behind_skf : FeatRun::mask_stream;
@@ -206,6 +210,8 @@
     p.ev_quality = ends(p.quality);
 
     p.outlier_div = (in.outlier_bands_per_alternative == 0 && p.steady && k.outlier_steady_div > 1) ? k.outlier_steady_div : 1;
+    p.outlier_threads = (in.outlier_bands_per_alternative == 0 && !cus_to_spare) ? 512 : 1024;
+    p.outlier_parts_scale = 1;
     return p;
 }
 
diff --git a/roft_amd/csrc/engine_debug.hip b/roft_amd/csrc/engine_debug.hip
--- a/roft_amd/csrc/engine_debug.hip
+++ b/roft_amd/csrc/engine_debug.hip
@@ -16,6 +16,17 @@
 extern "C" int roft_debug_outlier_split(int mode)
 {
     roft::set_outlier_split(mode);
+    return ROFT_OK;
+}
+
+extern "C" int roft_debug_outlier_shape(int threads, int parts_scale)
+{
+    return roft::set_outlier_shape(threads, parts_scale) ? ROFT_OK : fail(ROFT_ERR_INVALID, "outlier shape: threads 512 | 1024 | -1, parts_scale 1 | 2 | -1");
+}
+
+extern "C" int roft_debug_mask_kernel(int mode)
+{
+    roft::set_mask_kernel(mode < 0 ? -1 : mode);
     return ROFT_OK;
 }
 
diff --git a/roft_amd/csrc/engine_internal.h b/roft_amd/csrc/engine_internal.h
--- a/roft_amd/csrc/engine_internal.h
+++ b/roft_amd/csrc/engine_internal.h
@@ -187,7 +187,7 @@
     DevBuf<int> zcount;
     int ensure_zmerge(int n, size_t tpix)
     {
-        const size_t slabs = std::max<size_t>((size_t)n, std::min<size_t>((size_t)n * kMaxOutlierParts, (size_t)std::max(device_cu_count() / 2, 1)));
+        const size_t slabs = std::max<size_t>((size_t)n, std::min<size_t>((size_t)n * kMaxOutlierParts, (size_t)std::max(device_cu_count(), 1)));
         const size_t need = (size_t)kNumLin * slabs * 2 * tpix;
         if (need > zmerge.n || !zmerge.p || tpix != a.zmerge_stride || slabs != a.zmerge_slabs) {
             HIP_TRY(zmerge.ensure(need));
diff --git a/roft_amd/csrc/engine_step.hip b/roft_amd/csrc/engine_step.hip
--- a/roft_amd/csrc/engine_step.hip
+++ b/roft_amd/csrc/engine_step.hip
@@ -191,7 +191,7 @@
     hipStream_t s = e->stream;
     tmark(e, nullptr, 0);
     q.launches += launch_mask_chain(q.a, e->cfg.mask_frames_between, e->cfg.flow_aided_segmentation, e->pending.new_mask_frames, s,
-                                    Enqueue::stop(p.ev_mask, q.cur.ev_mask), p.part_gate ? q.cur.ev_part : nullptr);
+                                    Enqueue::stop(p.ev_mask, q.cur.ev_mask), p.part_gate ? q.cur.ev_part : nullptr, p.mask_single_flow);
     CHECK_LAUNCH("mask chain");
     tmark(e, "mask_chain", 0);
     TRY(q.signalled(p.ev_mask, q.cur.ev_mask, s));
@@ -272,6 +272,8 @@
     OutlierLaunchOpts oo;
     oo.render_mode = e->cfg.render_mode;
     if (q.p.outlier_div > 1) oo.parts = -q.p.outlier_div;
+    oo.threads = q.p.outlier_threads;
+    oo.parts_scale = q.p.outlier_parts_scale;
     const int n_seg = facts.n_segments[lin];
     for (int seg = 0; seg < n_seg; ++seg) {
         const bool last = seg == n_seg - 1;
@@ -383,6 +385,7 @@
         tr.steady = p.steady; tr.throttled = pb.throttled; tr.handoff = p.handoff;
         tr.early_lanes = (p.early_lanes ? 4 : 0) | (p.lane[0].early ? 1 : 0) | (p.lane[1].early ? 2 : 0);
         tr.outlier_parts_halved = p.outlier_div > 1 ? 1 : 0;
+        tr.outlier_shape = p.outlier_threads == 512 ? p.outlier_parts_scale : 0;
         tr.launches = (int)(e->stats.launches - launches0);
         tr.event_ops = (int)(e->stats.event_ops - evops0);
         tr.t_submit_us = pb.submit_t0; tr.submit_us = pb.submit_us; tr.wait_us = pb.wait_us;
diff --git a/roft_amd/csrc/k_mask.hip b/roft_amd/csrc/k_mask.hip
--- a/roft_amd/csrc/k_mask.hip
+++ b/roft_amd/csrc/k_mask.hip
@@ -1,4 +1,6 @@
 #include <algorithm>
+#include <atomic>
+#include <cstdlib>
 #include <initializer_list>
 
 #include "roft_device.h"
@@ -481,7 +483,7 @@
 }
 
 constexpr int kBinaryWalks = 8;
-template <int FT, int NW>
+template <int FT, int NW, bool SINGLE = false>
 __device__ __forceinline__ void propagate_binary(ChaseGeo g, const uint2* plane2, const uint32_t* list, int n_list, int n_flows,
                                                  bool clear00, const void* const* flows, const OrTarget tgt, const uint2* words)
 {
@@ -494,9 +496,10 @@
         return;
     }
     auto hit = [tgt](int tp, int, int, int) { tgt.hit(tp); };
-    if (g.mode == 2) chase_groups<FT, kBinaryWalks, 2, NW>(g, plane2, list, n_list, n_flows, clear00, flows, hit, words);
-    else if (g.mode == 1) chase_groups<FT, kBinaryWalks, 1, NW>(g, plane2, list, n_list, n_flows, clear00, flows, hit, words);
-    else chase_groups<FT, 4, 0, NW>(g, plane2, list, n_list, n_flows, clear00, flows, hit, words);
+    constexpr int kWalks = SINGLE ? 1 : kBinaryWalks, kWalksDiv = SINGLE ? 1 : 4;
+    if (g.mode == 2) chase_groups<FT, kWalks, 2, NW>(g, plane2, list, n_list, n_flows, clear00, flows, hit, words);
+    else if (g.mode == 1) chase_groups<FT, kWalks, 1, NW>(g, plane2, list, n_list, n_flows, clear00, flows, hit, words);
+    else chase_groups<FT, kWalksDiv, 0, NW>(g, plane2, list, n_list, n_flows, clear00, flows, hit, words);
 }
 
 template <int FT, int NW>
@@ -564,8 +567,8 @@
 #define MTICK(i) do {} while (0)
 #endif
 
-template <int FT, int THREADS>
-__global__ __launch_bounds__(THREADS) __attribute__((amdgpu_waves_per_eu(4, 8)))
+template <int FT, int THREADS, bool SINGLE = false>
+__global__ __launch_bounds__(THREADS) __attribute__((amdgpu_waves_per_eu(SINGLE ? 7 : 4, 8)))
 void mask_frame_kernel(EngineArrays a, int t, int frames_between, int flow_aided, int grp_per_wg, int margin, int win_cap)
 {
 #ifdef ROFT_MASK_PROFILE
@@ -660,7 +663,7 @@
         __syncthreads();
         MTICK(1);
         if (S.n_list > 0) ROFT_RESIDENT_AS(a, THREADS == kFreshThreads ? RK_MASK_FRESH : RK_MASK_FRAME);
-        propagate_binary<FT, THREADS / 64>(geo, plane2, s_list, S.n_list, r.n_flows, r.mode == 1, S.flows, tgt, s_words);
+        propagate_binary<FT, THREADS / 64, SINGLE>(geo, plane2, s_list, S.n_list, r.n_flows, r.mode == 1, S.flows, tgt, s_words);
     }
     __syncthreads();
     MTICK(2);
@@ -750,8 +753,11 @@
     }
 }
 
+static std::atomic<int> g_mask_kernel{-1};
+void set_mask_kernel(int mode) { g_mask_kernel.store(mode < 0 ? -1 : (mode ? 1 : 0), std::memory_order_relaxed); }
+
 int launch_mask_chain(const EngineArrays& a, int frames_between, int flow_aided, unsigned new_mask_frames, hipStream_t s, hipEvent_t stop,
-                      hipEvent_t stop_early)
+                      hipEvent_t stop_early, bool single_flow_kernel)
 {
     const int n_grp = a.cam.W * a.cam.H / 64;
     constexpr int kBandRows = 20, kBandRowsFresh = 6;
@@ -761,13 +767,18 @@
         return std::min(per, n_grp);
     };
     const size_t lds_cap = 160 * 1024 - 4096;
-    auto frame_kernel = [](bool s16, int threads) {
+    auto frame_kernel = [](bool s16, int threads, bool single) {
+        if (single) return s16 ? mask_frame_kernel<ROFT_FLOW_S16C2, kFrameThreads, true> : mask_frame_kernel<ROFT_FLOW_F32C2, kFrameThreads, true>;
         if (threads == kFrameThreads) return s16 ? mask_frame_kernel<ROFT_FLOW_S16C2, kFrameThreads> : mask_frame_kernel<ROFT_FLOW_F32C2, kFrameThreads>;
         return s16 ? mask_frame_kernel<ROFT_FLOW_S16C2, kFreshThreads> : mask_frame_kernel<ROFT_FLOW_F32C2, kFreshThreads>;
     };
     auto general_kernel = [](bool s16) { return s16 ? mask_general_kernel<ROFT_FLOW_S16C2> : mask_general_kernel<ROFT_FLOW_F32C2>; };
     for (int threads : {kFrameThreads, kFreshThreads})
-        for (bool f16 : {true, false}) (void)set_max_dynamic_lds(reinterpret_cast<const void*>(frame_kernel(f16, threads)), (int)lds_cap);
+        for (bool f16 : {true, false}) (void)set_max_dynamic_lds(reinterpret_cast<const void*>(frame_kernel(f16, threads, false)), (int)lds_cap);
+    for (bool f16 : {true, false}) (void)set_max_dynamic_lds(reinterpret_cast<const void*>(frame_kernel(f16, kFrameThreads, true)), (int)lds_cap);
+    static const int kernel_env = getenv("ROFT_MASK_KERNEL") ? atoi(getenv("ROFT_MASK_KERNEL")) : -1;
+    const int kernel_forced = g_mask_kernel.load(std::memory_order_relaxed) >= 0 ? g_mask_kernel.load(std::memory_order_relaxed) : kernel_env;
+    const bool kernel_mode = kernel_forced >= 0 ? kernel_forced != 0 : single_flow_kernel;
     int launches = 0;
     const bool s16 = a.ffmt.type == ROFT_FLOW_S16C2;
     auto launch_general = [&](hipEvent_t ev, int final_launch) {
@@ -786,7 +797,7 @@
         win_cap = std::min(win_cap, ((lds_cap - fixed) / 4) & ~(size_t)1);
         const size_t lds = win_cap * 4 + fixed;
         const dim3 grid((n_grp + per - 1) / per, a.n_obj);
-        hipLaunchKernelGGL(frame_kernel(s16, threads), grid, dim3(threads), (uint32_t)lds, s, a, t, frames_between, flow_aided, per, margin, (int)win_cap);
+        hipLaunchKernelGGL(frame_kernel(s16, threads, !fresh && kernel_mode), grid, dim3(threads), (uint32_t)lds, s, a, t, frames_between, flow_aided, per, margin, (int)win_cap);
         ++launches;
         if (stop_early && t == a.T - 2) { launch_general(stop_early, 0); ++launches; }
     }
diff --git a/roft_amd/csrc/k_render.hip b/roft_amd/csrc/k_render.hip
--- a/roft_amd/csrc/k_render.hip
+++ b/roft_amd/csrc/k_render.hip
@@ -1,5 +1,6 @@
 #include <algorithm>
 #include <atomic>
+#include <cstring>
 #include <string>
 
 #include "mesh_clusters.h"
@@ -285,21 +286,22 @@
     }
 }
 
-constexpr int kFusedThreads = 1024;
+constexpr int kFusedThreads = 1024, kFusedThreadsHalf = 512;
 #ifdef ROFT_FUSED_PROFILE
 #define UTICK(i) do { __syncthreads(); if (threadIdx.x == 0 && bx < 4) { long long _t = wall_clock64(); st.dbg[bx * 8 + (i)] += _t - u_t0; u_t0 = _t; } } while (0)
 #else
 #define UTICK(i) do {} while (0)
 #endif
 
-template <bool GL>
-__global__ __launch_bounds__(kFusedThreads) void outlier_fused_kernel(EngineArrays a, int lin, int vcache_cap, int win_cap, int parts,
+template <bool GL, int THREADS>
+__global__ __launch_bounds__(THREADS) __attribute__((amdgpu_waves_per_eu(4)))
+void outlier_fused_kernel(EngineArrays a, int lin, int vcache_cap, int win_cap, int parts,
                                                                      int split_tris, float* tile_dump)
 {
     ROFT_RESIDENT(a, RK_OUTLIER);
     extern __shared__ __attribute__((aligned(16))) unsigned char smem[];
-    __shared__ long long s_hi[kFusedThreads / 64], s_lo[kFusedThreads / 64];
-    __shared__ int s_cnt[kFusedThreads / 64];
+    __shared__ long long s_hi[THREADS / 64], s_lo[THREADS / 64];
+    __shared__ int s_cnt[THREADS / 64];
     __shared__ int s_box[4];
     __shared__ int s_behind;
     __shared__ int s_last;
@@ -334,7 +336,7 @@
         else project_vertex(v, P, fx, fy, cx, cy, sx, sy, z);
     };
     if constexpr (GL) {
-        project_mesh<kFusedThreads, 4>(prm.verts, nv, cached, s_v, tw, th, s_box, &s_behind, project);
+        project_mesh<THREADS, 4>(prm.verts, nv, cached, s_v, tw, th, s_box, &s_behind, project);
         __syncthreads();
     } else {
         if (tid < 64 && prm.n_clusters > 0) {
@@ -351,7 +353,7 @@
         }
         __syncthreads();
         if (!s_settled) {
-            project_mesh<kFusedThreads, 4>(prm.verts, nv, false, s_v, tw, th, s_box, &s_behind, project);
+            project_mesh<THREADS, 4>(prm.verts, nv, false, s_v, tw, th, s_box, &s_behind, project);
             __syncthreads();
         }
     }
@@ -391,9 +393,9 @@
         for (int js = j0; js <= j1; js += rows) {
             const int je = min(j1, js + rows - 1), npx = win_w * (je - js + 1);
             if constexpr (GL) {
-                for (int i = tid; i < npx; i += kFusedThreads) s_k[i] = kGlKeyClear;
+                for (int i = tid; i < npx; i += THREADS) s_k[i] = kGlKeyClear;
             } else {
-                for (int i = tid; i < npx; i += kFusedThreads) s_z[i] = kDepthEmpty;
+                for (int i = tid; i < npx; i += THREADS) s_z[i] = kDepthEmpty;
             }
             __syncthreads();
             UTICK(1);
@@ -407,19 +409,19 @@
             };
             if constexpr (GL) {
                 constexpr int kTB = 8;
-                for (int tb = tid; tb < nt; tb += kTB * kFusedThreads) {
+                for (int tb = tid; tb < nt; tb += kTB * THREADS) {
                     int idx[kTB][3];
 #pragma unroll
                     for (int k = 0; k < kTB; ++k) {
-                        const int32_t* tri = prm.tris + (size_t)3 * min(tb + k * kFusedThreads, nt - 1);
+                        const int32_t* tri = prm.tris + (size_t)3 * min(tb + k * THREADS, nt - 1);
                         idx[k][0] = tri[0]; idx[k][1] = tri[1]; idx[k][2] = tri[2];
                     }
 #pragma unroll
                     for (int k = 0; k < kTB; ++k) {
-                        if (tb + k * kFusedThreads >= nt) break;
+                        if (tb + k * THREADS >= nt) break;
                         float x0, y0, z0, x1, y1, z1, x2, y2, z2;
                         fetch_triangle(s_v, cached, prm.verts, idx[k][0], idx[k][1], idx[k][2], project, x0, y0, z0, x1, y1, z1, x2, y2, z2);
-                        const uint64_t t = (uint32_t)(tb + k * kFusedThreads);
+                        const uint64_t t = (uint32_t)(tb + k * THREADS);
                         raster_projected_gl(x0, y0, z0, x1, y1, z1, x2, y2, z2, tw, th, js, je,
                                             [&](int i, int j, uint32_t qz) { store_key(i, j, ((uint64_t)qz << 32) | t); });
                     }
@@ -429,7 +431,7 @@
                 const bool cones = rule_on && fx > 0.0f && fy > 0.0f && pose_is_rotation(P.R);
                 const float f_lo = fminf(fx, fy), f_hi = fmaxf(fx, fy), c_abs = fabsf(cx) + fabsf(cy);
                 const int lane = tid & 63, wave = __builtin_amdgcn_readfirstlane(tid >> 6);
-                const int nc = prm.n_clusters, n_waves = kFusedThreads / 64;
+                const int nc = prm.n_clusters, n_waves = THREADS / 64;
                 auto cluster_of = [=](int i) { return (i * n_waves + wave) * G + grp; };
                 auto fetch = [&](int c, float (&v)[3], uint32_t& w) {
                     const float* sl = prm.cl_slots + (size_t)c * 3 * kClusterSize + lane;
@@ -477,7 +479,7 @@
                 const size_t slab0 = (((size_t)lin * a.zmerge_slabs + (size_t)obj * parts + (size_t)band * G) * 2 + alt) * a.zmerge_stride;
                 uint32_t* mine = a.zmerge + slab0 + (size_t)grp * 2 * a.zmerge_stride;
                 int* arrivals = a.zcount + (((size_t)lin * a.n_obj + obj) * 2 + alt) * kMaxOutlierParts + band;
-                for (int i = tid; i < npx; i += kFusedThreads)
+                for (int i = tid; i < npx; i += THREADS)
                     __hip_atomic_store(&mine[i], s_z[i], __ATOMIC_RELAXED, __HIP_MEMORY_SCOPE_AGENT);
                 __atomic_signal_fence(__ATOMIC_SEQ_CST);
                 __builtin_amdgcn_s_waitcnt(0);
@@ -501,7 +503,7 @@
                         if (p < G && p != grp && k < 7) op[k++] = others + (size_t)p * slab_step;
                     for (; k < 7; ++k) op[k] = others;
                 }
-                for (int i = tid; i < npx; i += kFusedThreads) {
+                for (int i = tid; i < npx; i += THREADS) {
                     uint32_t m = s_z[i];
                     uint32_t v0, v1, v2, v3, v4, v5, v6;
                     switch (G - 1) {
@@ -543,25 +545,25 @@
             if (tile_dump) {
                 float* tile = tile_dump + (size_t)alt * tw * th;
                 if constexpr (GL) {
-                    for (int i = tid; i < npx; i += kFusedThreads) {
+                    for (int i = tid; i < npx; i += THREADS) {
                         const uint64_t key = s_k[i];
                         const int pi = i0 + i % win_w, pj = js + i / win_w;
                         tile[(size_t)pj * tw + pi] = ((uint32_t)(key >> 32) == kGlDepthClear) ? 0.0f : gl_resolve(key, pi, pj);
                     }
                 } else {
-                    for (int i = tid; i < npx; i += kFusedThreads) {
+                    for (int i = tid; i < npx; i += THREADS) {
                         const uint32_t b = s_z[i];
                         tile[(size_t)(js + i / win_w) * tw + (i0 + i % win_w)] = (b == kDepthEmpty) ? 0.0f : __uint_as_float(b);
                     }
                 }
             }
             constexpr int kBatch = 16;
-            for (int f0 = tid; f0 < n; f0 += kBatch * kFusedThreads) {
+            for (int f0 = tid; f0 < n; f0 += kBatch * THREADS) {
                 float dep[kBatch];
                 uint32_t pix[kBatch];
 #pragma unroll
                 for (int k = 0; k < kBatch; ++k) {
-                    const int i = f0 + k * kFusedThreads;
+                    const int i = f0 + k * THREADS;
                     dep[k] = (i < n) ? fdep[i] : 0.0f;
                     pix[k] = (i < n) ? fpix[i] : 0u;
                 }
@@ -599,7 +601,7 @@
     if (tid == 0) {
         long long hi = 0, lo = 0;
         int n2 = 0;
-        for (int w = 0; w < kFusedThreads / 64; ++w) { hi += s_hi[w]; lo += s_lo[w]; n2 += s_cnt[w]; }
+        for (int w = 0; w < THREADS / 64; ++w) { hi += s_hi[w]; lo += s_lo[w]; n2 += s_cnt[w]; }
         pl.part_hi[alt][band] = hi;
         pl.part_lo[alt][band] = lo;
         pl.part_cnt[alt][band] = (double)n2;
@@ -609,25 +611,45 @@
 
 static std::atomic<int> g_outlier_split{-1};
 void set_outlier_split(int mode) { g_outlier_split.store(mode < 0 ? -1 : (mode ? 1 : 0), std::memory_order_relaxed); }
+static std::atomic<int> g_outlier_threads{-1}, g_outlier_parts_scale{-1};
+bool set_outlier_shape(int threads, int parts_scale)
+{
+    if (!(threads < 0 || threads == kFusedThreads || threads == kFusedThreadsHalf) || !(parts_scale < 0 || parts_scale == 1 || parts_scale == 2)) return false;
+    g_outlier_threads.store(threads < 0 ? -1 : threads, std::memory_order_relaxed);
+    g_outlier_parts_scale.store(parts_scale < 0 ? -1 : parts_scale, std::memory_order_relaxed);
+    return true;
+}
+constexpr size_t kFusedHalfLds = 72 * 1024;
 
 int launch_outlier(const EngineArrays& a, int lin, hipStream_t s, hipEvent_t stop, const OutlierLaunchOpts* opts)
 {
     if (!(opts && opts->render_mode == ROFT_RENDER_GL) && a.meshes_without_clusters > 0)
         return host::fail(ROFT_ERR_STATE, "outlier test: a mesh went up without clusters (MeshLayout::kWalkClusters)");
-    const size_t lds_total = kRasterLdsBudget;
+    const size_t lds_budget = kRasterLdsBudget;
     const size_t vbytes = vertex_cache_bytes(a.max_verts);
     const bool gl = opts && opts->render_mode == ROFT_RENDER_GL;
     const size_t zb = gl ? 8 : 4;
     const size_t min_win = zb * std::max(8192, a.tile_w);
-    const bool cache = gl && vbytes + min_win <= lds_total && !(opts && opts->no_vertex_cache);
+    const bool cache = gl && vbytes + min_win <= lds_budget && !(opts && opts->no_vertex_cache);
     const int vcache_cap = cache ? a.max_verts : 0;
+    static const char* shape_env = getenv("ROFT_OUTLIER_SHAPE");
+    static const int env_threads = shape_env ? atoi(shape_env) : -1, env_scale = (shape_env && strchr(shape_env, ',')) ? atoi(strchr(shape_env, ',') + 1) : -1;
+    const int k_threads = g_outlier_threads.load(std::memory_order_relaxed), k_scale = g_outlier_parts_scale.load(std::memory_order_relaxed);
+    int threads = k_threads > 0 ? k_threads : env_threads > 0 ? env_threads : (opts && opts->threads > 0) ? opts->threads : kFusedThreads;
+    int parts_scale = k_scale > 0 ? k_scale : env_scale > 0 ? env_scale : (opts && opts->parts_scale > 0) ? opts->parts_scale : 1;
+    const bool half = !gl && threads == kFusedThreadsHalf;
+    if (!half) parts_scale = 1;
+    const size_t lds_total = half ? std::max((size_t)kFusedHalfLds, zb * (size_t)a.tile_w) : lds_budget;
     int win_cap = (int)((lds_total - (cache ? vbytes : 0)) / zb);
-    (void)set_max_dynamic_lds(gl ? reinterpret_cast<const void*>(outlier_fused_kernel<true>) : reinterpret_cast<const void*>(outlier_fused_kernel<false>),
-                              (int)lds_total);
+    const void* kernel = gl ? reinterpret_cast<const void*>(outlier_fused_kernel<true, kFusedThreads>)
+                       : half ? reinterpret_cast<const void*>(outlier_fused_kernel<false, kFusedThreadsHalf>)
+                              : reinterpret_cast<const void*>(outlier_fused_kernel<false, kFusedThreads>);
+    (void)set_max_dynamic_lds(kernel, (int)lds_budget);
     int parts = std::max(1, std::min(kMaxOutlierParts, device_cu_count() / (2 * std::max(a.n_obj, 1))));
     if (a.outlier_parts > 0) parts = std::min(a.outlier_parts, kMaxOutlierParts);
     if (opts && opts->parts > 0) parts = std::min(opts->parts, kMaxOutlierParts);
     if (opts && opts->parts < 0) parts = std::max(1, parts / -opts->parts);
+    if (parts_scale == 2 && 2 * parts <= kMaxOutlierParts) parts *= 2;
     static const int split_env = getenv("ROFT_OUTLIER_SPLIT") ? atoi(getenv("ROFT_OUTLIER_SPLIT")) : -1;
     const int forced = g_outlier_split.load(std::memory_order_relaxed) >= 0 ? g_outlier_split.load(std::memory_order_relaxed) : split_env;
     int split = (opts && opts->split >= 0) ? opts->split : (forced >= 0 ? forced : 1);
@@ -638,12 +660,17 @@
     const size_t lds = std::min(lds_total, (((cache ? vbytes : 0) + win_need + 15) & ~(size_t)15));
     win_cap = std::min(win_cap, (int)((lds - (cache ? vbytes : 0)) / zb));
     if (opts && opts->window_pixels > 0) win_cap = std::max(a.tile_w, std::min(win_cap, opts->window_pixels));
+    const dim3 grid(2 * parts * ((a.n_obj + 7) / 8) * 8);
+    float* const dump = opts ? opts->tile_dump : nullptr;
     if (gl)
-        hipExtLaunchKernelGGL(outlier_fused_kernel<true>, dim3(2 * parts * ((a.n_obj + 7) / 8) * 8), dim3(kFusedThreads), (uint32_t)lds, s, nullptr, stop, 0, a,
-                              lin, vcache_cap, win_cap, parts, split, opts ? opts->tile_dump : nullptr);
+        hipExtLaunchKernelGGL((outlier_fused_kernel<true, kFusedThreads>), grid, dim3(kFusedThreads), (uint32_t)lds, s, nullptr, stop, 0, a, lin, vcache_cap,
+                              win_cap, parts, split, dump);
+    else if (half)
+        hipExtLaunchKernelGGL((outlier_fused_kernel<false, kFusedThreadsHalf>), grid, dim3(kFusedThreadsHalf), (uint32_t)lds, s, nullptr, stop, 0, a, lin,
+                              vcache_cap, win_cap, parts, split, dump);
     else
-        hipExtLaunchKernelGGL(outlier_fused_kernel<false>, dim3(2 * parts * ((a.n_obj + 7) / 8) * 8), dim3(kFusedThreads), (uint32_t)lds, s, nullptr, stop, 0, a,
-                              lin, vcache_cap, win_cap, parts, split, opts ? opts->tile_dump : nullptr);
+        hipExtLaunchKernelGGL((outlier_fused_kernel<false, kFusedThreads>), grid, dim3(kFusedThreads), (uint32_t)lds, s, nullptr, stop, 0, a, lin, vcache_cap,
+                              win_cap, parts, split, dump);
     return ROFT_OK;
 }
 
diff --git a/roft_amd/csrc/roft_device.h b/roft_amd/csrc/roft_device.h
--- a/roft_amd/csrc/roft_device.h
+++ b/roft_amd/csrc/roft_device.h
@@ -360,7 +360,8 @@
     }
 }
 int launch_mask_chain(const EngineArrays& a, int frames_between, int flow_aided, unsigned new_mask_frames, hipStream_t s, hipEvent_t stop = nullptr,
-                      hipEvent_t stop_early = nullptr);
+                      hipEvent_t stop_early = nullptr,
+                      bool single_flow_kernel = false);
 void launch_planes_to_mask(const uint32_t* nz, const uint32_t* ob, int npix, uint8_t* mask, hipStream_t s);
 void launch_flow_measure(const EngineArrays& a, double depth_max, int radius, hipStream_t s,
                          hipEvent_t start = nullptr, hipEvent_t stop = nullptr);
@@ -381,9 +382,13 @@
     float* tile_dump = nullptr;
     int split = -1;
     int render_mode = ROFT_RENDER_CONTRACT;
+    int threads = 0;
+    int parts_scale = 0;
 };
 int launch_outlier(const EngineArrays& a, int lin, hipStream_t s, hipEvent_t stop = nullptr, const OutlierLaunchOpts* opts = nullptr);
 void set_outlier_split(int mode);
+bool set_outlier_shape(int threads, int parts_scale);
+void set_mask_kernel(int mode);
 void launch_outlier_only(const EngineArrays& a, hipStream_t s);
 
 int device_cu_count();
```

Result: slower. 1.731 million object-frames/s (-2.6%).
